# kazuto1011/dusty-gan-v2

Hardware: AMD Instinct MI355X
Metric: range-images/sec (G+D step) on dusty_v2 64x512 (higher is better)
Workload: dtype bf16; 1 GPU; configs[2]: configs/gans/dusty_v2.yaml full G+D train step (G step + D step + lazy R1 + ADA + EMA + Adam), 64x512 synthetic; global_batch=64, per_gpu_batch=64, parallelism=dp1, hip_graph=True, d_epilogue_dtype=fp32, pe_table_precomputed=True

## Files before the change

### dusty-gan-v2_amd/csrc/conv_wgrad_stream.hip

```cpp
#include "gemm_core.h"

namespace {

struct WSGeom {
  int B, H, W, C, O, Ho, Wo, k, stride, pad, ring;
  int tiles_h, tiles_w, ntiles, tiles_per_split, ctiles;
#ifdef DGV2_ABLATE
  int ablate;
#define WS_ABL (g.ablate)
#else
#define WS_ABL 0
#endif
  int x_shared;
  int x_exact;
  int* status;
};

template <typename T, int S, int MFN, int NFN, bool K3>
struct WSCfg {
  static constexpr int KS = TnFrag<T>::KS;
  static constexpr int CE = 16 / sizeof(T);
  static constexpr int TO = 16 * MFN, TC = 16 * NFN;
  static constexpr int PAD = sizeof(T) == 4 ? 16 : 0;
  static constexpr int RO = TO + PAD, RC = TC + PAD;
// ... 500 lines not shown
      rg[j][1] = src[1];
      if (!ok) rg[j][0] = rg[j][1] = make_float4(0.f, 0.f, 0.f, 0.f);
    }
#pragma unroll
    for (int j = 0; j < NX; ++j) {
      const int id = tid + j * 256;
      const int xp = xpos[j] < 0 ? 0 : xpos[j];
      int hi = h0 - 1 + (xp >> 16), wi = w0 - 1 + (xp & 0xffff);
      hi = hi < 0 ? 0 : (hi >= g.H ? g.H - 1 : hi);
      wi = wi < 0 ? wi + g.W : (wi >= g.W ? wi - g.W : wi);
      const float4* src = reinterpret_cast<const float4*>(xb + (hi * g.W + wi) * g.C + (id & 7) * 8);
      rx[j][0] = src[0];
      rx[j][1] = src[1];
    }
  };

  f32x4 acc[9][4];
#pragma unroll
  for (int t = 0; t < 9; ++t)
#pragma unroll
    for (int mw = 0; mw < 4; ++mw) acc[t][mw] = (f32x4){0.f, 0.f, 0.f, 0.f};

  const int fg = lane >> 4, fi = lane & 15;
  const int fq = fi >> 2, fp = fi & 3;
  int voffA[4][2], voffB[3][2];
#pragma unroll
  for (int h = 0; h < 2; ++h) {
    const int L = 8 * fg + fq + 4 * h;
#pragma unroll
    for (int mw = 0; mw < 4; ++mw) voffA[mw][h] = L * 128 + ((mw ^ wz_swz<128>(L)) * 32) + 8 * fp;
#pragma unroll
    for (int cs = 0; cs < 3; ++cs) voffB[cs][h] = 3 * GYB + (cs + L) * 128 + ((wave ^ wz_swz<128>(cs + L)) * 32) + 8 * fp;
  }

  const int t_begin = split * g.tiles_per_split;
  const int t_end = min(t_begin + g.tiles_per_split, g.ntiles);
  tw_n = t_begin % g.tiles_w;
  th_n = (t_begin / g.tiles_w) % g.tiles_h;
  b_n = t_begin / (g.tiles_w * g.tiles_h);
  if (t_begin < t_end) issue();
  for (int t = t_begin; t < t_end; ++t) {
    __syncthreads();
#pragma unroll
    for (int j = 0; j < NG; ++j) {
      uint4 h, m, l;
      wx_split8(rg[j][0], rg[j][1], h, m, l);
      lds_gy[gw_[j]] = h;
      lds_gy[GYB / 16 + gw_[j]] = m;
      lds_gy[2 * (GYB / 16) + gw_[j]] = l;
    }
#pragma unroll
    for (int j = 0; j < NX; ++j) {
      uint4 h, m, l;
      wx_split8(rx[j][0], rx[j][1], h, m, l);
      if (xpos[j] >= 0) {
        lds_x[xw_[j]] = h;
        if (!xe) {
          lds_x[XB / 16 + xw_[j]] = m;
          lds_x[2 * (XB / 16) + xw_[j]] = l;
        } else if ((m.x | m.y | m.z | m.w) != 0u) {
          atomicOr(g.status, DGV2_STATUS_X_INEXACT);
        }
      }
    }
    if (t + 1 < t_end) issue();
    __syncthreads();
    wx3_tile<XE>(acc, lbase, voffA, voffB);
  }
  __builtin_amdgcn_sched_barrier(0);
  asm volatile("s_nop 15\n\ts_nop 15" ::: "memory");
  __builtin_amdgcn_sched_barrier(0);

  const int lr = lane & 15, lc = lane >> 4;
  float* pb = part + (int64_t)split * g.O * 9 * g.C;
  const int c = c0 + wave * 16 + lr;
#pragma unroll
  for (int tap = 0; tap < 9; ++tap)
#pragma unroll
    for (int mw = 0; mw < 4; ++mw)
#pragma unroll
      for (int r = 0; r < 4; ++r) {
        const int o = o0 + mw * 16 + lc * 4 + r;
        pb[((int64_t)o * 9 + tap) * g.C + c] = acc[tap][mw][r];
      }
}

template <int NC>
__global__ __launch_bounds__(1024) void conv_wgrad_x3_tail_kernel(float* __restrict__ tpart, const float* __restrict__ gy,
                                                                  const float* __restrict__ x, WSGeom g, int c0, int tiles_per_ts) {
  __shared__ float red[8][128];
  const int ts = blockIdx.x, o0 = blockIdx.y * 128;
  const int ol = threadIdx.x & 127, pl = threadIdx.x >> 7;
  const int t_begin = ts * tiles_per_ts, t_end = min(t_begin + tiles_per_ts, g.ntiles);
  float acc[9][NC];
#pragma unroll
  for (int t = 0; t < 9; ++t)
#pragma unroll
    for (int k = 0; k < NC; ++k) acc[t][k] = 0.f;
  for (int tile = t_begin; tile < t_end; ++tile) {
    const int tw = tile % g.tiles_w, th = (tile / g.tiles_w) % g.tiles_h, b = tile / (g.tiles_w * g.tiles_h);
    const float* gyb = gy + (int64_t)b * g.Ho * g.Wo * g.O + o0 + ol;
    const float* xb = x + (int64_t)b * g.H * g.W * g.C + c0;
#pragma unroll 4
    for (int p = pl; p < 128; p += 8) {
      const int ho = th * 4 + (p >> 5), wo = tw * 32 + (p & 31);
      if (ho >= g.Ho) continue;
      const float gv = gyb[(ho * g.Wo + wo) * g.O];
#pragma unroll
      for (int t = 0; t < 9; ++t) {
        int hi = ho + t / 3 - 1, wi = wo + t % 3 - 1;
        hi = hi < 0 ? 0 : (hi >= g.H ? g.H - 1 : hi);
        wi = wi < 0 ? wi + g.W : (wi >= g.W ? wi - g.W : wi);
        const float* xp = xb + (hi * g.W + wi) * g.C;
#pragma unroll
        for (int k = 0; k < NC; ++k) acc[t][k] = fmaf(gv, xp[k], acc[t][k]);
      }
    }
  }
  float* out = tpart + ((int64_t)ts * g.O + o0 + ol) * 9 * NC;
#pragma unroll
  for (int t = 0; t < 9; ++t)
#pragma unroll
    for (int k = 0; k < NC; ++k) {
      red[pl][ol] = acc[t][k];
      __syncthreads();
      if (pl == 0) {
        float v = red[0][ol];
#pragma unroll
        for (int l = 1; l < 8; ++l) v += red[l][ol];
        out[t * NC + k] = v;
      }
      __syncthreads();
    }
}

__global__ __launch_bounds__(256) void conv_wgrad_x3_tail_reduce_kernel(float* __restrict__ part, const float* __restrict__ tpart,
                                                                        int O, int C, int c0, int clive, int NC, int TS, int nsplit) {
  const int nz = C - c0;
  const int64_t n = (int64_t)nsplit * O * 9 * nz;
  for (int64_t i = blockIdx.x * 256 + threadIdx.x; i < n; i += (int64_t)gridDim.x * 256) {
    const int k = (int)(i % nz);
    const int64_t r = i / nz;
    const int t = (int)(r % 9);
    const int o = (int)((r / 9) % O), split = (int)(r / 9 / O);
    float v = 0.f;
    if (split == 0 && k < NC && c0 + k < clive)
      for (int s = 0; s < TS; ++s) v += tpart[(((int64_t)s * O + o) * 9 + t) * NC + k];
    part[(((int64_t)split * O + o) * 9 + t) * C + c0 + k] = v;
  }
}

__global__ __launch_bounds__(256) void wgrad_reduce_kernel(float* __restrict__ gw, const float* __restrict__ part,
                                                           int64_t n, int nsplit, float scale = 1.f, int kkC = 0,
                                                           int Cc = 0, int64_t ldo = 0) {
  __shared__ float4 red[16][16];
  const int col = threadIdx.x & 15, sl = threadIdx.x >> 4;
  const int64_t i = ((int64_t)blockIdx.x * 16 + col) * 4;
  part += (int64_t)blockIdx.y * nsplit * n;
  gw += (int64_t)blockIdx.y * (ldo > 0 ? (n / Cc) * ldo : n);
  float4 s = make_float4(0.f, 0.f, 0.f, 0.f);
  if (i < n) {
#pragma unroll 4
    for (int k = sl; k < nsplit; k += 16) {
      const float4 v = *reinterpret_cast<const float4*>(part + (int64_t)k * n + i);
      s.x += v.x; s.y += v.y; s.z += v.z; s.w += v.w;
    }
  }
  red[sl][col] = s;
  __syncthreads();
  if (sl == 0 && i < n) {
#pragma unroll
    for (int k = 1; k < 16; ++k) {
      const float4 v = red[k][col];
      s.x += v.x; s.y += v.y; s.z += v.z; s.w += v.w;
    }
    s.x *= scale; s.y *= scale; s.z *= scale; s.w *= scale;
    if (kkC == 0 && ldo > 0) {
      const int64_t r = i / Cc;
      *reinterpret_cast<float4*>(gw + r * ldo + (i - r * Cc)) = s;
    } else if (kkC == 0) {
      *reinterpret_cast<float4*>(gw + i) = s;
    } else {
      const float v4[4] = {s.x, s.y, s.z, s.w};
      const int kk = kkC / Cc;
#pragma unroll
      for (int e = 0; e < 4; ++e) {
        const int64_t lin = i + e;
        const int64_t o = lin / kkC;
        const int r = (int)(lin - o * kkC);
        const int t = r / Cc, c = r - t * Cc;
        gw[(o * Cc + c) * kk + t] = v4[e];
      }
    }
  }
}

struct WSPlan {
  WSGeom g;
  int nsplit, otiles, mfn, nfn;
  int go;
};

bool ws_plan(WSPlan& p, int B, int H, int W, int C, int O, int k, int stride, int pad, int ring, int dtype,
             bool per_image = false) {
  if (B <= 0 || H <= 0 || W <= 0 || C <= 0 || O <= 0) return false;
  if ((k != 1 && k != 3) || pad != (k - 1) / 2 || (stride != 1 && stride != 2)) return false;
  const int ce = dtype == DGV2_BF16 ? 8 : 4;
  if (C % ce || O % ce) return false;
  WSGeom& g = p.g;
  g = WSGeom{B, H, W, C, O, (H + 2 * pad - k) / stride + 1, (W + 2 * pad - k) / stride + 1, k, stride, pad, ring};
  if (g.Ho <= 0 || g.Wo <= 0) return false;
  const bool wide32 = dtype == DGV2_F32 && k == 3 && stride == 1 && C >= 128 && O >= 128;
  const bool big = dtype == DGV2_BF16 || wide32;
  p.mfn = (big && O > 32) ? 4 : 2;
  p.nfn = (big && C > 32) ? 4 : 2;
  const int wr = stride == 1 ? 4 : 2;
  g.tiles_h = (g.Ho + wr - 1) / wr;
  g.tiles_w = (g.Wo + 31) / 32;
  g.ntiles = B * g.tiles_h * g.tiles_w;
  g.ctiles = (C + 16 * p.nfn - 1) / (16 * p.nfn);
  static const bool no_go2 = getenv("DGV2_WS_NO_GO2") != nullptr;
  static const bool go2_s1 = getenv("DGV2_WS_GO2_S1") != nullptr;
  p.go = (!no_go2 && dtype == DGV2_BF16 && p.mfn == 4 && p.nfn == 4 && k == 3 && (stride == 2 || go2_s1) && O % 128 == 0 &&
          !per_image) ? 2 : 1;
  p.otiles = (O + 16 * p.mfn * p.go - 1) / (16 * p.mfn * p.go);
  const int pairs = g.ctiles * p.otiles;
#ifdef DGV2_ABLATE
  static const int abl = getenv("DGV2_WS_ABLATE") ? atoi(getenv("DGV2_WS_ABLATE")) : 0;
  g.ablate = abl;
#endif
  g.x_shared = 0;
  static const int blocks_big = getenv("DGV2_WS_BLOCKS_BIG") ? atoi(getenv("DGV2_WS_BLOCKS_BIG")) : 512;
  static const int blocks_small = getenv("DGV2_WS_BLOCKS_SMALL") ? atoi(getenv("DGV2_WS_BLOCKS_SMALL")) : 512;
  int nsplit = (p.go == 2 ? 256 : wide32 ? 512 : (p.mfn == 4 && p.nfn == 4) ? blocks_big : blocks_small) / pairs;
  nsplit = nsplit < 1 ? 1 : (nsplit > g.ntiles ? g.ntiles : nsplit);
  g.tiles_per_split = (g.ntiles + nsplit - 1) / nsplit;
  p.nsplit = (g.ntiles + g.tiles_per_split - 1) / g.tiles_per_split;
  if (per_image) {
    const int tpi = g.tiles_h * g.tiles_w;
    int spi = nsplit / B;
    spi = spi < 1 ? 1 : (spi > tpi ? tpi : spi);
    while (tpi % spi) --spi;
    g.tiles_per_split = tpi / spi;
    p.nsplit = B * spi;
  }
  return true;
}

template <typename T, int S, int MFN, int NFN, bool K3>
int ws_launch(float* part, const void* gy, const void* x, const WSPlan& p, hipStream_t st) {
  dim3 grid(p.nsplit, p.g.ctiles * p.otiles);
  if constexpr (sizeof(T) == 2) {
    if constexpr (MFN == 4 && NFN == 4 && K3) {
      if (p.go == 2) {
        using Cf2 = WZCfg<S, MFN, NFN, K3, 2>;
        auto kern2 = conv_wgrad_stream_bf16_kernel<S, MFN, NFN, K3, 2>;
        if (Cf2::LDS > 64 * 1024) {
          hipError_t e = hipFuncSetAttribute((const void*)kern2, hipFuncAttributeMaxDynamicSharedMemorySize, (int)Cf2::LDS);
          if (e != hipSuccess) return (int)e;
        }
        kern2<<<grid, 512, Cf2::LDS, st>>>(part, (const bf16_t*)gy, (const bf16_t*)x, p.g);
        return 0;
      }
    }
    using Cf = WZCfg<S, MFN, NFN, K3>;
    auto kern = conv_wgrad_stream_bf16_kernel<S, MFN, NFN, K3, 1>;
    if (Cf::LDS > 64 * 1024) {
      hipError_t e = hipFuncSetAttribute((const void*)kern, hipFuncAttributeMaxDynamicSharedMemorySize, (int)Cf::LDS);
      if (e != hipSuccess) return (int)e;
    }
    kern<<<grid, 256, Cf::LDS, st>>>(part, (const bf16_t*)gy, (const bf16_t*)x, p.g);
  } else {
    using Cf = WSCfg<T, S, MFN, NFN, K3>;
    auto kern = conv_wgrad_stream_kernel<T, S, MFN, NFN, K3>;
    if (Cf::LDS > 64 * 1024) {
      hipError_t e = hipFuncSetAttribute((const void*)kern, hipFuncAttributeMaxDynamicSharedMemorySize, (int)Cf::LDS);
      if (e != hipSuccess) return (int)e;
    }
    kern<<<grid, 256, Cf::LDS, st>>>(part, (const T*)gy, (const T*)x, p.g);
  }
  return 0;
}

template <typename T, int S, bool K3>
int ws_dispatch(float* part, const void* gy, const void* x, const WSPlan& p, hipStream_t st) {
  if constexpr (sizeof(T) == 2) {
    if (p.mfn == 4 && p.nfn == 4) return ws_launch<T, S, 4, 4, K3>(part, gy, x, p, st);
    if (p.mfn == 4) return ws_launch<T, S, 4, 2, K3>(part, gy, x, p, st);
    if (p.nfn == 4) return ws_launch<T, S, 2, 4, K3>(part, gy, x, p, st);
  } else if constexpr (S == 1 && K3) {
    if (p.mfn == 4 && p.nfn == 4) return ws_launch<T, S, 4, 4, K3>(part, gy, x, p, st);
  }
  return ws_launch<T, S, 2, 2, K3>(part, gy, x, p, st);
}

template <typename T>
int ws_dispatch_geom(float* part, const void* gy, const void* x, const WSPlan& p, hipStream_t st) {
  if (p.g.k == 3)
    return p.g.stride == 1 ? ws_dispatch<T, 1, true>(part, gy, x, p, st) : ws_dispatch<T, 2, true>(part, gy, x, p, st);
  return p.g.stride == 1 ? ws_dispatch<T, 1, false>(part, gy, x, p, st) : ws_dispatch<T, 2, false>(part, gy, x, p, st);
}

}

extern "C" int dgv2_conv_wgrad_stream_scratch(int64_t* elems, int B, int H, int W, int C, int O, int k, int stride,
                                              int pad, int dtype) {
  if (!elems) return DGV2_EINVAL;
  *elems = 0;
  WSPlan p;
  if (!ws_plan(p, B, H, W, C, O, k, stride, pad, 1, dtype)) return DGV2_EINVAL;
  *elems = (int64_t)p.nsplit * O * k * k * C;
  return 0;
}

extern "C" int dgv2_bmm_tn_stream_scratch(int64_t* elems, int B, int H, int W, int C, int O, int dtype) {
  if (!elems) return DGV2_EINVAL;
  *elems = 0;
  WSPlan p;
  if (!ws_plan(p, B, H, W, C, O, 1, 1, 0, 0, dtype, true)) return DGV2_EINVAL;
  *elems = (int64_t)p.nsplit * O * C;
  return 0;
}

extern "C" int dgv2_bmm_tn_stream_ld(float* gw, int64_t ldo, float* scratch, int64_t scratch_elems, const void* gy,
                                     const void* x, int x_shared, int B, int H, int W, int C, int O, int dtype, void* stream) {
  if (!gw || !scratch || !gy || !x || !aligned16(gy) || !aligned16(x) || !aligned16(scratch) || !aligned16(gw))
    return DGV2_EINVAL;
  if (ldo < 0 || (ldo > 0 && (ldo < C || (ldo & 3)))) return DGV2_EINVAL;
  if (dtype != DGV2_BF16 && dtype != DGV2_F32) return DGV2_EINVAL;
  WSPlan p;
  if (!ws_plan(p, B, H, W, C, O, 1, 1, 0, 0, dtype, true)) return DGV2_EINVAL;
  p.g.x_shared = x_shared != 0;
  const int64_t n = (int64_t)O * C;
  if (scratch_elems < (int64_t)p.nsplit * n || (n & 3)) return DGV2_EINVAL;
  hipStream_t st = (hipStream_t)stream;
  const int rc = dtype == DGV2_BF16 ? ws_dispatch_geom<bf16_t>(scratch, gy, x, p, st)
                                    : ws_dispatch_geom<float>(scratch, gy, x, p, st);
  if (rc) return rc;
  dim3 grid((unsigned)((n / 4 + 15) / 16), B);
  wgrad_reduce_kernel<<<grid, 256, 0, st>>>(gw, scratch, n, p.nsplit / B, 1.f, 0, C, ldo);
  DGV2_RETURN_LAST();
}

extern "C" int dgv2_conv_wgrad_stream_pl(float* gw, float* scratch, int64_t scratch_elems, const void* gy, const void* x,
                                         int B, int H, int W, int C, int O, int k, int stride, int pad, int ring,
                                         float scale, int param_layout, int dtype, void* stream) {
  if (!gw || !scratch || !gy || !x || !aligned16(gy) || !aligned16(x) || !aligned16(scratch) || !aligned16(gw))
    return DGV2_EINVAL;
  if (dtype != DGV2_BF16 && dtype != DGV2_F32) return DGV2_EINVAL;
  WSPlan p;
  if (!ws_plan(p, B, H, W, C, O, k, stride, pad, ring, dtype)) return DGV2_EINVAL;
  const int64_t n = (int64_t)O * k * k * C;
  if (scratch_elems < (int64_t)p.nsplit * n) return DGV2_EINVAL;
  hipStream_t st = (hipStream_t)stream;
  int rc;
  if (ring && (p.g.tiles_w * 32 - 1) * stride + k - 1 - pad < 2 * W && pad <= W) p.g.ring = 2;
  rc = dtype == DGV2_BF16 ? ws_dispatch_geom<bf16_t>(scratch, gy, x, p, st) : ws_dispatch_geom<float>(scratch, gy, x, p, st);
  if (rc) return rc;
  wgrad_reduce_kernel<<<(int)((n / 4 + 15) / 16), 256, 0, st>>>(gw, scratch, n, p.nsplit, scale,
                                                                 param_layout ? k * k * C : 0, C);
  DGV2_RETURN_LAST();
}

extern "C" int dgv2_conv3x3_x3_wgrad(float* gw, float* scratch, int64_t scratch_elems, const void* gy, const void* x, int B,
                                     int H, int W, int C, int clive, int x_exact, int O, float scale, int param_layout,
                                     int* status, void* stream) {
  if (!gw || !scratch || !gy || !x || !aligned16(gy) || !aligned16(x) || !aligned16(scratch) || !aligned16(gw))
    return DGV2_EINVAL;
  if (B < 1 || H < 1 || W < 1 || C < 1 || O < 1 || clive < 1 || clive > C || x_exact < 0 || x_exact > C) return DGV2_EINVAL;
  if (x_exact > 0 && !status) return DGV2_EINVAL;
  static const bool off = getenv("DGV2_NO_CONV_X3") != nullptr || getenv("DGV2_NO_WGRAD_X3") != nullptr;
  const int ctiles = C / 64, ntail = clive - ctiles * 64;
  if (off || O % 64 || ctiles < 1 || C % 8 || ntail > 16 || W % 32) return DGV2_ENOTSUP;
  if ((int64_t)B * H * W * (C > O ? C : O) >= (1ll << 31)) return DGV2_ENOTSUP;
  WSPlan p;
  WSGeom& g = p.g;
  g = WSGeom{B, H, W, C, O, H, W, 3, 1, 1, 2};
  g.tiles_h = (H + 3) / 4;
  g.tiles_w = W / 32;
  g.ntiles = B * g.tiles_h * g.tiles_w;
  g.ctiles = ctiles;
  g.x_shared = 0;
  g.x_exact = x_exact;
  g.status = status;
#ifdef DGV2_ABLATE
  g.ablate = 0;
#endif
  const int pairs = ctiles * (O / 64);
  int nsplit = 256 / pairs;
  nsplit = nsplit < 1 ? 1 : (nsplit > g.ntiles ? g.ntiles : nsplit);
  g.tiles_per_split = (g.ntiles + nsplit - 1) / nsplit;
  nsplit = (g.ntiles + g.tiles_per_split - 1) / g.tiles_per_split;
  const int64_t n = (int64_t)O * 9 * C;
  const bool tail = C > ctiles * 64;
  const int NC = ntail <= 1 ? 1 : (ntail <= 4 ? 4 : 16);
  const int TS = g.ntiles < 64 ? g.ntiles : 64, tiles_per_ts = (g.ntiles + TS - 1) / TS;
  const int64_t tneed = tail ? (int64_t)TS * O * 9 * NC : 0;
  if (scratch_elems < (int64_t)nsplit * n + tneed || O % 128) return DGV2_ENOTSUP;
  hipStream_t st = (hipStream_t)stream;
  const bool xe = x_exact >= ctiles * 64;
  auto kern = xe ? conv_wgrad_x3_kernel<true> : conv_wgrad_x3_kernel<false>;
  static bool attr_set[2] = {false, false};
  if (!attr_set[xe]) {
    hipError_t e = hipFuncSetAttribute((const void*)kern, hipFuncAttributeMaxDynamicSharedMemorySize, (int)WXCfg::LDS);
    if (e != hipSuccess) return (int)e;
    attr_set[xe] = true;
  }
  kern<<<dim3(nsplit, pairs), 256, WXCfg::LDS, st>>>(scratch, (const float*)gy, (const float*)x, g);
  if (tail) {
    float* tpart = scratch + (int64_t)nsplit * n;
    const dim3 tg(TS, O / 128);
    const int c0 = ctiles * 64;
    if (NC == 1) conv_wgrad_x3_tail_kernel<1><<<tg, 1024, 0, st>>>(tpart, (const float*)gy, (const float*)x, g, c0, tiles_per_ts);
    else if (NC == 4) conv_wgrad_x3_tail_kernel<4><<<tg, 1024, 0, st>>>(tpart, (const float*)gy, (const float*)x, g, c0, tiles_per_ts);
    else conv_wgrad_x3_tail_kernel<16><<<tg, 1024, 0, st>>>(tpart, (const float*)gy, (const float*)x, g, c0, tiles_per_ts);
    conv_wgrad_x3_tail_reduce_kernel<<<grid_for((int64_t)nsplit * O * 9 * (C - c0), 256), 256, 0, st>>>(scratch, tpart, O, C, c0,
                                                                                                      clive, NC, TS, nsplit);
  }
  wgrad_reduce_kernel<<<(int)((n / 4 + 15) / 16), 256, 0, st>>>(gw, scratch, n, nsplit, scale, param_layout ? 9 * C : 0, C);
  DGV2_RETURN_LAST();
}

extern "C" int dgv2_conv3x3_x3_wgrad_scratch(int64_t* elems, int B, int H, int W, int C, int clive, int O) {
  if (!elems) return DGV2_EINVAL;
  *elems = 0;
  if (B < 1 || H < 1 || W < 1 || C < 64 || O < 1 || clive < 1 || clive > C) return DGV2_EINVAL;
  const int ctiles = C / 64, ntail = clive - ctiles * 64;
  if (O % 128 || C % 8 || ntail > 16 || W % 32) return DGV2_ENOTSUP;
  const int ntiles = B * ((H + 3) / 4) * (W / 32);
  int nsplit = 256 / (ctiles * (O / 64));
  nsplit = nsplit < 1 ? 1 : (nsplit > ntiles ? ntiles : nsplit);
  const int tps = (ntiles + nsplit - 1) / nsplit;
  nsplit = (ntiles + tps - 1) / tps;
  const int NC = ntail <= 1 ? 1 : (ntail <= 4 ? 4 : 16);
  const int TS = ntiles < 64 ? ntiles : 64;
  *elems = (int64_t)nsplit * O * 9 * C + (C > ctiles * 64 ? (int64_t)TS * O * 9 * NC : 0);
  return 0;
}
```

### dusty-gan-v2_amd/csrc/conv_x3.hip

```cpp
#include <stdlib.h>

#include "gemm_core.h"

namespace {

struct CX3 {
  int B, H, W, Cx;
  int nchunks;
  int O, ldy;
  int xexact;
  int tiles_h, tiles_w, ntiles, npairs, nslab, per_xcd, total;
  int* status;
  const float* bias;
  const float* resid;
  int act;
  float alpha, scale;
#ifdef DGV2_ABLATE
  int ablate;
#define X3_ABL (p.ablate)
#else
#define X3_ABL 0
#endif
};

constexpr int X_ICOLS = 34, X_NPIX = 6 * X_ICOLS, X_PIN = 208, X_PW = 9 * 64, X_NI = 4, X_NW = 5;
constexpr int X_TILE = 3 * 4 * X_PIN;
constexpr int X_WBUF = 4 * X_PW;
constexpr size_t X_LDS = sizeof(uint4) * (2 * X_TILE + 2 * X_WBUF + 512);
static_assert(X_LDS <= 160 * 1024 - 1024, "LDS image");

__device__ __forceinline__ void split3x8(const float4& lo, const float4& hi, uint4& h, uint4& m, uint4& l) {
  const float f[8] = {lo.x, lo.y, lo.z, lo.w, hi.x, hi.y, hi.z, hi.w};
  union { uint4 u; bf16_t e[8]; } ph, pm, pl;
#pragma unroll
  for (int i = 0; i < 8; ++i) {
    const bf16_t hh = (bf16_t)f[i];
    const float r1 = f[i] - (float)hh;
    const bf16_t mm = (bf16_t)r1;
    const float r2 = r1 - (float)mm;
    ph.e[i] = hh;
    pm.e[i] = mm;
    pl.e[i] = (bf16_t)r2;
  }
  h = ph.u;
  m = pm.u;
  l = pl.u;
}


__device__ __forceinline__ bool exact1x8(const float4& lo, const float4& hi, uint4& h) {
  const float f[8] = {lo.x, lo.y, lo.z, lo.w, hi.x, hi.y, hi.z, hi.w};
  union { uint4 u; bf16_t e[8]; } ph;
  bool bad = false;
#pragma unroll
  for (int i = 0; i < 8; ++i) {
    ph.e[i] = (bf16_t)f[i];
    bad |= (f[i] - (float)ph.e[i]) != 0.f;
  }
  h = ph.u;
  return bad;
}

template <bool NOP>
__device__ __forceinline__ void mfma4_bf16(f32x4& c0, f32x4& c1, f32x4& c2, f32x4& c3, const uint4& a0, const uint4& a1,
                                           const uint4& a2, const uint4& a3, const uint4& b) {
  union U { uint4 u; bf16x8 v; };
  U ua0, ua1, ua2, ua3, ub;
  ua0.u = a0; ua1.u = a1; ua2.u = a2; ua3.u = a3; ub.u = b;
  if constexpr (NOP) {
    asm volatile(
        "v_mfma_f32_16x16x32_bf16 %0, %4, %8, %0\n\t"
        "v_mfma_f32_16x16x32_bf16 %1, %5, %8, %1\n\t"
        "v_mfma_f32_16x16x32_bf16 %2, %6, %8, %2\n\t"
        "v_mfma_f32_16x16x32_bf16 %3, %7, %8, %3\n\t"
        "s_nop 7"
        : "+v"(c0), "+v"(c1), "+v"(c2), "+v"(c3)
        : "v"(ua0.v), "v"(ua1.v), "v"(ua2.v), "v"(ua3.v), "v"(ub.v));
  } else {
    asm volatile(
        "v_mfma_f32_16x16x32_bf16 %0, %4, %8, %0\n\t"
        "v_mfma_f32_16x16x32_bf16 %1, %5, %8, %1\n\t"
        "v_mfma_f32_16x16x32_bf16 %2, %6, %8, %2\n\t"
        "v_mfma_f32_16x16x32_bf16 %3, %7, %8, %3"
        : "+v"(c0), "+v"(c1), "+v"(c2), "+v"(c3)
        : "v"(ua0.v), "v"(ua1.v), "v"(ua2.v), "v"(ua3.v), "v"(ub.v));
  }
}

#define X3_SB() __builtin_amdgcn_sched_barrier(0)
#ifdef DGV2_ABLATE
__device__ int x3_abl_noreads;
#define X3_NOREADS (x3_abl_noreads != 0)
#else
#define X3_NOREADS false
#endif

template <int NX, int HZ, typename Side>
__device__ __forceinline__ void x3_stage(f32x4 (&acc)[4][2], const uint4* __restrict__ a_base, const uint4* __restrict__ xb,
                                         const int (&bpix)[2], unsigned dead, Side&& side) {
  constexpr int SLOTS = 2 * NX;
  const bool noreads = X3_NOREADS;
  uint4 a[2][4], bb[2][NX];
  unsigned dd = 0u;
  if constexpr (HZ != 0) {
    dd = dead;
    asm volatile("" : "+s"(dd));
  }
#pragma unroll
  for (int mf = 0; mf < 4; ++mf) a[0][mf] = a_base[mf * 16];
#pragma unroll
  for (int nf = 0; nf < 2; ++nf)
#pragma unroll
    for (int q = 0; q < NX; ++q) bb[nf][q] = xb[q * 4 * X_PIN + bpix[nf]];
#pragma unroll
  for (int t = 0; t < 9; ++t) {
#pragma unroll
    for (int nf = 0; nf < 2; ++nf) {
#pragma unroll
      for (int qi = 0; qi < NX; ++qi) {
        const int q = NX - 1 - qi;
        X3_SB();
        if (!(HZ && ((dd >> t) & 1u)))
        {
          mfma4_bf16<true>(acc[0][nf], acc[1][nf], acc[2][nf], acc[3][nf], a[t & 1][0], a[t & 1][1], a[t & 1][2], a[t & 1][3], bb[nf][q]);
        }
        if constexpr (HZ != 0) {
          if (t < 3 || t >= 6) {
            const int tm = t < 3 ? t + 6 : t - 6;
            if ((dd >> tm) & 1u) {
              const uint4 bx = xb[q * 4 * X_PIN + bpix[nf] + X_ICOLS + t % 3];
              mfma4_bf16<true>(acc[0][nf], acc[1][nf], acc[2][nf], acc[3][nf], a[t & 1][0], a[t & 1][1], a[t & 1][2], a[t & 1][3], bx);
            }
          }
        }
        X3_SB();
        if (t + 1 < 9 && !noreads) {
          const int ky = (t + 1) / 3, kx = (t + 1) % 3;
          bb[nf][q] = xb[q * 4 * X_PIN + bpix[nf] + ky * X_ICOLS + kx];
          const int slot = nf * NX + qi;
#pragma unroll
          for (int k = 0; k < 4; ++k)
            if (k >= slot * 4 / SLOTS && k < (slot + 1) * 4 / SLOTS) a[(t + 1) & 1][k] = a_base[(t + 1) * 64 + k * 16];
        }
      }
    }
    X3_SB();
    side(t);
  }
  X3_SB();
}

template <int HZ, bool XE>
__global__ __launch_bounds__(512, 2) void conv_x3_kernel(float* __restrict__ y, const float* __restrict__ x,
                                                         const bf16_t* __restrict__ wimg, CX3 p) {
  extern __shared__ __attribute__((aligned(16))) uint4 smem[];
  __shared__ __attribute__((aligned(16))) float s_bias[64];
  const int n = blockIdx.x, kk = n >> 3;
  const int item = (n & 7) * p.per_xcd + kk;
  if (kk >= p.per_xcd || item >= p.total) return;
  const int slab = item / p.npairs, pair = item - slab * p.npairs;

  const int tid = threadIdx.x;
  const int t256 = tid & 255, gn = tid >> 8;
  const int wave4 = (tid >> 6) & 3, lane = tid & 63;
  const int lr = lane & 15, lc = lane >> 4;
  uint4* const xs = smem + gn * X_TILE;
  uint4* const wb = smem + 2 * X_TILE;
// ... 19 lines not shown
    gh = gh < 0 ? 0 : (gh >= p.H ? p.H - 1 : gh);
    int gw = w0 - 1 + ix;
    gw = gw < 0 ? gw + p.W : (gw >= p.W ? gw - p.W : gw);
    goff[j] = (gh * p.W + gw) * p.Cx + in_plane * 8;
    lrow[j] = pix < X_NPIX ? pix : -1;
  }
  float4 rin[X_NI][2];
  bool rin_ok = true;
  auto issue_in = [&](int c0) {
    rin_ok = c0 + in_plane * 8 < p.Cx;
    const int cc = rin_ok ? c0 : -in_plane * 8;
#pragma unroll
    for (int j = 0; j < X_NI; ++j) {
      const float4* src = reinterpret_cast<const float4*>(xb_g + cc + goff[j]);
      rin[j][0] = src[0];
      rin[j][1] = src[1];
    }
  };
  typedef __attribute__((ext_vector_type(4))) unsigned u32x4;
  u32x4 rwt[X_NW];
  const size_t plane_units = (size_t)p.nslab * p.nchunks * (X_PW * 4);
  auto issue_w = [&](int st) {
    const int c = st / 3, pl = st - c * 3;
    const u32x4* img = reinterpret_cast<const u32x4*>(wimg) + pl * plane_units + ((size_t)slab * p.nchunks + c) * (X_PW * 4) + tid;
#pragma unroll
    for (int j = 0; j < X_NW; ++j)
      if (j < X_NW - 1 || tid + 512 * j < X_PW * 4) rwt[j] = img[512 * j];
  };
  const int w_plane = (tid >> 3) & 3, w_row0 = ((tid >> 5) << 3) | (tid & 7);
  auto write_w = [&](int buf) {
    uint4* dst = wb + buf * X_WBUF + w_plane * X_PW + w_row0;
#pragma unroll
    for (int j = 0; j < X_NW; ++j)
      if (j < X_NW - 1 || tid + 512 * j < X_PW * 4) *reinterpret_cast<u32x4*>(dst + 128 * j) = rwt[j];
  };

  f32x4 acc[4][2];
#pragma unroll
  for (int mf = 0; mf < 4; ++mf)
#pragma unroll
    for (int nf = 0; nf < 2; ++nf) acc[mf][nf] = (f32x4){0.f, 0.f, 0.f, 0.f};
  int bpix[2];
#pragma unroll
  for (int nf = 0; nf < 2; ++nf) bpix[nf] = wave4 * X_ICOLS + nf * 16 + lr;
  if (tid < 64) s_bias[tid] = p.bias ? p.bias[o0 + tid] : 0.f;

  unsigned dead = 0u;
  if constexpr (HZ != 0) {
    const int orow = h0 + wave4;
    unsigned m = 0;
#pragma unroll
    for (int t = 0; t < 9; ++t)
      if ((unsigned)(orow + t / 3 - 1) >= (unsigned)p.H) m |= 1u << t;
    dead = (unsigned)__builtin_amdgcn_readfirstlane((int)m);
  }

  const int nst = p.nchunks * 3;
  uint4* const w_dummy = smem + 2 * X_TILE + 2 * X_WBUF + tid;
  auto w_store = [&](int st, int j) {
    if (X3_ABL & 8) return;
    const bool in = j < X_NW - 1 || tid + 512 * j < X_PW * 4;
    uint4* dst = wb + ((st + 1) & 1) * X_WBUF + w_plane * X_PW + w_row0 + 128 * j;
    dst = in ? dst : w_dummy;
    *reinterpret_cast<u32x4*>(dst) = rwt[j];
  };
  auto w_load = [&](int st, int j) {
    if (X3_ABL & 8) return;
    const bool in = j < X_NW - 1 || tid + 512 * j < X_PW * 4;
    const int s2 = min(st + 2, nst - 1);
    const int c = s2 / 3, pl = s2 - c * 3;
    const u32x4* img = reinterpret_cast<const u32x4*>(wimg) + pl * plane_units + ((size_t)slab * p.nchunks + c) * (X_PW * 4) + tid;
    rwt[j] = img[in ? 512 * j : 0];
  };
  auto w_side = [&](int st, int t) {
    if (t < X_NW) w_store(st, t);
    if (t == 5) { w_load(st, 0); w_load(st, 1); }
    if (t > 5) w_load(st, t - 4);
  };
  uint4 xh[X_NI];
  auto split_store = [&](int j, bool all, bool ex) {
    if (ex) {
      const bool bad = exact1x8(rin[j][0], rin[j][1], xh[j]);
      if (bad && rin_ok && lrow[j] >= 0) atomicOr(p.status, DGV2_STATUS_X_INEXACT);
      if (!rin_ok) xh[j] = make_uint4(0u, 0u, 0u, 0u);
      if (all && lrow[j] >= 0) xs[in_plane * X_PIN + lrow[j]] = xh[j];
      return;
    }
    uint4 m, l;
    split3x8(rin[j][0], rin[j][1], xh[j], m, l);
    if (!rin_ok) xh[j] = m = l = make_uint4(0u, 0u, 0u, 0u);
    if (lrow[j] >= 0) {
      uint4* d = xs + in_plane * X_PIN + lrow[j];
      if (all) d[0] = xh[j];
      d[4 * X_PIN] = m;
      d[8 * X_PIN] = l;
    }
  };

  issue_w(0);
  issue_in(0);
  write_w(0);
  if (nst > 1) issue_w(1);
#pragma unroll
  for (int j = 0; j < X_NI; ++j) split_store(j, true, XE && 32 <= p.xexact);
  __syncthreads();
  const uint4* const xlane = xs + lc * X_PIN;
  for (int c = 0; c < p.nchunks; ++c) {
    const bool more = c + 1 < p.nchunks && !(X3_ABL & 4);
    const int st = c * 3;
    const bool ex = XE && (c + 1) * 32 <= p.xexact, ex_next = XE && (min(c + 1, p.nchunks - 1) + 1) * 32 <= p.xexact;
    const uint4* const a0 = wb + (st & 1) * X_WBUF + lc * X_PW + lr;
    const uint4* const a1 = wb + ((st + 1) & 1) * X_WBUF + lc * X_PW + lr;
    auto side0 = [&](int t) {
      w_side(st, t);
      if (t == 5 && !(X3_ABL & 4)) issue_in(min(c + 1, p.nchunks - 1) * 32);
    };
    if (X3_ABL & 2) { for (int t = 0; t < 9; ++t) side0(t); }
    else if (ex) x3_stage<1, HZ>(acc, a0, xlane, bpix, dead, side0);
    else x3_stage<3, HZ>(acc, a0, xlane, bpix, dead, side0);
    if (!(X3_ABL & 64)) __syncthreads();
    auto side1 = [&](int t) { w_side(st + 1, t); };
    if (X3_ABL & 2) { for (int t = 0; t < 9; ++t) side1(t); }
    else if (ex) x3_stage<1, HZ>(acc, a1, xlane, bpix, dead, side1);
    else x3_stage<2, HZ>(acc, a1, xlane, bpix, dead, side1);
    if (!(X3_ABL & 64)) __syncthreads();
    auto side2 = [&](int t) {
      if (t < X_NI && !(X3_ABL & 4)) split_store(t, false, ex_next);
      w_side(st + 2, t);
    };
    if (X3_ABL & 2) { for (int t = 0; t < 9; ++t) side2(t); }
    else x3_stage<1, HZ>(acc, a0, xlane, bpix, dead, side2);
    if (!(X3_ABL & 64)) __syncthreads();
    if (more) {
#pragma unroll
      for (int j = 0; j < X_NI; ++j)
        if (lrow[j] >= 0) xs[in_plane * X_PIN + lrow[j]] = xh[j];
      if (!(X3_ABL & 64)) __syncthreads();
    }
  }

  mfma_drain();
  const int gh = h0 + wave4;
#pragma unroll
  for (int nf = 0; nf < 2; ++nf) {
    const int gw = w0 + nf * 16 + lr;
    const bool live = tile_live && gh < p.H && gw < p.W;
    const int64_t row = (((int64_t)b * p.H + gh) * p.W + gw) * p.ldy;
#pragma unroll
    for (int mf = 0; mf < 4; ++mf) {
      const int o = o0 + mf * 16 + lc * 4;
      const float4 b4 = *reinterpret_cast<const float4*>(&s_bias[mf * 16 + lc * 4]);
      const float bq[4] = {b4.x, b4.y, b4.z, b4.w};
      float f[4];
#pragma unroll
      for (int r = 0; r < 4; ++r) {
        float t = acc[mf][nf][r] + bq[r];
        if (p.act == 3) t = fmaxf(t, t * p.alpha) * p.scale;
        f[r] = t;
      }
      if (live && o < p.O) {
        if (p.resid) {
          const float4 r4 = *reinterpret_cast<const float4*>(p.resid + row + o);
          f[0] += r4.x; f[1] += r4.y; f[2] += r4.z; f[3] += r4.w;
        }
        *reinterpret_cast<float4*>(y + row + o) = make_float4(f[0], f[1], f[2], f[3]);
      }
    }
  }
}

__global__ __launch_bounds__(256) void x3_dgrad_tail_kernel(float* __restrict__ gx, const float* __restrict__ gy,
                                                            const float* __restrict__ wt, const float* __restrict__ resid,
                                                            int B, int H, int W, int ldx, int O, int c0, int nc, int cend) {
  const int row = blockIdx.x;
  const int b = row / H, h = row - b * H;
  const int lane = threadIdx.x & 63, wave = threadIdx.x >> 6;
  const int per = (W + 3) / 4;
  const float* gimg = gy + (int64_t)b * H * W * O;
  const bool border = h == 0 || h == H - 1;
  for (int ci = 0; ci < nc; ++ci) {
    const float* wc = wt + (size_t)(c0 + ci) * 9 * O;
    for (int w0 = wave * per; w0 < min(W, (wave + 1) * per); w0 += 8) {
      float s[8];
#pragma unroll
      for (int k = 0; k < 8; ++k) s[k] = 0.f;
      for (int ob = lane * 4; ob < O; ob += 256) {
#pragma unroll
        for (int d = 0; d < 3; ++d) {
          const int gh = h + d - 1;
          if (gh < 0 || gh >= H) continue;
          const float* grow = gimg + (int64_t)gh * W * O + ob;
#pragma unroll
          for (int kx = 0; kx < 3; ++kx) {
            float4 k4 = *reinterpret_cast<const float4*>(wc + ((2 - d) * 3 + kx) * O + ob);
            if (d == 1 && border) {
              const float4 e = *reinterpret_cast<const float4*>(wc + ((h == 0 ? 0 : 2) * 3 + kx) * O + ob);
              k4.x += e.x; k4.y += e.y; k4.z += e.z; k4.w += e.w;
            }
#pragma unroll
            for (int k = 0; k < 8; ++k) {
              int j = w0 + k + 1 - kx;
              j = j < 0 ? j + W : (j >= W ? j - W : j);
              j = j >= W ? 0 : j;
              const float4 g = *reinterpret_cast<const float4*>(grow + (int64_t)j * O);
              s[k] = fmaf(g.x, k4.x, fmaf(g.y, k4.y, fmaf(g.z, k4.z, fmaf(g.w, k4.w, s[k]))));
            }
          }
        }
      }
#pragma unroll
      for (int k = 0; k < 8; ++k) {
        const float v = wave_sum(s[k]);
        const int w = w0 + k;
        if (lane == 0 && w < min(W, (wave + 1) * per)) {
          const int64_t at = ((int64_t)row * W + w) * ldx + c0 + ci;
          gx[at] = v + (resid ? resid[at] : 0.f);
        }
      }
    }
  }
  const int nz = cend - c0 - nc;
  for (int i = threadIdx.x; i < W * nz; i += 256) {
    const int64_t at = ((int64_t)row * W + i / nz) * ldx + c0 + nc + i % nz;
    gx[at] = resid ? resid[at] : 0.f;
  }
}

__global__ __launch_bounds__(256) void x3_image_fwd_kernel(bf16_t* __restrict__ w3, const float* __restrict__ w, int O, int Cp,
                                                           int nch) {
  const int n = O * 9 * nch * 4;
  const size_t plane = (size_t)(O >> 6) * nch * (X_PW * 4);
  for (int i = blockIdx.x * 256 + threadIdx.x; i < n; i += gridDim.x * 256) {
    const int c8 = i % (nch * 4), r = i / (nch * 4);
    const int t = r % 9, o = r / 9;
    float4 lo = make_float4(0.f, 0.f, 0.f, 0.f), hi = lo;
    if (c8 * 8 < Cp) {
      const float4* src = reinterpret_cast<const float4*>(w + ((size_t)o * 9 + t) * Cp + c8 * 8);
      lo = src[0];
      hi = src[1];
    }
    uint4 h, m, l;
    split3x8(lo, hi, h, m, l);
    const int row = t * 64 + (o & 63);
    const size_t unit = ((size_t)(o >> 6) * nch + (c8 >> 2)) * (X_PW * 4) + (row >> 3) * 32 + (c8 & 3) * 8 + (row & 7);
    uint4* img = reinterpret_cast<uint4*>(w3);
    img[unit] = h;
    img[plane + unit] = m;
    img[2 * plane + unit] = l;
  }
}

__global__ __launch_bounds__(256) void x3_image_bwd_kernel(bf16_t* __restrict__ w3t, const float* __restrict__ w, int O, int Cp,
                                                           int nslab) {
  const int CS = nslab * 64, nch = O / 32;
  const int n = CS * 9 * (O / 8);
  const size_t plane = (size_t)nslab * nch * (X_PW * 4);
  for (int i = blockIdx.x * 256 + threadIdx.x; i < n; i += gridDim.x * 256) {
    const int c = i % CS, r = i / CS;
    const int t = r % 9, o8 = r / 9;
    float f[8];
#pragma unroll
    for (int k = 0; k < 8; ++k) f[k] = w[((size_t)(o8 * 8 + k) * 9 + t) * Cp + c];
    uint4 h, m, l;
    split3x8(make_float4(f[0], f[1], f[2], f[3]), make_float4(f[4], f[5], f[6], f[7]), h, m, l);
    const int row = (8 - t) * 64 + (c & 63);
    const size_t unit = ((size_t)(c >> 6) * nch + (o8 >> 2)) * (X_PW * 4) + (row >> 3) * 32 + (o8 & 3) * 8 + (row & 7);
    uint4* img = reinterpret_cast<uint4*>(w3t);
    img[unit] = h;
    img[plane + unit] = m;
    img[2 * plane + unit] = l;
  }
}

template <int HZ, bool XE>
int launch_x3(float* y, const float* x, const bf16_t* wimg, CX3 p, hipStream_t st) {
  auto kern = conv_x3_kernel<HZ, XE>;
  static bool attr_set = false;
  if (!attr_set) {
    hipError_t e = hipFuncSetAttribute((const void*)kern, hipFuncAttributeMaxDynamicSharedMemorySize, (int)X_LDS);
    if (e != hipSuccess) return (int)e;
    attr_set = true;
  }
  p.tiles_h = (p.H + 3) / 4;
  p.tiles_w = p.W / 32;
  p.ntiles = p.B * p.tiles_h * p.tiles_w;
  p.npairs = (p.ntiles + 1) / 2;
  p.total = p.npairs * p.nslab;
  p.per_xcd = (p.total + 7) / 8;
#ifdef DGV2_ABLATE
  p.ablate = getenv("DGV2_X3_ABLATE") ? atoi(getenv("DGV2_X3_ABLATE")) : 0;
  {
    const int nr = (p.ablate & 128) ? 1 : 0;
    (void)hipMemcpyToSymbol(HIP_SYMBOL(x3_abl_noreads), &nr, sizeof(int));
  }
#endif
  kern<<<p.per_xcd * 8, 512, X_LDS, st>>>(y, x, wimg, p);
  return 0;
}

}

extern "C" int dgv2_conv3x3_x3_fwd(void* y, const void* x, const void* w3, int B, int H, int W, int Cx, int x_exact, int O,
                                   const float* bias, const void* resid, int act, float alpha, float scale, int* status,
                                   void* stream) {
  if (!y || !x || !w3 || B < 1 || H < 1 || W < 1 || Cx < 1 || O < 1 || x_exact < 0 || x_exact > Cx) return DGV2_EINVAL;
  if (x_exact > 0 && !status) return DGV2_EINVAL;
  if (act != 0 && act != 3) return DGV2_EINVAL;
  static const bool off = getenv("DGV2_NO_CONV_X3") != nullptr;
  if (off || W % 32 || Cx % 8 || O % 64 || Cx < 64) return DGV2_ENOTSUP;
  if (!aligned16(y) || !aligned16(x) || !aligned16(w3) || (resid && !aligned16(resid))) return DGV2_ENOTSUP;
  if ((int64_t)B * H * W * (Cx > O ? Cx : O) >= (1ll << 31)) return DGV2_ENOTSUP;
  CX3 p;
  p.B = B; p.H = H; p.W = W; p.Cx = Cx; p.nchunks = (Cx + 31) / 32; p.O = O; p.ldy = O; p.nslab = O / 64;
  p.xexact = x_exact;
  p.status = status;
  p.bias = bias; p.resid = (const float*)resid; p.act = act; p.alpha = alpha; p.scale = scale;
  const int rc = x_exact >= 32 ? launch_x3<0, true>((float*)y, (const float*)x, (const bf16_t*)w3, p, (hipStream_t)stream)
                               : launch_x3<0, false>((float*)y, (const float*)x, (const bf16_t*)w3, p, (hipStream_t)stream);
  if (rc) return rc;
  DGV2_RETURN_LAST();
}

extern "C" int dgv2_conv3x3_x3_dgrad(void* gx, const void* gy, const void* w3t, const void* wt, int B, int H, int W, int C,
                                     int ldx, int O, const void* resid, void* stream) {
  if (!gx || !gy || !w3t || !wt || B < 1 || H < 1 || W < 1 || C < 1 || ldx < C || O < 1) return DGV2_EINVAL;
  static const bool off = getenv("DGV2_NO_CONV_X3") != nullptr;
  const int nslab = C / 64, ntail = C - nslab * 64;
  if (off || H < 2 || W % 32 || O % 32 || O < 64 || nslab < 1 || ntail > 16 || ldx % 4 || nslab != ldx / 64)
    return DGV2_ENOTSUP;
  if (!aligned16(gx) || !aligned16(gy) || !aligned16(w3t) || !aligned16(wt) || (resid && !aligned16(resid))) return DGV2_ENOTSUP;
  if ((int64_t)B * H * W * (ldx > O ? ldx : O) >= (1ll << 31)) return DGV2_ENOTSUP;
  CX3 p;
  p.B = B; p.H = H; p.W = W; p.Cx = O; p.nchunks = O / 32; p.O = nslab * 64; p.ldy = ldx; p.nslab = nslab;
  p.xexact = 0;
  p.status = nullptr;
  p.bias = nullptr; p.resid = (const float*)resid; p.act = 0; p.alpha = 0.2f; p.scale = 1.f;
  hipStream_t st = (hipStream_t)stream;
  const int rc = launch_x3<1, false>((float*)gx, (const float*)gy, (const bf16_t*)w3t, p, st);
  if (rc) return rc;
  if (ldx > nslab * 64)
    x3_dgrad_tail_kernel<<<B * H, 256, 0, st>>>((float*)gx, (const float*)gy, (const float*)wt, (const float*)resid, B, H, W,
                                               ldx, O, nslab * 64, ntail, ldx);
  DGV2_RETURN_LAST();
}

extern "C" int dgv2_conv_x3_images(void* w3, void* w3t, const void* w, int O, int Cp, void* stream) {
  if ((!w3 && !w3t) || !w || O < 64 || O % 64 || Cp < 64 || Cp % 8) return DGV2_EINVAL;
  if ((w3 && !aligned16(w3)) || !aligned16(w) || (w3t && !aligned16(w3t))) return DGV2_EINVAL;
  hipStream_t st = (hipStream_t)stream;
  const int nch = (Cp + 31) / 32;
  if (w3)
    x3_image_fwd_kernel<<<grid_for((int64_t)O * 9 * nch * 4, 256), 256, 0, st>>>((bf16_t*)w3, (const float*)w, O, Cp, nch);
  if (w3t)
    x3_image_bwd_kernel<<<grid_for((int64_t)(Cp / 64) * 64 * 9 * (O / 8), 256), 256, 0, st>>>((bf16_t*)w3t, (const float*)w, O,
                                                                                                 Cp, Cp / 64);
  DGV2_RETURN_LAST();
}
```

### dusty-gan-v2_amd/csrc/mbstd.hip

```cpp
#include "common.h"

namespace {

constexpr int MB_G = 8;

struct MbGeom {
  int B, P, C, Cp, S, g, m, NS;
};

template <typename T, int N> __device__ __forceinline__ void ldN(const T* p, float (&f)[N]) {
  constexpr int V = vec16<T>::N;
#pragma unroll
  for (int h = 0; h < N / V; ++h) {
    vec16<T> v;
    v.load(p + h * V);
#pragma unroll
    for (int j = 0; j < V; ++j) f[h * V + j] = v.get(j);
  }
}
template <typename T, int N> __device__ __forceinline__ void stN(T* p, const float (&f)[N]) {
  constexpr int V = vec16<T>::N;
#pragma unroll
  for (int h = 0; h < N / V; ++h) {
    vec16<T> v;
#pragma unroll
    for (int j = 0; j < V; ++j) v.set(j, f[h * V + j]);
    v.store(p + h * V);
  }
}
template <typename TA, typename TB> struct mb_vn {
  static constexpr int value = vec16<TA>::N > vec16<TB>::N ? vec16<TA>::N : vec16<TB>::N;
};

template <typename T>
__global__ __launch_bounds__(256) void mbstd_partial_kernel(float* __restrict__ partial, const T* __restrict__ x, MbGeom q) {
  __shared__ float red[16];
  constexpr int VN = vec16<T>::N;
  const int sm = blockIdx.x, split = blockIdx.y;
  const int s = sm / q.m, mi = sm - s * q.m;
  const int64_t PC = (int64_t)q.P * q.C;
  const int64_t nvec = PC / VN;
  float acc = 0.f;
  for (int64_t v = (int64_t)split * 256 + threadIdx.x; v < nvec; v += (int64_t)q.NS * 256) {
    vec16<T> a[MB_G];
    float mu[VN];
#pragma unroll
    for (int j = 0; j < VN; ++j) mu[j] = 0.f;
#pragma unroll
    for (int gi = 0; gi < MB_G; ++gi) {
      if (gi < q.g) {
        const int b = (s * q.g + gi) * q.m + mi;
        a[gi].load(x + (int64_t)b * PC + v * VN);
#pragma unroll
        for (int j = 0; j < VN; ++j) mu[j] += a[gi].get(j);
      }
    }
    const float ig = 1.f / q.g;
#pragma unroll
    for (int j = 0; j < VN; ++j) {
      const float mean = mu[j] * ig;
      float var = 0.f;
#pragma unroll
      for (int gi = 0; gi < MB_G; ++gi)
        if (gi < q.g) {
          const float d = a[gi].get(j) - mean;
          var = fmaf(d, d, var);
        }
      acc += sqrtf(var * ig + 1e-8f);
    }
  }
  const float t = block_sum(acc, red);
  if (threadIdx.x == 0) partial[sm * q.NS + split] = t;
}

template <typename TX, typename TY>
__global__ __launch_bounds__(256) void mbstd_cat_kernel(TY* __restrict__ out, const TX* __restrict__ x,
                                                        const float* __restrict__ partial, MbGeom q) {
  constexpr int VN = mb_vn<TX, TY>::value;
  const int cvp = q.Cp / VN, cvx = q.C / VN;
  const int64_t total = (int64_t)q.B * q.P * cvp;
  const float inv = 1.f / ((float)q.P * q.C);
  for (int64_t i = (int64_t)blockIdx.x * 256 + threadIdx.x; i < total; i += (int64_t)gridDim.x * 256) {
    const int cv = (int)(i % cvp);
    const int64_t bp = i / cvp;
    float o[VN];
    if (cv < cvx) {
      ldN<TX, VN>(x + bp * q.C + cv * VN, o);
    } else {
#pragma unroll
      for (int j = 0; j < VN; ++j) o[j] = 0.f;
      if (cv == cvx) {
        const int b = (int)(bp / q.P);
        const int sg = b / q.m, mi = b - sg * q.m, s = sg / q.g;
        float st = 0.f;
        for (int k = 0; k < q.NS; ++k) st += partial[(s * q.m + mi) * q.NS + k];
        o[0] = st * inv;
      }
    }
    stN<TY, VN>(out + bp * q.Cp + cv * VN, o);
  }
}

template <typename TX, typename TG>
__global__ __launch_bounds__(256) void mbstd_bwd_kernel(TX* __restrict__ gx, const TG* __restrict__ gout,
                                                        const TX* __restrict__ x, MbGeom q) {
  __shared__ float red[16];
  __shared__ float s_gst;
  constexpr int VN = mb_vn<TX, TG>::value;
  const int sm = blockIdx.x, split = blockIdx.y;
  const int s = sm / q.m, mi = sm - s * q.m;
  const int64_t PC = (int64_t)q.P * q.C;
  float part = 0.f;
  for (int e = threadIdx.x; e < q.g * q.P; e += 256) {
    const int gi = e / q.P, p = e - gi * q.P;
    const int b = (s * q.g + gi) * q.m + mi;
    part += to_f32(gout[((int64_t)b * q.P + p) * q.Cp + q.C]);
  }
  part = block_sum(part, red);
  if (threadIdx.x == 0) s_gst = part / ((float)q.P * q.C);
  __syncthreads();
  const float k = s_gst / q.g;
  const int cvx = q.C / VN;
  const int64_t nvec = PC / VN;
  for (int64_t v = (int64_t)split * 256 + threadIdx.x; v < nvec; v += (int64_t)q.NS * 256) {
    const int64_t p = v / cvx;
    const int cv = (int)(v - p * cvx);
    float a[MB_G][VN];
    float mu[VN];
#pragma unroll
    for (int j = 0; j < VN; ++j) mu[j] = 0.f;
#pragma unroll
    for (int gi = 0; gi < MB_G; ++gi) {
      if (gi < q.g) {
        const int b = (s * q.g + gi) * q.m + mi;
        ldN<TX, VN>(x + (int64_t)b * PC + v * VN, a[gi]);
#pragma unroll
        for (int j = 0; j < VN; ++j) mu[j] += a[gi][j];
      }
    }
    const float ig = 1.f / q.g;
    float coef[VN];
#pragma unroll
    for (int j = 0; j < VN; ++j) {
      mu[j] *= ig;
      float var = 0.f;
#pragma unroll
      for (int gi = 0; gi < MB_G; ++gi)
        if (gi < q.g) {
          const float d = a[gi][j] - mu[j];
          var = fmaf(d, d, var);
        }
      coef[j] = k / sqrtf(var * ig + 1e-8f);
    }
#pragma unroll
    for (int gi = 0; gi < MB_G; ++gi) {
      if (gi < q.g) {
        const int b = (s * q.g + gi) * q.m + mi;
        float go[VN], o[VN];
        ldN<TG, VN>(gout + ((int64_t)b * q.P + p) * q.Cp + cv * VN, go);
#pragma unroll
        for (int j = 0; j < VN; ++j) o[j] = go[j] + coef[j] * (a[gi][j] - mu[j]);
        stN<TX, VN>(gx + (int64_t)b * PC + v * VN, o);
      }
    }
  }
}

bool mb_ok(const MbGeom& q, int vn) {
  return q.B > 0 && q.P > 0 && q.C > 0 && q.S > 0 && q.g > 0 && q.g <= MB_G && q.m > 0 && q.S * q.g * q.m == q.B &&
         q.C % vn == 0 && q.Cp % vn == 0 && q.Cp > q.C && (int64_t)q.B * q.P * q.Cp < (1LL << 40);
}

int mb_splits(const MbGeom& q, int vn) {
  const int64_t nvec = (int64_t)q.P * q.C / vn;
  int ns = (int)((nvec + 1023) / 1024);
  const int want = (1024 + q.S * q.m - 1) / (q.S * q.m);
  ns = ns < want ? ns : want;
  return ns < 1 ? 1 : (ns > 64 ? 64 : ns);
}

}

extern "C" int dgv2_mbstd_cat_fwd_x(void* out, float* scratch, const void* x, int B, int P, int C, int Cp, int splits,
                                    int group, int xdtype, int ydtype, void* stream) {
  if (!out || !scratch || !x || splits < 1 || group < 1 || B % (splits * group)) return DGV2_EINVAL;
  if (xdtype != ydtype && !(xdtype == DGV2_BF16 && ydtype == DGV2_F32)) return DGV2_ENOTSUP;
  MbGeom q{B, P, C, Cp, splits, group, B / (splits * group), 1};
  const int vx = xdtype == DGV2_BF16 ? 8 : 4;
  if (!mb_ok(q, vx) || !aligned16(out) || !aligned16(x)) return DGV2_EINVAL;
  q.NS = mb_splits(q, vx);
  hipStream_t st = (hipStream_t)stream;
  dim3 grid(q.S * q.m, q.NS);
  const int64_t total = (int64_t)B * P * (Cp / vx);
  const int gc = grid_for(total, 256, 4096);
  if (xdtype == DGV2_F32) {
    mbstd_partial_kernel<float><<<grid, 256, 0, st>>>(scratch, (const float*)x, q);
    mbstd_cat_kernel<float, float><<<gc, 256, 0, st>>>((float*)out, (const float*)x, scratch, q);
  } else if (xdtype == DGV2_BF16) {
    mbstd_partial_kernel<bf16_t><<<grid, 256, 0, st>>>(scratch, (const bf16_t*)x, q);
    if (ydtype == DGV2_BF16)
      mbstd_cat_kernel<bf16_t, bf16_t><<<gc, 256, 0, st>>>((bf16_t*)out, (const bf16_t*)x, scratch, q);
    else
      mbstd_cat_kernel<bf16_t, float><<<gc, 256, 0, st>>>((float*)out, (const bf16_t*)x, scratch, q);
  } else {
    return DGV2_EINVAL;
  }
  DGV2_RETURN_LAST();
}

extern "C" int dgv2_mbstd_cat_bwd_x(void* gx, const void* gout, const void* x, int B, int P, int C, int Cp, int splits,
                                    int group, int xdtype, int gdtype, void* stream) {
  if (!gx || !gout || !x || splits < 1 || group < 1 || B % (splits * group)) return DGV2_EINVAL;
  if (xdtype != gdtype && !(xdtype == DGV2_BF16 && gdtype == DGV2_F32)) return DGV2_ENOTSUP;
  MbGeom q{B, P, C, Cp, splits, group, B / (splits * group), 1};
  const int vx = xdtype == DGV2_BF16 ? 8 : 4;
  if (!mb_ok(q, vx) || !aligned16(gx) || !aligned16(gout) || !aligned16(x)) return DGV2_EINVAL;
  q.NS = mb_splits(q, vx);
  hipStream_t st = (hipStream_t)stream;
  dim3 grid(q.S * q.m, q.NS);
  if (xdtype == DGV2_F32)
    mbstd_bwd_kernel<float, float><<<grid, 256, 0, st>>>((float*)gx, (const float*)gout, (const float*)x, q);
  else if (xdtype == DGV2_BF16 && gdtype == DGV2_BF16)
    mbstd_bwd_kernel<bf16_t, bf16_t><<<grid, 256, 0, st>>>((bf16_t*)gx, (const bf16_t*)gout, (const bf16_t*)x, q);
  else if (xdtype == DGV2_BF16)
    mbstd_bwd_kernel<bf16_t, float><<<grid, 256, 0, st>>>((bf16_t*)gx, (const float*)gout, (const bf16_t*)x, q);
  else
    return DGV2_EINVAL;
  DGV2_RETURN_LAST();
}
```

### dusty-gan-v2_amd/csrc/weight_bank.hip

```cpp
#include <stdlib.h>

#include "common.h"

namespace {

constexpr int WB_MAX = 32;

struct BankArgs {
  const float* src[WB_MAX];
  void* wf[WB_MAX];
  void* wt[WB_MAX];
  void* w8[WB_MAX];
  void* w8t[WB_MAX];
  int O[WB_MAX], C[WB_MAX], Cpad[WB_MAX], kk[WB_MAX];
  float scale[WB_MAX];
};

template <typename T>
__global__ __launch_bounds__(256) void weight_bank_kernel(BankArgs a) {
  const int l = blockIdx.y;
  const int O = a.O[l], C = a.C[l], Cp = a.Cpad[l], kk = a.kk[l];
  const float s = a.scale[l];
  const float* src = a.src[l];
  T* wf = reinterpret_cast<T*>(a.wf[l]);
  T* wt = reinterpret_cast<T*>(a.wt[l]);
  const int n = O * kk * Cp;
  for (int i = blockIdx.x * 256 + threadIdx.x; i < n; i += gridDim.x * 256) {
    const int c = i % Cp, r = i / Cp;
    const int t = r % kk, o = r / kk;
    const float v = c < C ? src[(o * C + c) * kk + t] * s : 0.f;
    wf[i] = from_f32<T>(v);
    wt[(c * kk + t) * O + o] = from_f32<T>(v);
  }
}

constexpr int WB_TO = 16, WB_TC = 32, WB_KK = 9;

template <typename T, int KK>
__global__ __launch_bounds__(256) void weight_bank_tiled_kernel(BankArgs a) {
  const int l = blockIdx.y;
  const int O = a.O[l], C = a.C[l], Cp = a.Cpad[l];
  const int kk = KK > 0 ? KK : a.kk[l];
  if (KK > 0 && a.kk[l] != KK) return;
  const int tc = (Cp + WB_TC - 1) / WB_TC, to = (O + WB_TO - 1) / WB_TO;
  if ((int)blockIdx.x >= tc * to) return;
  const int o0 = (blockIdx.x / tc) * WB_TO, c0 = (blockIdx.x % tc) * WB_TC;
  const float s = a.scale[l];
  const float* src = a.src[l];
  T* wf = reinterpret_cast<T*>(a.wf[l]);
  T* wt = reinterpret_cast<T*>(a.wt[l]);
  __shared__ float tile[WB_TO][WB_TC * WB_KK + 1];
  const int run = WB_TC * kk;
  for (int e0 = threadIdx.x; e0 < WB_TO * run; e0 += 256 * 8) {
    float v[8];
#pragma unroll
    for (int u = 0; u < 8; ++u) {
      const int e = e0 + u * 256;
      const int ec = min(e, WB_TO * run - 1);
      const int o = ec / run, r = ec - o * run;
      const int c = c0 + r / kk;
      const bool ok = e < WB_TO * run && o0 + o < O && c < C;
      const size_t idx = ok ? ((size_t)(o0 + o) * C + c0) * kk + r : 0;
      v[u] = ok ? src[idx] * s : 0.f;
    }
#pragma unroll
    for (int u = 0; u < 8; ++u) {
      const int e = e0 + u * 256;
      if (e < WB_TO * run) {
        const int o = e / run, r = e - o * run;
        tile[o][r] = v[u];
      }
    }
  }
  __syncthreads();
  for (int f = threadIdx.x; f < WB_TO * run; f += 256) {
    const int c = f % WB_TC, r = f / WB_TC;
    const int t = r % kk, o = r / kk;
    if (o0 + o < O && c0 + c < Cp) wf[((size_t)(o0 + o) * kk + t) * Cp + c0 + c] = from_f32<T>(tile[o][c * kk + t]);
  }
  if (KK == 9 && sizeof(T) == 2 && a.w8[l]) {
    T* w8 = reinterpret_cast<T*>(a.w8[l]);
    const int nchunks = Cp / WB_TC;
    for (int f = threadIdx.x; f < WB_TO * run; f += 256) {
      const int c = f % WB_TC, r = f / WB_TC;
      const int t = r % kk, o = r / kk;
      if (o0 + o < O) {
        const int og = o0 + o, row = t * 64 + (og & 63), plane = c >> 3;
        const size_t unit = ((size_t)(og >> 6) * nchunks + c0 / WB_TC) * (576 * 4) + (row >> 3) * 32 + plane * 8 + (row & 7);
        w8[unit * 8 + (c & 7)] = from_f32<T>(tile[o][c * kk + t]);
      }
    }
  }
  if (KK == 9 && sizeof(T) == 2 && a.w8t[l]) {
    T* w8t = reinterpret_cast<T*>(a.w8t[l]);
    const int nchunks = O / 32;
    for (int g = threadIdx.x; g < WB_TO * run; g += 256) {
      const int o = g % WB_TO, r = g / WB_TO;
      const int t = r % kk, c = r / kk;
      if (o0 + o < O && c0 + c < Cp) {
        const int og = o0 + o, cg = c0 + c, row = (8 - t) * 64 + (cg & 63), plane = (og & 31) >> 3;
        const size_t unit = ((size_t)(cg >> 6) * nchunks + (og >> 5)) * (576 * 4) + (row >> 3) * 32 + plane * 8 + (row & 7);
        w8t[unit * 8 + (og & 7)] = from_f32<T>(tile[o][c * kk + t]);
      }
    }
  }
  if constexpr (KK == 9 && sizeof(T) == 4) {
    auto split = [](float v, bf16_t& h, bf16_t& m, bf16_t& l) {
      h = (bf16_t)v;
      const float r1 = v - (float)h;
      m = (bf16_t)r1;
      l = (bf16_t)(r1 - (float)m);
    };
    if (a.w8[l]) {
      bf16_t* w8 = reinterpret_cast<bf16_t*>(a.w8[l]);
      const int nchunks = tc;
      const size_t plane = (size_t)(O >> 6) * nchunks * (576 * 4) * 8;
      for (int f = threadIdx.x; f < WB_TO * run; f += 256) {
        const int c = f % WB_TC, r = f / WB_TC;
        const int t = r % kk, o = r / kk;
        if (o0 + o < O) {
          const int og = o0 + o, row = t * 64 + (og & 63), pl = c >> 3;
          const size_t unit = ((size_t)(og >> 6) * nchunks + c0 / WB_TC) * (576 * 4) + (row >> 3) * 32 + pl * 8 + (row & 7);
          bf16_t h, m, lo;
          split(tile[o][c * kk + t], h, m, lo);
          w8[unit * 8 + (c & 7)] = h;
          w8[plane + unit * 8 + (c & 7)] = m;
          w8[2 * plane + unit * 8 + (c & 7)] = lo;
        }
      }
    }
    if (a.w8t[l]) {
      bf16_t* w8t = reinterpret_cast<bf16_t*>(a.w8t[l]);
      const int nchunks = O / 32, nslab = Cp >> 6;
      const size_t plane = (size_t)nslab * nchunks * (576 * 4) * 8;
      for (int g = threadIdx.x; g < WB_TO * run; g += 256) {
        const int o = g % WB_TO, r = g / WB_TO;
        const int t = r % kk, c = r / kk;
        if (o0 + o < O && c0 + c < nslab * 64) {
          const int og = o0 + o, cg = c0 + c, row = (8 - t) * 64 + (cg & 63), pl = (og & 31) >> 3;
          const size_t unit = ((size_t)(cg >> 6) * nchunks + (og >> 5)) * (576 * 4) + (row >> 3) * 32 + pl * 8 + (row & 7);
          bf16_t h, m, lo;
          split(tile[o][c * kk + t], h, m, lo);
          w8t[unit * 8 + (og & 7)] = h;
          w8t[plane + unit * 8 + (og & 7)] = m;
          w8t[2 * plane + unit * 8 + (og & 7)] = lo;
        }
      }
    }
  }
  for (int g = threadIdx.x; g < WB_TO * run; g += 256) {
    const int o = g % WB_TO, r = g / WB_TO;
    const int t = r % kk, c = r / kk;
    if (o0 + o < O && c0 + c < Cp) wt[((size_t)(c0 + c) * kk + t) * O + o0 + o] = from_f32<T>(tile[o][c * kk + t]);
  }
}

}

extern "C" int dgv2_conv_weight_bank_ex(void* const* wf, void* const* wt, void* const* w8, void* const* w8t,
                                        const float* const* src, const int* O, const int* C, const int* Cpad, const int* kk,
                                        const float* scale, int L, int dtype, void* stream) {
  if (!wf || !wt || !src || !O || !C || !Cpad || !kk || !scale || L < 1 || L > WB_MAX) return DGV2_EINVAL;
  BankArgs a;
  for (int l = 0; l < L; ++l) {
    a.w8[l] = w8 ? w8[l] : nullptr;
    a.w8t[l] = w8t ? w8t[l] : nullptr;
    if (dtype == DGV2_F32) {
      if (a.w8[l] && (kk[l] != 9 || O[l] % 64 || Cpad[l] % 8)) return DGV2_EINVAL;
      if (a.w8t[l] && (kk[l] != 9 || Cpad[l] < 64 || O[l] % 32)) return DGV2_EINVAL;
      continue;
    }
    if (a.w8[l] && (kk[l] != 9 || O[l] % 64 || Cpad[l] % 32 || dtype != DGV2_BF16)) return DGV2_EINVAL;
    if (a.w8t[l] && (kk[l] != 9 || Cpad[l] % 64 || O[l] % 32 || dtype != DGV2_BF16)) return DGV2_EINVAL;
  }
  int nmax = 0, tmax = 0, kmax = 0;
  for (int l = 0; l < L; ++l) {
    if (!wf[l] || !wt[l] || !src[l] || O[l] < 1 || C[l] < 1 || Cpad[l] < C[l] || kk[l] < 1) return DGV2_EINVAL;
    a.src[l] = src[l]; a.wf[l] = wf[l]; a.wt[l] = wt[l];
    a.O[l] = O[l]; a.C[l] = C[l]; a.Cpad[l] = Cpad[l]; a.kk[l] = kk[l]; a.scale[l] = scale[l];
    const int64_t n = (int64_t)O[l] * kk[l] * Cpad[l];
    if (n >= (1 << 30)) return DGV2_EINVAL;
    nmax = n > nmax ? (int)n : nmax;
    const int tiles = ((Cpad[l] + WB_TC - 1) / WB_TC) * ((O[l] + WB_TO - 1) / WB_TO);
    tmax = tiles > tmax ? tiles : tmax;
    kmax = kk[l] > kmax ? kk[l] : kmax;
  }
  hipStream_t st = (hipStream_t)stream;
  static const bool no_tiled = getenv("DGV2_NO_WB_TILED") != nullptr;
  if (kmax <= WB_KK && !no_tiled) {
    dim3 tgrid(tmax, L);
    bool has1 = false, has9 = false, other = false;
    for (int l = 0; l < L; ++l) {
      if (kk[l] == 1) has1 = true;
      else if (kk[l] == 9) has9 = true;
      else other = true;
    }
    if (other)
      for (int l = 0; l < L; ++l)
        if (a.w8[l] || a.w8t[l]) return DGV2_ENOTSUP;
    DGV2_DISPATCH_DTYPE(dtype, {
      if (other) {
        weight_bank_tiled_kernel<T, 0><<<tgrid, 256, 0, st>>>(a);
      } else {
        if (has9) weight_bank_tiled_kernel<T, 9><<<tgrid, 256, 0, st>>>(a);
        if (has1) weight_bank_tiled_kernel<T, 1><<<tgrid, 256, 0, st>>>(a);
      }
    });
    DGV2_RETURN_LAST();
  }
  for (int l = 0; l < L; ++l)
    if (a.w8[l] || a.w8t[l]) return DGV2_ENOTSUP;
  dim3 grid(grid_for(nmax, 256, 256), L);
  DGV2_DISPATCH_DTYPE(dtype, { weight_bank_kernel<T><<<grid, 256, 0, st>>>(a); });
  DGV2_RETURN_LAST();
}
```

### dusty-gan-v2_amd/dgv2_native/__init__.py

```python
import ctypes
import os

import torch

_HERE = os.path.dirname(os.path.abspath(__file__))
LIB_PATH = os.environ.get("DGV2_LIB_PATH") or os.path.join(os.path.dirname(_HERE), "lib", "libdgv2.so")

F32, BF16 = 0, 1
F16 = 3
ABI_VERSION = 60

_c_int, _c_i64, _c_f32, _c_ptr = ctypes.c_int, ctypes.c_int64, ctypes.c_float, ctypes.c_void_p

SIGNATURES = {
    "dgv2_abi_version": [],
    "dgv2_fused_bias_act": [_c_ptr] * 4 + [_c_i64] * 3 + [_c_int, _c_int, _c_f32, _c_f32, _c_int, _c_ptr],
    "dgv2_bias_grad": [_c_ptr, _c_ptr, _c_i64, _c_i64, _c_i64, _c_int, _c_ptr],
    "dgv2_bias_act_bwd_rs": [_c_ptr] * 4 + [_c_i64, _c_int, _c_f32, _c_f32, _c_ptr, _c_ptr, _c_i64, _c_int, _c_ptr],
    "dgv2_surface_normal": [_c_ptr, _c_ptr] + [_c_int] * 5 + [_c_ptr],
    "dgv2_gemm_x3": [_c_ptr, _c_ptr, _c_i64, _c_ptr, _c_ptr, _c_int, _c_int, _c_i64, _c_int, _c_int, _c_i64, _c_i64, _c_i64,
                     _c_int, _c_f32, _c_ptr],
    "dgv2_pe_wgrad_scratch": [_c_ptr] + [_c_int] * 4,
    "dgv2_pe_wgrad": [_c_ptr, _c_ptr, _c_i64, _c_ptr, _c_ptr] + [_c_int] * 4 + [_c_i64, _c_int, _c_ptr],
    "dgv2_mbstd_cat_fwd_x": [_c_ptr] * 3 + [_c_int] * 8 + [_c_ptr],
    "dgv2_mbstd_cat_bwd_x": [_c_ptr] * 3 + [_c_int] * 8 + [_c_ptr],
    "dgv2_scale_cast": [_c_ptr] * 3 + [_c_i64, _c_int, _c_int, _c_int, _c_ptr],
    "dgv2_upfirdn2d": [_c_ptr] * 3 + [_c_int] * 15 + [_c_ptr],
    "dgv2_resample": [_c_ptr] * 4 + [_c_int] * 19 + [_c_ptr],
    "dgv2_resample_tab_add_affine": [_c_ptr] * 8 + [_c_int] + [_c_ptr] * 3 + [_c_int] * 8 + [_c_ptr],
    "dgv2_fourier_feature": [_c_ptr] * 5 + [_c_int] * 8 + [_c_ptr],
    "dgv2_downsample_angle": [_c_ptr] * 4 + [_c_int] * 5 + [_c_ptr],
    "dgv2_bmm_tn": [_c_ptr] * 3 + [_c_int] * 7 + [_c_ptr],
    "dgv2_bmm_nn_cat_sq": [_c_ptr] * 4 + [_c_int] * 5 + [_c_ptr, _c_ptr, _c_int, _c_f32, _c_f32, _c_int, _c_int, _c_ptr, _c_int, _c_ptr,
                           _c_ptr],
    "dgv2_bmm_nn_sq": [_c_ptr] * 3 + [_c_int] * 6 + [_c_i64, _c_ptr, _c_ptr, _c_int, _c_f32, _c_f32, _c_ptr, _c_int, _c_int, _c_ptr, _c_int,
                       _c_ptr, _c_ptr],
    "dgv2_modconv_pe_fwd_sq": [_c_ptr] * 4 + [_c_int] * 5 + [_c_ptr, _c_ptr, _c_int, _c_f32, _c_f32, _c_int, _c_ptr, _c_int, _c_ptr,
                               _c_ptr],
    "dgv2_modconv_pe_fwd_head": [_c_ptr] * 4 + [_c_int] * 5 + [_c_ptr, _c_ptr, _c_int, _c_f32, _c_f32, _c_int, _c_ptr, _c_int, _c_ptr,
                                 _c_ptr, _c_ptr, _c_ptr],
    "dgv2_kitti_rows": [_c_ptr, _c_ptr, _c_ptr, _c_int, _c_int, _c_ptr],
    "dgv2_kitti_project": [_c_ptr] * 4 + [_c_int] * 4 + [_c_f32, _c_f32, _c_int, _c_ptr],
    "dgv2_fps_scratch": [_c_ptr, _c_int, _c_int],
    "dgv2_fps": [_c_ptr] * 3 + [_c_int] * 3 + [_c_ptr],
    "dgv2_gather_points": [_c_ptr] * 3 + [_c_int] * 4 + [_c_ptr],
    "dgv2_gather_points_grad": [_c_ptr] * 3 + [_c_int] * 4 + [_c_ptr],
    "dgv2_chamfer_fwd": [_c_ptr] * 6 + [_c_int] * 3 + [_c_ptr],
    "dgv2_nn_search": [_c_ptr] * 4 + [_c_int] * 4 + [_c_ptr],
    "dgv2_chamfer_bwd": [_c_ptr] * 8 + [_c_int] * 3 + [_c_ptr],
    "dgv2_emd_approxmatch": [_c_ptr] * 4 + [_c_int] * 3 + [_c_ptr],
    "dgv2_emd_matchcost": [_c_ptr] * 4 + [_c_int] * 3 + [_c_ptr],
    "dgv2_emd_matchcost_grad": [_c_ptr] * 5 + [_c_int] * 3 + [_c_ptr],
    "dgv2_emd_pairwise_cost": [_c_ptr] * 3 + [_c_int] * 4 + [_c_ptr],
    "dgv2_nsgan_loss": [_c_ptr, _c_ptr, _c_ptr, _c_int, _c_int, _c_f32, _c_ptr, _c_ptr, _c_ptr],
    "dgv2_modconv_pe_dgrad_actbwd_scratch": [_c_ptr] + [_c_int] * 4,
    "dgv2_modconv_pe_dgrad_actbwd": [_c_ptr, _c_ptr, _c_ptr, _c_i64] + [_c_ptr] * 4 + [_c_f32, _c_f32] + [_c_int] * 4 + [_c_ptr],
    "dgv2_colmean_lerp": [_c_ptr, _c_ptr, _c_int, _c_int, _c_i64, _c_f32, _c_ptr],
    "dgv2_d_tail_fwd": [_c_ptr] * 6 + [_c_int, _c_int] + [_c_f32] * 4 + [_c_ptr],
    "dgv2_d_tail_bwd": [_c_ptr] * 7 + [_c_int, _c_int] + [_c_f32] * 4 + [_c_ptr],
    "dgv2_rng_fill": [_c_ptr] * 5 + [_c_int, _c_ptr, _c_ptr],
    "dgv2_modconv_up_fwd": [_c_ptr] * 4 + [_c_int] * 7 + [_c_ptr] * 6 + [_c_int, _c_f32, _c_f32, _c_int, _c_ptr, _c_int, _c_ptr,
                            _c_ptr],
    "dgv2_modconv_up_t_lag": [_c_ptr] * 4 + [_c_f32] + [_c_ptr] * 4 + [_c_int] * 9 + [_c_ptr, _c_int, _c_ptr, _c_ptr],
    "dgv2_fir_same_mfma_q8": [_c_ptr] * 3 + [_c_int] * 4 + [_c_ptr],
    "dgv2_resample_tab_q8": [_c_ptr] * 5 + [_c_int] + [_c_ptr] * 3 + [_c_int] * 7 + [_c_ptr],
    "dgv2_fp8_quant_weights": [_c_ptr] * 6 + [_c_int] + [_c_ptr] * 3,
    "dgv2_fp8_dequant": [_c_ptr, _c_ptr, _c_i64, _c_f32, _c_ptr],
    "dgv2_conv_direct_fwd_fp8": [_c_ptr] * 4 + [_c_int] * 7 + [_c_ptr, _c_ptr, _c_int, _c_f32, _c_f32, _c_ptr],
    "dgv2_modconv_up_t": [_c_ptr] * 5 + [_c_f32] + [_c_int] * 9 + [_c_ptr],
    "dgv2_up2_lag_sumsq": [_c_ptr] * 5 + [_c_int] * 5 + [_c_ptr, _c_int, _c_ptr, _c_ptr],
    "dgv2_resample_tab_actbwd_scratch": [_c_ptr] + [_c_int] * 6,
    "dgv2_resample_tab_actbwd": [_c_ptr, _c_ptr, _c_ptr, _c_i64, _c_ptr, _c_ptr] + [_c_ptr] * 3 + [_c_int] + [_c_ptr] * 3
                                + [_c_int] * 7 + [_c_f32, _c_f32, _c_int, _c_ptr],
    "dgv2_fir_same_mfma_prep_scratch": [_c_ptr, _c_int, _c_int],
    "dgv2_fir_same_mfma_prep": [_c_ptr, _c_i64] + [_c_ptr] * 3 + [_c_int] + [_c_ptr] * 3 + [_c_int] * 3 + [_c_ptr, _c_ptr],
    "dgv2_fir_same_mfma": [_c_ptr] * 3 + [_c_int] * 4 + [_c_ptr],
    "dgv2_fir_same_mfma_actbwd_scratch": [_c_ptr] + [_c_int] * 4,
    "dgv2_fir_same_mfma_actbwd": [_c_ptr, _c_ptr, _c_ptr, _c_i64, _c_ptr, _c_ptr, _c_ptr] + [_c_int] * 4 + [_c_f32, _c_f32, _c_ptr],
    "dgv2_resample_tab_sq": [_c_ptr] * 5 + [_c_int] + [_c_ptr] * 3 + [_c_int] * 10 + [_c_ptr, _c_int, _c_ptr, _c_ptr],
    "dgv2_bmm_tn_cat": [_c_ptr] * 4 + [_c_int] * 6 + [_c_ptr],
    "dgv2_lerp_list": [_c_ptr] * 3 + [_c_int, _c_f32, _c_ptr],
    "dgv2_adam_prep": [_c_ptr, _c_ptr, _c_f32, _c_f32, _c_ptr],
    "dgv2_adam_step": [_c_ptr] * 5 + [_c_int, _c_ptr] + [_c_f32] * 4 + [_c_ptr],
    "dgv2_sumsq_list": [_c_ptr, _c_ptr, _c_int, _c_ptr, _c_ptr],
    "dgv2_clip_prep": [_c_ptr, _c_int, _c_f32, _c_ptr, _c_f32, _c_f32, _c_int, _c_ptr, _c_ptr],
    "dgv2_sgd_step": [_c_ptr] * 4 + [_c_int, _c_ptr] + [_c_f32] * 3 + [_c_ptr],
    "dgv2_pack2d": [_c_ptr] * 4 + [_c_int] * 3 + [_c_ptr],
    "dgv2_unpack2d": [_c_ptr] * 4 + [_c_int] * 3 + [_c_ptr],
    "dgv2_ema_scalar": [_c_ptr] * 3 + [_c_int] + [_c_f32] * 3 + [_c_int, _c_ptr, _c_int, _c_ptr],
    "dgv2_ema_scalar_group": [_c_ptr, _c_ptr, _c_int, _c_ptr, _c_int] + [_c_f32] * 3 + [_c_int, _c_ptr, _c_ptr],
    "dgv2_bmm_nn_small": [_c_ptr] * 4 + [_c_int] * 5 + [_c_ptr],
    "dgv2_bmm_nn_small_act_scratch": [_c_ptr] + [_c_int] * 5,
    "dgv2_bmm_nn_small_act": [_c_ptr] * 4 + [_c_int] * 4 + [_c_ptr, _c_ptr, _c_f32, _c_f32, _c_ptr, _c_ptr, _c_i64, _c_int, _c_ptr],
    "dgv2_bmm_tn_small": [_c_ptr] * 3 + [_c_int] * 5 + [_c_ptr],
    "dgv2_head_bwd_scratch": [_c_ptr] + [_c_int] * 5,
    "dgv2_head_bwd": [_c_ptr] * 5 + [_c_i64] + [_c_ptr] * 6 + [_c_f32, _c_f32] + [_c_int] * 5 + [_c_ptr],
    "dgv2_transpose_list": [_c_ptr] * 5 + [_c_int] * 3 + [_c_ptr],
    "dgv2_mod_prep_all_fwd": [_c_ptr] * 13 + [_c_ptr, _c_int, _c_int, _c_ptr],
    "dgv2_mod_prep_all_bwd": [_c_ptr, _c_i64] + [_c_ptr] * 15 + [_c_ptr, _c_int, _c_int, _c_ptr, _c_i64, _c_ptr],
    "dgv2_mod_prep_all_bwd_scratch": [_c_ptr, _c_ptr, _c_ptr, _c_int, _c_int],
    "dgv2_mod_prep_fwd": [_c_ptr] * 8 + [_c_int] * 9 + [_c_ptr],
    "dgv2_mod_prep_bwd": [_c_ptr] * 11 + [_c_int] * 9 + [_c_ptr],
    "dgv2_sum_squares": [_c_ptr, _c_ptr, _c_i64, _c_int, _c_int, _c_int, _c_ptr],
    "dgv2_conv_fwd": [_c_ptr] * 3 + [_c_int] * 10 + [_c_ptr, _c_int, _c_f32, _c_f32, _c_int, _c_ptr],
    "dgv2_conv_direct_fwd": [_c_ptr] * 3 + [_c_int] * 7 + [_c_ptr, _c_ptr, _c_int, _c_f32, _c_f32, _c_int, _c_ptr],
    "dgv2_conv_direct_dgrad": [_c_ptr] * 3 + [_c_int] * 7 + [_c_ptr, _c_int, _c_ptr],
    "dgv2_conv_wgrad_direct": [_c_ptr] * 3 + [_c_int] * 10 + [_c_ptr],
    "dgv2_conv1x1_fwd": [_c_ptr] * 3 + [_c_int] * 4 + [_c_ptr, _c_int, _c_ptr],
    "dgv2_conv1x1_dgrad": [_c_ptr] * 3 + [_c_int] * 4 + [_c_ptr, _c_int, _c_ptr],
    "dgv2_gemm_stream_nn": [_c_ptr] * 3 + [_c_int] * 6 + [_c_i64, _c_ptr, _c_ptr, _c_int, _c_f32, _c_f32, _c_ptr, _c_int, _c_int, _c_ptr,
                            _c_int, _c_ptr, _c_ptr],
    "dgv2_gemm_stream_nn_cat": [_c_ptr] * 4 + [_c_int] * 5 + [_c_ptr, _c_ptr, _c_int, _c_f32, _c_f32, _c_int, _c_int, _c_ptr, _c_int,
                                _c_ptr, _c_ptr],
    "dgv2_gemm_stream_tn": [_c_ptr] * 3 + [_c_int] * 7 + [_c_ptr],
    "dgv2_gemm_stream_tn_cat": [_c_ptr] * 4 + [_c_int] * 6 + [_c_ptr],
    "dgv2_bmm_tn_stream_scratch": [_c_ptr] + [_c_int] * 6,
    "dgv2_bmm_tn_stream_ld": [_c_ptr, _c_i64, _c_ptr, _c_i64, _c_ptr, _c_ptr] + [_c_int] * 7 + [_c_ptr],
    "dgv2_conv_weight_bank_ex": [_c_ptr] * 10 + [_c_int, _c_int, _c_ptr],
    "dgv2_glin_fwd": [_c_ptr] * 6 + [_c_int] * 3 + [_c_f32, _c_f32, _c_int, _c_f32, _c_int, _c_ptr, _c_ptr],
    "dgv2_glin_dinput": [_c_ptr, _c_int, _c_ptr, _c_i64, _c_ptr, _c_ptr, _c_ptr, _c_ptr, _c_int, _c_int, _c_int, _c_f32, _c_f32,
                         _c_int, _c_ptr],
    "dgv2_glin_dweight": [_c_ptr] * 7 + [_c_int] * 3 + [_c_f32, _c_f32, _c_f32, _c_ptr, _c_ptr],
    "dgv2_conv3x3_dgrad8": [_c_ptr] * 3 + [_c_int] * 5 + [_c_ptr, _c_int, _c_ptr],
    "dgv2_conv3x3_s2_dgrad8": [_c_ptr] * 3 + [_c_int] * 6 + [_c_ptr],
    "dgv2_conv3x3_x3_wgrad_scratch": [_c_ptr] + [_c_int] * 6,
    "dgv2_conv3x3_x3_wgrad": [_c_ptr, _c_ptr, _c_i64] + [_c_ptr] * 2 + [_c_int] * 7 + [_c_f32, _c_int, _c_ptr, _c_ptr],
    "dgv2_conv_x3_images": [_c_ptr] * 3 + [_c_int] * 2 + [_c_ptr],
    "dgv2_conv3x3_x3_dgrad": [_c_ptr] * 4 + [_c_int] * 6 + [_c_ptr, _c_ptr],
    "dgv2_conv3x3_x3_fwd": [_c_ptr] * 3 + [_c_int] * 6 + [_c_ptr, _c_ptr, _c_int, _c_f32, _c_f32, _c_ptr, _c_ptr],
    "dgv2_conv3x3_fwd8": [_c_ptr] * 3 + [_c_int] * 6 + [_c_ptr, _c_ptr, _c_int, _c_f32, _c_f32, _c_int, _c_ptr],
    "dgv2_conv_wgrad_stream_scratch": [_c_ptr] + [_c_int] * 9,
    "dgv2_conv_wgrad_stream_pl": [_c_ptr, _c_ptr, _c_i64, _c_ptr, _c_ptr] + [_c_int] * 9 + [_c_f32, _c_int, _c_int, _c_ptr],
    "dgv2_conv_dgrad": [_c_ptr] * 4 + [_c_int] * 11 + [_c_ptr],
    "dgv2_conv_wgrad": [_c_ptr] * 3 + [_c_int] * 11 + [_c_ptr],
    "dgv2_stem_fwd": [_c_ptr] * 4 + [_c_int] * 5 + [_c_f32, _c_f32, _c_int, _c_ptr],
    "dgv2_stem_bwd_scratch": [_c_ptr] + [_c_int] * 4,
    "dgv2_stem_bwd_skip": [_c_ptr] * 4 + [_c_i64] + [_c_ptr] * 8 + [_c_int] + [_c_ptr] * 3 + [_c_int] * 8 + [_c_f32, _c_f32, _c_int,
                                                                                                        _c_ptr],
    "dgv2_gen_tail_fwd": [_c_ptr] * 7 + [_c_int] * 3 + [_c_f32] * 3 + [_c_ptr],
    "dgv2_gen_tail_bwd": [_c_ptr] * 11 + [_c_int] * 3 + [_c_f32] * 3 + [_c_ptr],
    "dgv2_ada_apply": [_c_ptr] * 8 + [_c_int] * 5 + [_c_ptr],
    "dgv2_ada_sample": [_c_ptr] * 7 + [_c_int] * 3 + [_c_ptr],
    "dgv2_ada_build": [_c_ptr] * 8 + [_c_int] * 4 + [_c_ptr],
    "dgv2_ada_sample_img": [_c_ptr] * 7 + [_c_int, _c_ptr],
    "dgv2_ada_fold": [_c_ptr] * 11 + [_c_int] * 6 + [_c_ptr],
    "dgv2_ada_apply_img": [_c_ptr] * 11 + [_c_int] * 5 + [_c_ptr],
    "dgv2_coords_convert": [_c_ptr] * 4 + [_c_int] * 3 + [_c_f32] * 3 + [_c_int, _c_ptr],
    "dgv2_msml_prepare": [_c_ptr] * 6 + [_c_int] * 5 + [_c_ptr],
    "dgv2_msml_fwd": [_c_ptr] * 7 + [_c_int] * 7 + [_c_ptr],
    "dgv2_msml_bwd": [_c_ptr] * 9 + [_c_int] * 7 + [_c_ptr],
    "dgv2_coords_convert_bwd": [_c_ptr] * 5 + [_c_int] * 3 + [_c_f32, _c_f32, _c_int, _c_ptr],
    "dgv2_fourier_feature_bwd": [_c_ptr] * 6 + [_c_int] * 8 + [_c_ptr],
    "dgv2_frame_points": [_c_ptr] * 4 + [_c_int] * 3 + [_c_f32, _c_f32, _c_int, _c_ptr],
    "dgv2_colorize": [_c_ptr] * 3 + [_c_int] * 4 + [_c_ptr],
    "dgv2_crf_rnn_forward": [_c_ptr] * 11 + [_c_int] * 7 + [_c_ptr],
    "dgv2_crf_rnn_backward_scratch": [_c_ptr] + [_c_int] * 5,
    "dgv2_crf_rnn_backward": [_c_ptr] * 5 + [_c_i64] + [_c_ptr] * 11 + [_c_int] * 7 + [_c_ptr],
    "dgv2_knn2d": [_c_ptr] * 4 + [_c_int] * 7 + [_c_f32, _c_ptr],
    "dgv2_seg_confusion": [_c_ptr] * 4 + [_c_i64, _c_int, _c_ptr],
    "dgv2_seg_loss_scratch": [_c_ptr] + [_c_int] * 3,
    "dgv2_seg_loss_forward": [_c_ptr] * 5 + [_c_i64] + [_c_ptr] * 4 + [_c_int] * 4 + [_c_f32, _c_int, _c_ptr],
    "dgv2_seg_loss_backward": [_c_ptr] * 7 + [_c_int] * 4 + [_c_f32, _c_int, _c_int, _c_ptr],
    "dgv2_fire_fwd": [_c_ptr] * 23 + [_c_f32] * 3 + [_c_int] * 9 + [_c_ptr],
    "dgv2_cam_fwd": [_c_ptr] * 6 + [_c_int] * 6 + [_c_ptr],
}


def _load():
    if not os.path.exists(LIB_PATH):
        raise ImportError(
            f"{LIB_PATH} not found: build it with `make` (or __graft_entry__.build()). "
            "The MI355X path has no CPU fallback."
        )
    lib = ctypes.CDLL(LIB_PATH)
    for name, argtypes in SIGNATURES.items():
        fn = getattr(lib, name)
        fn.argtypes = argtypes
        fn.restype = ctypes.c_int
    got = lib.dgv2_abi_version()
    if got != ABI_VERSION:
        raise ImportError(f"libdgv2.so ABI version {got}, binding expects {ABI_VERSION}")
    return lib


lib = _load()


def dtype_code(t):
    if t.dtype == torch.float32:
        return F32
    if t.dtype == torch.bfloat16:
        return BF16
    raise RuntimeError(f"dgv2: unsupported dtype {t.dtype} (float32 / bfloat16 only)")


def check(*tensors):
    for t in tensors:
        if t is None:
            continue
        if not t.is_cuda:
            raise RuntimeError("dgv2: tensor must be a CUDA/HIP tensor (no CPU fallback)")
        if not t.is_contiguous():
            raise RuntimeError("dgv2: tensor must be contiguous")


def ptr(t):
    return None if t is None else t.data_ptr()


def stream():
    return torch.cuda.current_stream().cuda_stream


def ptr_array(tensors):
    return (ctypes.c_void_p * len(tensors))(*[None if t is None else t.data_ptr() for t in tensors])


def addr_array(addrs):
    return (ctypes.c_void_p * len(addrs))(*[None if v is None else int(v) for v in addrs])


def int_array(vals):
    return (ctypes.c_int * len(vals))(*[int(v) for v in vals])


EINVAL = -1
ENOTSUP = -3


def call(name, *args):
    rc = getattr(lib, name)(*args)
    if rc != 0:
        raise RuntimeError(f"{name} failed with code {rc}")


def try_call(name, *args):
    rc = getattr(lib, name)(*args)
    if rc == ENOTSUP:
        return False
    if rc != 0:
        raise RuntimeError(f"{name} failed with code {rc}")
    return True


_scratch_memo = {}


def scratch_elems(entry, *args):
    key = (entry, tuple(tuple(a) if isinstance(a, (list, tuple)) else a for a in args))
    n = _scratch_memo.get(key)
    if n is None:
        out = ctypes.c_int64(0)
        rc = getattr(lib, entry)(ctypes.addressof(out), *[int_array(a) if isinstance(a, tuple) else a for a in key[1]])
        if rc not in (0, ENOTSUP):
            raise RuntimeError(f"{entry} failed with code {rc}")
        n = _scratch_memo[key] = 0 if rc else out.value
    return n


SUMSQ_PARTS = 64
SGD_N_MAX = 2147483647 - (1 << 17)
STATUS_X_INEXACT, STATUS_FIR_TABLE = 1, 2
_STATUS_TEXT = {
    STATUS_X_INEXACT: "a launch with an x_exact promise (fp32 conv on conv_x3.hip / its weight gradient: 'these input "
                      "channels hold bf16-representable values') staged a value that is not: that launch computed on the "
                      "bf16 rounding of its input",
    STATUS_FIR_TABLE: "dgv2_fir_same_mfma_prep met a table entry outside its contract: the band operands are unusable",
}
_status_words = {}


def status_word(device=None):
    idx = torch.cuda.current_device() if device is None else torch.device(device).index
    idx = torch.cuda.current_device() if idx is None else idx
    w = _status_words.get(idx)
    if w is None:
        if torch.cuda.is_current_stream_capturing():
            raise RuntimeError("dgv2: the status word must exist before a hipGraph capture (call dgv2_native.status_word() "
                               "once outside the capture; gans.trainer.Trainer does)")
# ... 19 lines not shown
```

### dusty-gan-v2_amd/gans/models/dusty_v2.py

```python
import math
import os

import numpy as np
import torch
import torch.nn as nn
import torch.nn.functional as F
from torch.nn.modules.utils import _pair

from . import base, dusty_v1, ops
from .ops import native
from .ops.fourier import _CONST_CACHE

LOW = torch.bfloat16


class MappingNetwork(nn.Sequential):

    def __init__(self, in_ch, out_ch, depth=2):
        self.in_ch, self.out_ch, self.depth = in_ch, out_ch, depth
        layers = [ops.PixelNorm()]
        ch = in_ch
        for _ in range(depth):
            layers.append(nn.Sequential(
                ops.EqualLR(nn.Linear(ch, out_ch), gain=math.sqrt(2), lr_mul=0.01),
# ... 483 lines not shown
        v = v * self.synthesis_network.output_scale
        image_orig, logit = torch.tanh(v[:, :1]), v[:, 1:2]
        soft = torch.sigmoid((logit + u.log() - (-u).log1p()) / mm.gumbel_sigmoid.temperature)
        mask = ((soft > 0.5).to(soft.dtype) - soft).detach() + soft
        image = image_orig + (1.0 - mask) * (mm.const_host - image_orig)
        return {"image": image, "raydrop_logit": logit, "w": w, "raydrop_mask": mask, "image_orig": image_orig}

    def __init__(self, mapping_kwargs, synthesis_kwargs, measurement_kwargs):
        super().__init__(
            mapping_network=MappingNetwork(**mapping_kwargs),
            synthesis_network=SynthesisNetwork(**synthesis_kwargs),
            measurement_model=dusty_v1.RayDropModel(**measurement_kwargs),
        )

    def forward_synthesis(self, w, angle=None):
        angle = self.angle if angle is None else angle
        return self.synthesis_network(w, angle)

    def forward(self, z, angle=None, style_mixing=False, truncation_psi=1.0, input_w=False, noise=None,
                second_order=False):
        mm = self.measurement_model
        if len(mm.gumbel_sigmoid._forward_hooks) > 0:
            return super().forward(z, angle, style_mixing, truncation_psi, input_w)
        low = all(getattr(m, "use_fp16", False) for m in self.synthesis_network.layers)
        with native.glin_grad(low and not second_order):
            w = z if input_w else self.forward_mapping(z, style_mixing)
            assert w.ndim == 3
            if self.training:
                self.moving_average_w(w)
            else:
                w = self.truncation_trick(w, truncation_psi)
            angle = self.angle if angle is None else angle
            noise = noise or {}
            skip, shift = self.synthesis_network.synthesize(w, angle, noise.get("shifts", "auto"), composable=second_order)
        B, H, W, _ = skip.shape
        u = noise.get("gumbel_u")
        u = native.gumbel_uniform((B, 1, H, W), skip.device) if u is None else u.float().contiguous()
        if second_order:
            return self._output_stage_composable(skip, shift, u, w)
        image, image_orig, logit, mask = native.gen_tail(
            skip, shift, u, self.synthesis_network.output_scale, mm.const_host,
            mm.gumbel_sigmoid.temperature)
        return {"image": image, "raydrop_logit": logit, "w": w, "raydrop_mask": mask, "image_orig": image_orig}


def _ring_shift(v, shift_rad):
    B, C, H, W = v.shape
    pos = torch.arange(W, dtype=torch.float32, device=v.device)[None, :] + (shift_rad / (2 * math.pi))[:, None] * W
    j0 = pos.floor()
    f = (pos - j0)[:, None, None, :]
    j0 = j0.long()
    i0 = (j0 % W)[:, None, None, :].expand(B, C, H, W)
    i1 = ((j0 + 1) % W)[:, None, None, :].expand(B, C, H, W)
    return v.gather(3, i0) * (1 - f) + v.gather(3, i1) * f


class ResidualBlock(nn.Module):

    def __init__(self, in_ch: int, out_ch: int):
        super().__init__()
        kw = dict(bias=False, ring=True, equal_lr=True)
        self.conv1 = ops.Conv2d(in_ch, in_ch, 3, 1, 1, **kw)
        self.bias_act1 = ops.FusedLeakyReLU(in_ch)
        self.resample = ops.Resample(window=[1, 3, 3, 1], ring=True)
        self.conv2 = ops.Conv2d(in_ch, out_ch, 3, 2, 1, **kw)
        self.bias_act2 = ops.FusedLeakyReLU(out_ch)
        self.skip = ops.Conv2d(in_ch, out_ch, 1, 2, 0, **kw)
        self.blur_down = native.ResampleSpec([1, 3, 3, 1], down=(2, 2), ring=True, pads=(2, 1))
        self.skip_geom = native.ConvGeom(1, 1, 1, 0, True)

    def bank_entries(self, vec):
        c = 1.0 / math.sqrt(2)
        fused = self.skip.in_ch % vec == 0 and self.skip._params_bias()[0] is None
        return [(self.conv1, self.conv1.bank_entry()), (self.conv2, self.conv2.bank_entry()),
                (self.skip, self.skip.bank_entry(wscale=c if fused else None))]

    def fp8_entries(self, vec):
        if self.conv2.in_ch % 64 or self.conv2.out_ch < 64 or self.skip.in_ch % vec or self.skip._params_bias()[0] is not None:
            return []
        c = 1.0 / math.sqrt(2)
        return [(self.conv2, self.conv2.bank_entry()[:2]), (self.skip, self.skip.bank_entry(wscale=c)[:2])]

    def _forward_fp8(self, x, bank, fp8):
        spec = self.resample.spec
        if x.requires_grad:
            hd_h, hd8, x = self.conv1.forward_cl(x, act=self.bias_act1, bank=bank, fork=True, down=spec, q8=True)
        else:
            hd_h, hd8 = self.conv1.forward_cl(x, act=self.bias_act1, bank=bank, down=spec, q8=True)
        c = 1.0 / math.sqrt(2)
        xs = native.resample_q8(x, self.blur_down)
        h = self.conv2.forward_cl((hd_h, hd8), act=self.bias_act2, act_scale=self.bias_act2.scale * c, bank=bank,
                                  fp8=fp8[self.conv2])
        return self.skip.forward_cl(xs, geom=self.skip_geom, resid=h, wscale=c, bank=bank, fp8=fp8[self.skip])

    def forward_cl(self, x, bank=None, fp8=None, xs=None):
        if (xs is None and fp8 is not None and self.conv2 in fp8 and bank is not None and bank.get(self.conv1) is not None
                and isinstance(self.resample, ops.Resample) and native.fp8_ok(x, self.conv2.out_ch)):
            return self._forward_fp8(x, bank, fp8)
        hd = None
        if bank is not None and bank.get(self.conv1) is not None and isinstance(self.resample, ops.Resample):
            if x.requires_grad and xs is None:
                hd, x = self.conv1.forward_cl(x, act=self.bias_act1, bank=bank, fork=True, down=self.resample.spec)
            else:
                hd = self.conv1.forward_cl(x, act=self.bias_act1, bank=bank, down=self.resample.spec)
        else:
            h = self.conv1.forward_cl(x, act=self.bias_act1, bank=bank)
        c = 1.0 / math.sqrt(2)
        if xs is None:
            xs = native.resample(x, self.blur_down)
        if native.conv_resid_ok(xs, self.skip_geom) and self.skip._params_bias()[0] is None:
            h = self.conv2.forward_cl(self.resample.forward_cl(h) if hd is None else hd, act=self.bias_act2,
                                      act_scale=self.bias_act2.scale * c, bank=bank)
            return self.skip.forward_cl(xs, geom=self.skip_geom, resid=h, wscale=c, bank=bank)
        h = self.conv2.forward_cl(self.resample.forward_cl(h) if hd is None else hd, act=self.bias_act2, bank=bank)
        s = self.skip.forward_cl(xs, geom=self.skip_geom, bank=bank)
        return (h + s) * c

    def forward(self, x):
        return ops.from_cl(self.forward_cl(ops.to_cl(x)))


class Discriminator(nn.Module):

    def __init__(self, in_ch: int, ch_base: int = 32, ch_max: int = 512, mbdis_group: int = 4, mbdis_feat: int = 1,
                 resolution=(64, 512), ring=True, num_fp16_layers=-1, pre_blur=True):
        super().__init__()
        res_in = _pair(256 if resolution is None else resolution)
        n_down = int(np.log2(min(res_in) / 4))
        res_out = tuple(map(lambda x: x >> n_down, res_in))

        def ch(i):
            return min(ch_base << i, ch_max)

        kw = dict(bias=False, ring=ring, equal_lr=True)
        self.num_fp16_layers = num_fp16_layers
        self.epilogue_dtype = os.environ.get("DGV2_D_EPILOGUE", "fp32")
        self.fp8_branches = os.environ.get("DGV2_FP8", "0") == "1"
        c_in = in_ch * 2 if pre_blur else in_ch
        layers = [ops.BlurVH(ring=ring)] if pre_blur else []
        layers += [ops.Conv2d(c_in, ch(0), 1, 1, 0, **kw)]
        layers += [ops.FusedLeakyReLU(ch(0))]
        layers += [ResidualBlock(ch(i), ch(i + 1)) for i in range(n_down)]
        self.layers = nn.Sequential(*layers)
        self.epilogue = nn.Sequential(
            ops.MinibatchStdDev(group=mbdis_group, features=mbdis_feat),
            ops.Conv2d(ch(4) + mbdis_feat, ch(4), 3, 1, 1, **kw),
            ops.FusedLeakyReLU(ch(4)),
            nn.Flatten(),
            ops.EqualLR(nn.Linear(ch(4) * int(np.prod(res_out)), ch(4), bias=False)),
            ops.FusedLeakyReLU(ch(4)),
            ops.EqualLR(nn.Linear(ch(4), 1)),
        )

    def _weight_bank(self):
        if self.num_fp16_layers not in (-1, 0):
            return None
        dt = LOW if self.num_fp16_layers == -1 else torch.float32
        vec = 32 if dt == LOW else 16
        items = []
        for layer in self.layers:
            if isinstance(layer, ResidualBlock):
                items += layer.bank_entries(vec)
        mb, conv = self.epilogue[0], self.epilogue[1]
        cin = conv.in_ch
        edt = self._epilogue_dtype()
        evec = 32 if edt == LOW else 16
        epi = (conv, conv.bank_entry(pad_in_to=(cin + evec - 1) // evec * evec))
        if edt == dt:
            items.append(epi)
        if len(items) > 32:
            return None
        prepared = native.conv_weight_bank([e for _, e in items], dt,
                                           image8=[dt == LOW and (True if m.geom.stride == 1 else "fwd") for m, _ in items])
        bank = {m: native.PreparedConv(e[1], e[2], *images) for (m, e), images in zip(items, prepared)}
        if edt != dt:
            images, = native.conv_weight_bank([epi[1]], edt, image8=[True])
            bank[conv] = native.PreparedConv(epi[1][1], epi[1][2], *images)
        return bank

    def _fp8_bank(self):
        items = []
        for layer in self.layers:
            if isinstance(layer, ResidualBlock):
                items += layer.fp8_entries(32)
        if not items or len(items) > 16:
            return None
        prepared = native.fp8_quant_weights([e for _, e in items])
        return {m: wd for (m, _), wd in zip(items, prepared)}

    def _epilogue_dtype(self):
        if self.epilogue_dtype not in ("fp32", "bf16"):
            raise ValueError(f"epilogue_dtype must be 'fp32' or 'bf16', got {self.epilogue_dtype!r}")
        return LOW if (self.epilogue_dtype == "bf16" and self.num_fp16_layers == -1) else torch.float32

    def _fused_stem(self, h, layers, down=None):
        blur, conv, act = layers[0], layers[1], layers[2]
        w, b, _ = conv._params()
        low = self.num_fp16_layers > 1 or self.num_fp16_layers == -1
        return native.stem(h, w, act.bias, blur.blur_h.spec.ring, act.negative_slope, act.scale,
                           LOW if low else torch.float32, down=down)

    _cut = None

    def head_parameters(self):
        return [p for m in self.epilogue[4:] for p in m.parameters()]

    def take_cut(self):
        cut, self._cut = self._cut, None
        return cut

    _bank_keep = None

    def forward(self, h, splits=1, double_backward=False, features_only=False, cut=False, reuse_bank=False):
        layers = list(self.layers)
        i = 0
        keep = self._bank_keep if (reuse_bank and not double_backward and h.is_cuda) else None
        if keep is not None and keep[0] == (self.num_fp16_layers, self._epilogue_dtype(), self.fp8_branches):
            bank, fp8 = keep[1], keep[2]
        else:
            r1_bank = double_backward and _R1_BANK and self.num_fp16_layers == -1
            bank = None if ((double_backward and not r1_bank) or not h.is_cuda) else self._weight_bank()
            fp8 = self._fp8_bank() if (bank is not None and self.fp8_branches and self.num_fp16_layers == -1) else None
            if bank is not None:
                self._bank_keep = ((self.num_fp16_layers, self._epilogue_dtype(), self.fp8_branches), bank, fp8)
        fused = (not double_backward and h.is_cuda and h.shape[1] == 1 and len(layers) > 3
                 and isinstance(layers[0], ops.BlurVH) and isinstance(layers[1], ops.Conv2d)
                 and isinstance(layers[2], ops.FusedLeakyReLU) and layers[2].bias is not None
                 and layers[1]._params_bias()[0] is None and tuple(layers[1].raw_weight().shape[1:]) == (2, 1, 1)
                 and layers[1].raw_weight().shape[0] in (8, 16, 32, 64))
        xs0 = None
        if fused:
            blk0 = layers[3] if len(layers) > 3 and isinstance(layers[3], ResidualBlock) else None
            want = (blk0 is not None and _STEM_SKIP and torch.is_grad_enabled() and fp8 is None
                    and (self.num_fp16_layers == -1 or self.num_fp16_layers == 0))
            x = self._fused_stem(h, layers, down=blk0.blur_down if want else None)
            if want:
                x, xs0 = x
            i = 3
        else:
            x = ops.to_cl(h.float())
        while i < len(layers):
            low = (self.num_fp16_layers > i) or (self.num_fp16_layers == -1)
            x = x.to(LOW if low else torch.float32)
            layer = layers[i]
            nxt = layers[i + 1] if i + 1 < len(layers) else None
            if isinstance(layer, ops.Conv2d) and isinstance(nxt, ops.FusedLeakyReLU):
                x = layer.forward_cl(x, act=nxt)
                i += 2
            elif isinstance(layer, ResidualBlock):
                x = layer.forward_cl(x, bank=bank, fp8=fp8, xs=xs0)
                xs0 = None
                i += 1
            else:
                x = layer.forward_cl(x)
                i += 1
        if features_only:
            return x
        mb, conv, act1, _, lin1, act2, lin2 = self.epilogue
        edt = self._epilogue_dtype()
        trunk_low, n_trunk = x.dtype == LOW, int(x.shape[3])
        cin = x.shape[3] + mb.features
        vec = 32 if edt == LOW else 16
        cpad = (cin + vec - 1) // vec * vec
        if (not double_backward and cpad > x.shape[3]
                and native.mbstd_cat_ok(x, mb.group, splits, mb.features, cpad, out_dtype=edt)):
            x = native.mbstd_cat(x, mb.group, splits, cpad, out_dtype=edt)
        else:
            x = mb.forward_cl(x.to(edt).float(), pad_to=cpad, splits=splits).to(edt)
        if edt == torch.float32 and trunk_low and x.dtype == torch.float32:
            x._dgv2_exact = n_trunk
        x = conv.forward_cl(x, pad_in_to=cpad, act=act1, bank=bank)
        x = native.flatten_nchw(x) if (x.is_cuda and not double_backward) else ops.from_cl(x).flatten(1)
        if cut:
            leaf = x.detach().requires_grad_(True)
            self._cut = (x, leaf)
            x = leaf
        if edt == LOW and lin1.module.bias is None and lin1.gain_ == 1.0:
            x = native.linear_low(x, lin1.module.weight, lin1.scale) if x.is_cuda else \
                F.linear(x, lin1.module.weight.to(LOW)).float() * lin1.scale
        elif x.is_cuda and lin1.module.bias is None and lin1.gain_ == 1.0 and x.shape[1] >= 8192:
            x = native.linear_f32(x.float(), lin1.module.weight, lin1.scale)
        else:
            x = lin1(x.float())
        if not double_backward and native.d_tail_ok(x, act2, lin2):
            return native.d_tail(x, act2, lin2)
        x = act2.forward_cl(x)
        return lin2(x)
```

### dusty-gan-v2_amd/gans/models/ops/native/conv.py

```python
import contextlib
import ctypes as _ct
import os
from typing import NamedTuple, Optional

import torch
from torch.autograd import Function

import dgv2_native as N
from . import act_resample
from .act_resample import ResampleSpec, _BiasActBackward, _Resample, _dt, _resample_raw, want_param_grad
from .fp8 import _conv_fwd_fp8, _handle, _resample_q8_raw, fp8_dequant
from .modgemm import _values


class ConvGeom:
    def __init__(self, kh, kw, stride, pad, ring):
        self.kh, self.kw, self.stride, self.pad, self.ring = kh, kw, stride, pad, int(bool(ring))

    def out_hw(self, H, W):
        return (H + 2 * self.pad - self.kh) // self.stride + 1, (W + 2 * self.pad - self.kw) // self.stride + 1

    @property
    def ring3x3(self):
        return bool(self.ring) and (self.kh, self.kw, self.pad) == (3, 3, 1)
# ... 91 lines not shown
    gx = torch.empty(xshape, device=gy.device, dtype=gy.dtype)
    ok = N.try_call("dgv2_conv3x3_dgrad8", N.ptr(gx), N.ptr(gy), N.ptr(w8t), B, H, W, C, gy.shape[3], N.ptr(resid), _dt(gy),
                    N.stream())
    return gx if ok else None


def _conv_dgrad_direct(gy, wt3, g, xshape, resid=None):
    B, H, W, C = xshape
    gx = torch.empty(xshape, device=gy.device, dtype=gy.dtype)
    if (g.stride == 2 and resid is None and _S2D8 and gy.dtype == torch.bfloat16 and g.ring and C % 128 == 0
            and wt3.is_contiguous()
            and N.try_call("dgv2_conv3x3_s2_dgrad8", N.ptr(gx), N.ptr(gy), N.ptr(wt3), B, H // 2, W // 2, C, gy.shape[3],
                           _dt(gy), N.stream())):
        return gx
    if N.try_call("dgv2_conv_direct_dgrad", N.ptr(gx), N.ptr(gy), N.ptr(wt3), B, H, W, C, gy.shape[3], g.kh, g.stride,
                  N.ptr(resid), _dt(gy), N.stream()):
        return gx
    if resid is None:
        raise RuntimeError("dgv2_conv_direct_dgrad refused a call without a residual")
    return _conv_dgrad_direct(gy, wt3, g, xshape) + resid


def _conv_dgrad_raw(gy, w, g, xshape, wt=None, resid=None, w8t=None):
    B, H, W, C = xshape
    O = gy.shape[3]
    if (w8t is not None and _CONV8_IMG and gy.dtype == torch.bfloat16 and g.ring3x3 and g.stride == 1
            and w8t.dtype == gy.dtype):
        N.check(gy, w8t, resid)
        gx = _conv_dgrad8(gy, w8t, xshape, resid)
        if gx is not None:
            return gx
    if (w8t is not None and _CONV_X3 and gy.dtype == torch.float32 and w8t.dtype == torch.bfloat16 and wt is not None
            and g.ring3x3 and g.stride == 1 and getattr(w8t, "_dgv2_clive", None)):
        clive = w8t._dgv2_clive
        N.check(gy, w8t, wt, resid)
        gx = torch.empty(xshape, device=gy.device, dtype=gy.dtype)
        if N.try_call("dgv2_conv3x3_x3_dgrad", N.ptr(gx), N.ptr(gy), N.ptr(w8t), N.ptr(wt), B, H, W, int(clive), C, O,
                      N.ptr(resid), N.stream()):
            return gx
    if wt is None:
        c = getattr(w, "_dgv2_vals_t", None)
        if c is not None and c[0] == w._version:
            wt = c[1]
        else:
            wt = w.permute(3, 1, 2, 0).contiguous()
            w._dgv2_vals_t = (w._version, wt)
    N.check(gy, wt, resid)
    if (w is not None and _X3_AUTO[0] and gy.dtype == torch.float32 and g.ring3x3 and g.stride == 1
            and W % 32 == 0 and H >= 2 and C % 64 <= 16):
        w3t = _x3_auto_images(w, False)
        if w3t is not None:
            gx = torch.empty(xshape, device=gy.device, dtype=gy.dtype)
            if N.try_call("dgv2_conv3x3_x3_dgrad", N.ptr(gx), N.ptr(gy), N.ptr(w3t), N.ptr(wt), B, H, W,
                          int(_X3_AUTO[1].get(C, C)), C, O, N.ptr(resid), N.stream()):
                return gx
    if _is_1x1(g) and gy.is_contiguous():
        gx = torch.empty(xshape, device=gy.device, dtype=gy.dtype)
        if _conv1x1("dgv2_conv1x1_dgrad", gx, gy, wt, B, H * W, C, O, resid):
            return gx
    even = g.stride == 1 or (H % 2 == 0 and W % 2 == 0)
    if _direct_ok(g, O % _kstep(gy) == 0) and even and not (g.kh == 1 and g.stride == 2):
        return _conv_dgrad_direct(gy, wt.reshape(C, g.kh * g.kw, O), g, xshape, resid)
    if resid is not None:
        return _conv_dgrad_raw(gy, w, g, xshape, wt) + resid
    gx = torch.empty(xshape, device=gy.device, dtype=gy.dtype)
    scratch = None
    if g.pad > 0:
        scratch = torch.empty((B, H + 2 * g.pad, W + 2 * g.pad, C), device=gy.device, dtype=gy.dtype)
    N.call("dgv2_conv_dgrad", N.ptr(gx), N.ptr(scratch), N.ptr(gy), N.ptr(wt), B, H, W, C, O, g.kh, g.kw, g.stride,
           g.pad, g.ring, _dt(gy), N.stream())
    return gx


_WGRAD_DIRECT_MAXC = int(os.environ.get("DGV2_WGRAD_DIRECT_MAXC", "64"))


_WGRAD_STREAM = os.environ.get("DGV2_NO_WGRAD_STREAM") is None


_TN_STREAM = os.environ.get("DGV2_NO_TN_STREAM") is None


_LIB_WGRAD = os.environ.get("DGV2_NO_LIB_WGRAD") is None


def _bmm_tn_small(gy, x, B, P, I, O, batch_sum=False):
    lanes = 256 // max(I * x.element_size() // 16, 1)
    ns = 1
    while B * ns < 1024 and P % (2 * ns) == 0 and P // (2 * ns) >= lanes * 16:
        ns *= 2
    parts = torch.empty((B, ns, O, I), device=x.device, dtype=torch.float32)
    if not N.try_call("dgv2_bmm_tn_small", N.ptr(parts), N.ptr(gy), N.ptr(x), B * ns, P // ns, I, O, _dt(x), N.stream()):
        return None
    if batch_sum:
        return parts.sum(dim=(0, 1))
    return parts.view(B, O, I) if ns == 1 else parts.sum(dim=1)


def _conv_wgrad_raw(gy, x, g, gscale=None, x3=None, xexact=0, out=None):
    B, H, W, C = x.shape
    O = gy.shape[3]
    N.check(gy, x)
    if x3 is None and _X3_AUTO[0]:
        x3 = int(_X3_AUTO[1].get(C, C))
    if (x3 and _CONV_X3 and x.dtype == torch.float32 and g.ring3x3 and g.stride == 1
            and O % 128 == 0 and C >= 64 and C % 8 == 0 and W % 32 == 0 and 0 <= x3 - C // 64 * 64 <= 16):
        scratch = torch.empty(N.scratch_elems("dgv2_conv3x3_x3_wgrad_scratch", B, H, W, C, int(x3), O), device=x.device,
                              dtype=torch.float32)
        gw3 = (out if (out is not None and gscale is not None and tuple(out.shape) == (O, C, 3, 3)) else
               torch.empty((O, C, 3, 3) if gscale is not None else (O, 3, 3, C), device=x.device, dtype=torch.float32))
        if N.try_call("dgv2_conv3x3_x3_wgrad", N.ptr(gw3), N.ptr(scratch), scratch.numel(), N.ptr(gy), N.ptr(x), B, H, W, C,
                      int(x3), min(int(xexact), C), O, 1.0 if gscale is None else float(gscale), int(gscale is not None),
                      N.ptr(N.status_word(x.device)), N.stream()):
            return gw3 if gscale is None else gw3.permute(0, 2, 3, 1)
    stream_ok = (_WGRAD_STREAM and g.kh == g.kw and (g.kh, g.pad) in ((3, 1), (1, 0)) and g.stride in (1, 2)
                 and C % (16 // x.element_size()) == 0 and O % (16 // x.element_size()) == 0)
    if gscale is not None:
        if not stream_ok:
            gp = _conv_wgrad_raw(gy, x, g).permute(0, 3, 1, 2)
            return torch.mul(gp, gscale, out=torch.empty(gp.shape, device=x.device)).permute(0, 2, 3, 1)
        gw = (out if (out is not None and tuple(out.shape) == (O, C, g.kh, g.kw)) else
              torch.empty((O, C, g.kh, g.kw), device=x.device, dtype=torch.float32))
    else:
        gw = torch.empty((O, g.kh, g.kw, C), device=x.device, dtype=torch.float32)
    if stream_ok:
        scratch = torch.empty(N.scratch_elems("dgv2_conv_wgrad_stream_scratch", B, H, W, C, O, g.kh, g.stride, g.pad, _dt(x)),
                              device=x.device, dtype=torch.float32)
        N.call("dgv2_conv_wgrad_stream_pl", N.ptr(gw), N.ptr(scratch), scratch.numel(), N.ptr(gy), N.ptr(x), B, H, W,
               C, O, g.kh, g.stride, g.pad, g.ring, 1.0 if gscale is None else float(gscale), int(gscale is not None),
               _dt(x), N.stream())
        return gw if gscale is None else gw.permute(0, 2, 3, 1)
    small = C % 32 == 0 and C <= _WGRAD_DIRECT_MAXC and O % 8 == 0 and g.kh == g.kw and (g.kh, g.pad) in ((3, 1), (1, 0))
    if small and g.stride in (1, 2) and (x.dtype == torch.bfloat16 or g.stride == 1):
        N.call("dgv2_conv_wgrad_direct", N.ptr(gw), N.ptr(gy), N.ptr(x), B, H, W, C, O, g.kh, g.stride, g.pad,
               g.ring, _dt(x), N.stream())
        return gw
    if g.kh == 1 and g.kw == 1 and g.stride == 1 and g.pad == 0 and C <= 4 and gy.dtype == x.dtype:
        per = _bmm_tn_small(x, gy, B, H * W, O, C, batch_sum=True)
        if per is not None:
            gw.copy_(per.t().reshape(O, 1, 1, C))
            return gw
    N.call("dgv2_conv_wgrad", N.ptr(gw), N.ptr(gy), N.ptr(x), B, H, W, C, O, g.kh, g.kw, g.stride, g.pad, g.ring,
           _dt(x), N.stream())
    return gw


class PreparedConv(NamedTuple):
    scale: float
    cpad: int
    wf: torch.Tensor
    wt: torch.Tensor
    w8: Optional[torch.Tensor] = None
    w8t: Optional[torch.Tensor] = None


class ConvEpilogue(NamedTuple):
    geom: ConvGeom
    act: Optional[tuple] = None
    down: Optional[ResampleSpec] = None
    fork: bool = False
    q8: bool = False
    x_exact: int = 0
    resid: bool = False
    fp8: Optional[tuple] = None

    @property
    def first_order(self):
        return self.fork or self.down is not None or self.fp8 is not None


def _weights(ctx, w, dtype):
    rec, gscale = getattr(w, "_dgv2_bank", (None, None))
    if rec is None or rec.wf.dtype != dtype:
        ctx.bank = (None, None, gscale)
        return _values(w, dtype).reshape(w.shape), None
    ctx.bank = (rec.wt, rec.w8t, gscale)
    return rec.wf.reshape(w.shape), rec.w8


def _dgrad(gy, w, g, xshape, wt=None, resid=None, gscale=None, w8t=None):
    return _ConvDgrad.apply(gy, w, g, xshape, wt, resid, gscale, w8t)


class _ConvDgrad(Function):

    @staticmethod
    def forward(ctx, gy, w, g, xshape, wt, resid, gscale=None, w8t=None):
        gy = gy.contiguous()
        ctx.save_for_backward(gy, w)
        ctx.g, ctx.gscale = g, gscale
        if resid is not None:
            resid = resid.contiguous().to(gy.dtype)
        if wt is not None and wt.dtype == gy.dtype:
            return _conv_dgrad_raw(gy, None, g, xshape, wt=wt, resid=resid, w8t=w8t)
        wc = _values(w, gy.dtype)
        return _conv_dgrad_raw(gy, wc, g, xshape, resid=resid)

    @staticmethod
    def backward(ctx, ggx):
        gy, w = ctx.saved_tensors
        g_gy = conv_ring(ggx, w, ctx.g) if ctx.needs_input_grad[0] else None
        g_w = _ConvWgrad.apply(gy, ggx, ctx.g, ctx.gscale) if ctx.needs_input_grad[1] else None
        return g_gy, g_w, None, None, None, (ggx if ctx.needs_input_grad[5] else None), None, None


def _wgrad_out(w, gscale):
    if gscale is None or torch.is_grad_enabled():
        return None
    base = getattr(w, "_base", None)
    out = getattr(base, "_dgv2_grad_out", None) if base is not None else None
    if out is None or out.data_ptr() % 16 or out.dtype != torch.float32 or tuple(out.shape) != tuple(base.shape):
        return None
    return out.view_as(out)


class _ConvWgrad(Function):
    @staticmethod
    def forward(ctx, gy, x, g, gscale=None, x3=None, xexact=0, out=None):
        gy = gy.contiguous()
        x = x.contiguous()
        ctx.save_for_backward(gy, x)
        ctx.g, ctx.gscale = g, gscale
        return _conv_wgrad_raw(gy.to(x.dtype), x, g, gscale, x3, xexact, out)

    @staticmethod
    def backward(ctx, ggw):
        if ctx.gscale is not None:
            ggw = ggw * ctx.gscale
        gy, x = ctx.saved_tensors
        g_gy = conv_ring(x, ggw, ctx.g) if ctx.needs_input_grad[0] else None
        g_x = _dgrad(gy, ggw, ctx.g, tuple(x.shape)) if ctx.needs_input_grad[1] else None
        return g_gy, g_x, None, None, None, None, None


class _LinearLow(Function):

    @staticmethod
    def forward(ctx, x, weight, scale):
        x16 = x.to(torch.bfloat16).contiguous()
        w16 = weight.detach().to(torch.bfloat16)
        Bn, K = x16.shape
        O = w16.shape[0]
        S = 32
        if K % (S * 8) == 0 and K >= 8192:
            kc = K // S
            part = torch.bmm(x16.view(Bn, S, kc).transpose(0, 1), w16.view(O, S, kc).permute(1, 2, 0),
                             out_dtype=torch.float32)
            y = part.sum(0)
        else:
            y = torch.mm(x16, w16.t(), out_dtype=torch.float32)
        y.mul_(scale)
        ctx.save_for_backward(x, weight, w16)
        ctx.scale = scale
        return y

    @staticmethod
    def backward(ctx, gy):
        x, weight, w16 = ctx.saved_tensors
        if torch.is_grad_enabled():
            g16 = (gy * ctx.scale).to(torch.bfloat16)
            return g16 @ weight.to(torch.bfloat16), (g16.t() @ x.to(torch.bfloat16)).float(), None
        g16 = torch.mul(gy, ctx.scale).to(torch.bfloat16)
        gx = torch.mm(g16, w16) if ctx.needs_input_grad[0] else None
        gw = None
        if ctx.needs_input_grad[1]:
            x16 = x.to(torch.bfloat16).contiguous()
            Bn, K = x16.shape
            O = w16.shape[0]
            if K % 8 == 0 and O % 8 == 0:
                gw = torch.empty((O, K), device=x.device, dtype=torch.float32)
                N.check(g16, x16)
                N.call("dgv2_bmm_tn", N.ptr(gw), N.ptr(g16), N.ptr(x16), 1, Bn, K, O, O, K, N.BF16, N.stream())
            else:
                gw = torch.mm(g16.t(), x16, out_dtype=torch.float32)
        return gx, gw, None


def linear_low(x, weight, scale):
    return _LinearLow.apply(x, weight, float(scale))


_X3 = os.environ.get("DGV2_NO_GEMM_X3") is None


def gemm_x3(a, b, a_trans, b_trans, I, J, T, scale=1.0, splits=1, out=None):
    if out is None:
        out = torch.empty((I, J), device=a.device, dtype=torch.float32)
    scratch = torch.empty(splits * I * J, device=a.device, dtype=torch.float32) if splits > 1 else None
    N.check(a, b, out)
    ok = N.try_call("dgv2_gemm_x3", N.ptr(out), N.ptr(scratch), 0 if scratch is None else scratch.numel(), N.ptr(a),
                    N.ptr(b), I, J, T, int(a_trans), int(b_trans), a.shape[1], b.shape[1], J, splits, float(scale),
                    N.stream())
    return out if ok else None


def _x3_ok(*ts):
    return _X3 and all(t.dtype == torch.float32 and t.is_cuda for t in ts)


class _LinearF32(Function):

    @staticmethod
    def forward(ctx, x, weight, scale):
        ctx.set_materialize_grads(False)
        x = x.contiguous()
        w = weight.detach()
# ... 45 lines not shown
        if gx is None:
            gx = torch.mm(g * scale, w)
        ctx.save_for_backward(g, weight)
        ctx.scale = scale
        return gx

    @staticmethod
    def backward(ctx, ggx):
        if ggx is None:
            return None, None, None
        g, weight = ctx.saved_tensors
        g_g = _LinearF32.apply(ggx, weight, ctx.scale) if ctx.needs_input_grad[0] else None
        g_w = _LinearF32Wgrad.apply(g, ggx, ctx.scale, None) if ctx.needs_input_grad[1] else None
        return g_g, g_w, None


class _LinearF32Wgrad(Function):

    @staticmethod
    def forward(ctx, g, x, scale, out):
        ctx.set_materialize_grads(False)
        g, x = g.contiguous(), x.contiguous()
        M, O = g.shape
        K = x.shape[1]
        gw = gemm_x3(g, x, True, True, O, K, M, scale=scale, out=out) if _x3_ok(g, x) else None
        if gw is None:
            gw = torch.mm((g * scale).t(), x)
        ctx.save_for_backward(g, x)
        ctx.scale = scale
        return gw

    @staticmethod
    def backward(ctx, ggw):
        if ggw is None:
            return None, None, None, None
        g, x = ctx.saved_tensors
        g_g = _LinearF32.apply(x, ggw, ctx.scale) if ctx.needs_input_grad[0] else None
        g_x = _LinearF32Dgrad.apply(g, ggw, ctx.scale) if ctx.needs_input_grad[1] else None
        return g_g, g_x, None, None


def linear_f32(x, weight, scale):
    return _LinearF32.apply(x, weight, float(scale))


class _DTail(Function):

    @staticmethod
    def forward(ctx, h, b1, w2, b2, cfg):
        ctx.set_materialize_grads(False)
        h = h.contiguous()
        B, K = h.shape
        y = torch.empty((B, 1), device=h.device, dtype=torch.float32)
        a = torch.empty_like(h)
        w2c = w2.detach().reshape(-1).contiguous()
        N.check(h, b1, w2c, b2)
        N.call("dgv2_d_tail_fwd", N.ptr(y), N.ptr(a), N.ptr(h), N.ptr(None if b1 is None else b1.detach()), N.ptr(w2c),
               N.ptr(None if b2 is None else b2.detach()), B, K, *cfg, N.stream())
        ctx.save_for_backward(a, w2, b1, b2)
        ctx.cfg = cfg
        return y

    @staticmethod
    def backward(ctx, gy):
        if gy is None:
            return None, None, None, None, None
        a, w2, b1, b2 = ctx.saved_tensors
        alpha, act_scale, scale2, gain2 = ctx.cfg
        B, K = a.shape
        if torch.is_grad_enabled():
            c = gain2 * scale2
            ga = gy.reshape(B, 1) * (c * w2.reshape(1, K))
            gh = ga * torch.where(a > 0, act_scale, alpha * act_scale)
            return (gh, gh.sum(0) if b1 is not None else None, (c * (gy.reshape(B, 1) * a).sum(0)).reshape(w2.shape),
                    (gain2 * gy.sum()).reshape(b2.shape) if b2 is not None else None, None)
        gy = gy.contiguous().float()
        gh = torch.empty_like(a)
        dev = a.device
        gb1 = torch.empty(K, device=dev, dtype=torch.float32) if (b1 is not None and want_param_grad(ctx, 1)) else None
        gw2 = torch.empty(K, device=dev, dtype=torch.float32) if want_param_grad(ctx, 2) else None
        gb2 = torch.empty(1, device=dev, dtype=torch.float32) if (b2 is not None and want_param_grad(ctx, 3)) else None
        w2c = w2.detach().reshape(-1).contiguous()
        N.check(gy, a, w2c)
        N.call("dgv2_d_tail_bwd", N.ptr(gh), N.ptr(gb1), N.ptr(gw2), N.ptr(gb2), N.ptr(gy), N.ptr(a), N.ptr(w2c), B, K,
               alpha, act_scale, scale2, gain2, N.stream())
        return (gh if ctx.needs_input_grad[0] else None, gb1, None if gw2 is None else gw2.reshape(w2.shape),
                None if gb2 is None else gb2.reshape(b2.shape), None)


_D_TAIL = os.environ.get("DGV2_NO_D_TAIL") is None


def d_tail_ok(x, act, lin):
    m = lin.module
    return bool(_D_TAIL and x.is_cuda and x.ndim == 2 and x.dtype == torch.float32 and isinstance(m, torch.nn.Linear)
                and m.out_features == 1 and m.in_features == x.shape[1] and m.weight.dtype == torch.float32
                and (act.bias is None or (act.bias.dtype == torch.float32 and act.bias.numel() == x.shape[1])))


def d_tail(x, act, lin):
    cfg = (float(act.negative_slope), float(act.scale), float(lin.scale), float(lin.gain_))
    return _DTail.apply(x, act.bias, lin.module.weight, lin.module.bias, cfg)


class _MbstdCat(Function):

    @staticmethod
    def forward(ctx, x, group, splits, cpad, out_dtype):
        x = x.contiguous()
        N.check(x)
        B, H, W, C = x.shape
        out_dtype = x.dtype if out_dtype is None else out_dtype
        out = torch.empty((B, H, W, cpad), device=x.device, dtype=out_dtype)
        scratch = torch.empty(64 * max(1, B // group), device=x.device, dtype=torch.float32)
        N.call("dgv2_mbstd_cat_fwd_x", N.ptr(out), N.ptr(scratch), N.ptr(x), B, H * W, C, cpad, splits, group, _dt(x),
               _dt(out), N.stream())
        ctx.save_for_backward(x)
        ctx.cfg = (group, splits, cpad, out_dtype)
        return out

    @staticmethod
    def backward(ctx, g):
        (x,) = ctx.saved_tensors
        group, splits, cpad, out_dtype = ctx.cfg
        B, H, W, C = x.shape
        if torch.is_grad_enabled():
            m = B // (splits * group)
            xf, gf = x.float(), g.float()
            y = xf.reshape(splits, group, m, H, W, C)
            d = y - y.mean(1, keepdim=True)
            sd = torch.sqrt((d * d).mean(1, keepdim=True) + 1e-8)
            gst = gf[..., C].reshape(splits, group, m, H * W).sum(dim=(1, 3))
            term = gst[:, None, :, None, None, None] / float(H * W * C) * d / (group * sd)
            return (gf[..., :C] + term.reshape(B, H, W, C)).to(x.dtype), None, None, None, None
        g = g.contiguous().to(out_dtype)
        gx = torch.empty_like(x)
        N.call("dgv2_mbstd_cat_bwd_x", N.ptr(gx), N.ptr(g), N.ptr(x), B, H * W, C, cpad, splits, group, _dt(x), _dt(g),
               N.stream())
        return gx, None, None, None, None


def mbstd_cat_ok(x, group, splits, features, cpad, out_dtype=None):
    vn = 8 if x.dtype == torch.bfloat16 else 4
    B, C = x.shape[0], x.shape[3]
    g = min(B // splits, group)
    mixed_ok = out_dtype in (None, x.dtype) or (x.dtype == torch.bfloat16 and out_dtype == torch.float32)
    return (x.is_cuda and features == 1 and x.dtype in (torch.bfloat16, torch.float32) and C % vn == 0 and cpad % vn == 0
            and cpad > C and 1 <= g <= 8 and B % (splits * g) == 0 and mixed_ok)


def mbstd_cat(x, group, splits, cpad, out_dtype=None):
    g = min(x.shape[0] // splits, group)
    return _MbstdCat.apply(x, g, splits, cpad, out_dtype)


class _FlattenNCHW(Function):

    @staticmethod
    def forward(ctx, x):
        x = x.contiguous()
        B, H, W, C = x.shape
        out = torch.empty((B, C * H * W), device=x.device, dtype=x.dtype)
        N.check(x)
        N.call("dgv2_transpose_list", N.ptr_array([out]), N.ptr_array([x]), N.int_array([H * W]), N.int_array([C]),
               N.int_array([C]), 1, B, x.element_size(), N.stream())
        ctx.shape = (B, H, W, C)
        return out

    @staticmethod
    def backward(ctx, g):
        B, H, W, C = ctx.shape
        if torch.is_grad_enabled():
            return g.reshape(B, C, H, W).permute(0, 2, 3, 1).contiguous()
        g = g.contiguous()
        gx = torch.empty((B, H, W, C), device=g.device, dtype=g.dtype)
        N.call("dgv2_transpose_list", N.ptr_array([gx]), N.ptr_array([g]), N.int_array([C]), N.int_array([H * W]),
               N.int_array([H * W]), 1, B, g.element_size(), N.stream())
        return gx


def flatten_nchw(x):
    return _FlattenNCHW.apply(x)


class _ScaledHandle(Function):

    @staticmethod
    def forward(ctx, param, scale, cpad):
        ctx.scale, ctx.C = scale, param.shape[1]
        O, C, kh, kw = param.shape
        return torch.empty((O, kh, kw, max(C, cpad)), device=param.device, dtype=param.dtype)

    @staticmethod
    def backward(ctx, g):
        gp = g[..., :ctx.C].permute(0, 3, 1, 2)
        out = torch.empty(gp.shape, device=g.device, dtype=g.dtype)
        return torch.mul(gp, ctx.scale, out=out), None, None


def scaled_handle(param, scale, cpad=0, bank=None):
    h = _ScaledHandle.apply(param, float(scale), int(cpad))
    h._dgv2_bank = (bank, None)
    return h


def conv8t_image_ok(p, cpad, dtype):
    return (dtype == torch.bfloat16 and tuple(p.shape[2:]) == (3, 3) and cpad % 64 == 0 and p.shape[0] % 32 == 0
            and p.shape[0] >= 64)


def conv8_image_ok(p, cpad, dtype):
    return (dtype == torch.bfloat16 and tuple(p.shape[2:]) == (3, 3) and p.shape[0] % 64 == 0 and cpad % 32 == 0
            and cpad >= 64)


def convx3_image_ok(p, cpad, dtype):
    return (dtype == torch.float32 and _CONV_X3 and tuple(p.shape[2:]) == (3, 3) and p.shape[0] % 64 == 0 and cpad % 8 == 0
            and cpad >= 64)


def convx3t_image_ok(p, cpad, dtype):
    return (dtype == torch.float32 and _CONV_X3 and tuple(p.shape[2:]) == (3, 3) and p.shape[0] % 32 == 0 and p.shape[0] >= 64
            and cpad >= 64 and p.shape[1] % 64 <= 4 and p.shape[1] // 64 == cpad // 64)


def conv_weight_bank(entries, dtype, image8=None):
    L = len(entries)
    dev = entries[0][0].device
    dims = [(p.shape[0], p.shape[1], int(cp), p.shape[2] * p.shape[3]) for p, _, cp in entries]
    sizes = [o * kk * cp for o, _, cp, kk in dims]
    flat_f = torch.empty(sum(sizes), device=dev, dtype=dtype)
    flat_t = torch.empty(sum(sizes), device=dev, dtype=dtype)
    x3 = dtype == torch.float32
    flags = image8 if image8 is not None else [False] * L
    want = [bool(f) and (convx3_image_ok if x3 else conv8_image_ok)(p, cp, dtype) for f, (p, _, cp) in zip(flags, entries)]
    want_t = [f is True and (convx3t_image_ok if x3 else conv8t_image_ok)(p, cp, dtype) for f, (p, _, cp) in zip(flags, entries)]
    if x3:
        n8 = [3 * (o // 64) * ((cp + 31) // 32) * 2304 * 8 for o, _, cp, _ in dims]
        n8t = [3 * (cp // 64) * (o // 32) * 2304 * 8 for o, _, cp, _ in dims]
    else:
        n8 = n8t = sizes
    idt = torch.bfloat16 if x3 else dtype
    flat_8 = torch.empty(sum(n for n, f in zip(n8, want) if f), device=dev, dtype=idt) if any(want) else None
    flat_8t = torch.empty(sum(n for n, f in zip(n8t, want_t) if f), device=dev, dtype=idt) if any(want_t) else None
    wfs, wts, w8s, w8ts, off, off8, off8t = [], [], [], [], 0, 0, 0
    for (o, c, cp, kk), n, m8, m8t, f, ft in zip(dims, sizes, n8, n8t, want, want_t):
        wfs.append(flat_f[off:off + n].view(o, kk, cp))
        wts.append(flat_t[off:off + n].view(cp, kk, o))
        w8s.append(flat_8[off8:off8 + m8] if f else None)
        w8ts.append(flat_8t[off8t:off8t + m8t] if ft else None)
        if ft and x3:
            w8ts[-1]._dgv2_clive = int(c)
        off += n
        off8 += m8 if f else 0
        off8t += m8t if ft else 0
    srcs = [p.detach() for p, _, _ in entries]
    N.check(*srcs)
    rest = (N.ptr_array(srcs), N.int_array([d[0] for d in dims]), N.int_array([d[1] for d in dims]),
            N.int_array([d[2] for d in dims]), N.int_array([d[3] for d in dims]),
            (_ct.c_float * L)(*[float(s) for _, s, _ in entries]), L, N.dtype_code(flat_f), N.stream())
    images = (None, None) if image8 is None else (N.ptr_array(w8s), N.ptr_array(w8ts))
    N.call("dgv2_conv_weight_bank_ex", N.ptr_array(wfs), N.ptr_array(wts), *images, *rest)
    return list(zip(wfs, wts)) if image8 is None else list(zip(wfs, wts, w8s, w8ts))


_FUSED_ACTBWD = os.environ.get("DGV2_NO_FUSED_ACTBWD") is None


def _resample_actbwd(g, out, spec, in_hw, alpha, scale):
    if not _FUSED_ACTBWD or g.dtype != out.dtype:
        return None
    B, H, W, C = out.shape
    Ho, Wo = spec.out_size(H, W)
    (ih_idx, ih_coef, ih_cnt, Eh), (iw_idx, iw_coef, iw_cnt, Ew) = spec.tables(H, W, True, g.device)
    tabs = (N.ptr(ih_idx), N.ptr(ih_coef), N.ptr(ih_cnt), Eh, N.ptr(iw_idx), N.ptr(iw_coef), N.ptr(iw_cnt), Ew)
    bands = None
    if act_resample._FIR_MFMA and g.dtype == torch.bfloat16 and (Ho, Wo) == (H, W) and C % 32 == 0:
        bands = spec.bands(H, W, True, g.device)
    mfma = bands is not None
    entry = "dgv2_fir_same_mfma_actbwd" if mfma else "dgv2_resample_tab_actbwd"
    tabs = (N.ptr(bands),) if mfma else tabs
    geo = (B, C, H, W) if mfma else (B, C, Ho, Wo, H, W)
    tail = (alpha, scale) if mfma else (alpha, scale, _dt(g))
    if mfma:
        need = N.scratch_elems(entry + "_scratch", B, C, H, W)
    else:
        need = N.scratch_elems(entry + "_scratch", B, C, H, W, Eh, _dt(g)) if Ew <= 4 else 0
    if need == 0:
        return None
    g = g.contiguous()
    N.check(g, out)
    gpre = torch.empty_like(out)
    gb = torch.empty(C, device=g.device, dtype=torch.float32)
    scratch = torch.empty(need, device=g.device, dtype=torch.float32)
    N.call(entry, N.ptr(gpre), N.ptr(gb), N.ptr(scratch), scratch.numel(), N.ptr(g), N.ptr(out), *tabs, *geo, *tail, N.stream())
    return gpre, gb


class _Conv(Function):

    @staticmethod
    def forward(ctx, x, w, bias, resid, x8, ep):
        ctx.set_materialize_grads(False)
        assert (ep.act is not None) == (bias is not None) and ep.resid == (resid is not None) and not (ep.act and ep.resid)
        assert ep.act is not None or (ep.down is None and not ep.fork), "blur/down and fork belong to the activation's forms"
        assert ep.fp8 is None or (ep.down is None and not ep.fork), "an e4m3 input has no blur/down or fork form"
        alpha, scale = ep.act or (0.2, 1.0)
        act = 0 if ep.act is None else 3
        if bias is not None:
            ctx.size_b = bias.numel()
            bias = bias.detach().float().contiguous()
        if resid is not None:
            resid = resid.contiguous()
        if ep.fp8 is not None:
            _weights(ctx, w, torch.bfloat16)
            x = x8
            out = _conv_fwd_fp8(x8, ep.fp8[0], ep.fp8[1], ep.geom, bias, act, alpha, scale, resid)
        else:
            x = x.contiguous()
            wc, w8 = _weights(ctx, w, x.dtype)
            out = _conv_fwd_raw(x, wc, ep.geom, bias, act, alpha, scale, resid, w8, ep.x_exact)
        ctx.save_for_backward(x, w, *(() if ep.act is None else (out,)))
        ctx.ep = ep
        if ep.down is None:
            y = (out,)
        elif ep.q8:
            y8 = _resample_q8_raw(out, ep.down, tuple(out.shape[1:3]))
            if y8 is None:
                raise RuntimeError("dgv2: no e4m3 resampling kernel covers this shape (check native.fp8_ok first)")
            ctx.mark_non_differentiable(y8)
            y = (_handle(y8.shape, x.device), y8)
        else:
            y = (_resample_raw(out, ep.down, False, tuple(out.shape[1:3])),)
        if ep.fork:
            y += (x.view_as(x),)
        return y if len(y) > 1 else y[0]

    @staticmethod
    def backward(ctx, gy, *rest):
        ep = ctx.ep
        gx_sibling = rest[-1] if ep.fork else None
        if gy is None:
            return gx_sibling, None, None, None, None, None
        x, w, *out = ctx.saved_tensors
        want_gw = ctx.needs_input_grad[1] if ep.first_order else want_param_grad(ctx, 1)
        gb = None
        if ep.act is not None:
            out, (alpha, scale) = out[0], ep.act
            fused = None
            if ep.down is not None:
                in_hw = tuple(out.shape[1:3])
                if not torch.is_grad_enabled():
                    fused = _resample_actbwd(gy.to(out.dtype), out, ep.down, in_hw, alpha, scale)
                if fused is None:
                    gy = _Resample.apply(gy, ep.down, True, in_hw)
            want_gb = ep.first_order or want_param_grad(ctx, 2)
            gy, gb = fused or _BiasActBackward.apply(gy, out, want_gb, alpha, scale, 1, ctx.size_b)
        wt, w8t, gscale = ctx.bank
        gx, gw = gx_sibling, None
        if ep.fp8 is not None:
            if ep.resid:
                gy = gy.contiguous()
            if ctx.needs_input_grad[0]:
                gx = _dgrad(gy, w, ep.geom, tuple(x.shape), wt, None, gscale)
            if want_gw:
                gw = _ConvWgrad.apply(gy, fp8_dequant(x), ep.geom, gscale)
        else:
            if ctx.needs_input_grad[0]:
                gx = _dgrad(gy, w, ep.geom, tuple(x.shape), wt, gx_sibling, gscale, w8t)
            if want_gw:
                x3 = None
                if gy.dtype == torch.float32 and w8t is not None and w8t.dtype == torch.bfloat16:
                    x3 = getattr(w8t, "_dgv2_clive", None)
                gw = _ConvWgrad.apply(gy, x, ep.geom, gscale, x3, ep.x_exact, _wgrad_out(w, gscale))
        return gx, gw, gb, (gy if ep.resid and ctx.needs_input_grad[3] else None), None, None


def conv_ring_ep(x, w, ep, bias=None, resid=None):
    x, x8 = x if ep.fp8 is not None else (x, None)
    return _Conv.apply(x, w, bias, resid, x8, ep)


def conv_ring(x, w, geom):
    return conv_ring_ep(x, w, ConvEpilogue(geom))


def conv_resid_ok(x, geom):
    return _direct_ok(geom, x.shape[3] % _kstep(x) == 0)


__all__ = ["ConvGeom", "x3_auto", "PreparedConv", "ConvEpilogue", "linear_low", "gemm_x3", "linear_f32", "d_tail_ok",
           "d_tail", "mbstd_cat_ok", "mbstd_cat", "flatten_nchw", "scaled_handle", "conv8t_image_ok", "conv8_image_ok",
           "convx3_image_ok", "convx3t_image_ok", "conv_weight_bank", "conv_ring_ep", "conv_ring", "conv_resid_ok",
           "_conv_fwd_raw", "_conv_dgrad_direct", "_conv_dgrad_raw", "_bmm_tn_small", "_conv_wgrad_raw",
           "_resample_actbwd", "_Conv"]
```

### include/dgv2.h

```cpp
#ifndef DGV2_H
#define DGV2_H

#include <stdint.h>

#ifdef __cplusplus
extern "C" {
#endif

#define DGV2_F32 0
#define DGV2_BF16 1
#define DGV2_FP8 2
#define DGV2_F16 3
#define DGV2_EINVAL (-1)
#define DGV2_ENOTSUP (-3)

#define DGV2_STATUS_X_INEXACT 1
#define DGV2_STATUS_FIR_TABLE 2

int dgv2_abi_version(void);


int dgv2_fused_bias_act(void* y, const void* x, const void* bias, const void* ref,
                        int64_t size_x, int64_t step_b, int64_t size_b,
                        int act, int grad, float alpha, float scale, int dtype, void* stream);

int dgv2_bias_grad(float* gb, const void* x, int64_t size_x, int64_t step_b, int64_t size_b,
                   int dtype, void* stream);

int dgv2_bias_act_bwd_rs(void* gx, float* gb, const void* gy, const void* ref, int64_t rows, int C,
                         float alpha, float scale, const float* row_scale, float* scratch,
                         int64_t scratch_elems, int dtype, void* stream);
int dgv2_scale_cast(void* y, const void* x, const float* row_scale, int64_t n, int C, int xdtype, int ydtype,
                    void* stream);

int dgv2_upfirdn2d(void* out, const void* in, const float* kernel,
                   int major, int in_h, int in_w, int minor, int kh, int kw,
                   int up_x, int up_y, int down_x, int down_y,
                   int pad_x0, int pad_x1, int pad_y0, int pad_y1, int dtype, void* stream);

int dgv2_resample(void* y, const void* x, const float* taps_h, const float* taps_w,
                  int B, int H, int W, int C, int Ho, int Wo, int ldx, int ldy,
                  int kh, int up_h, int down_h, int p0_h,
                  int kw, int up_w, int down_w, int p0_w,
                  int ring, int adjoint, int dtype, void* stream);

int dgv2_resample_tab_sq(void* y, const void* x, const int* idx_h, const float* coef_h, const int* cnt_h,
                         int Eh, const int* idx_w, const float* coef_w, const int* cnt_w, int Ew,
                         int B, int C, int ldx, int ldy, int in_h, int in_w, int out_h, int out_w,
                         int dtype, float* sumsq, int sumsq_cap, int* sumsq_used, void* stream);

int dgv2_resample_tab_add_affine(void* y, const void* x, const void* resid, const float* rscale, const float* rbias,
                                 const int* idx_h, const float* coef_h, const int* cnt_h, int Eh, const int* idx_w,
                                 const float* coef_w, const int* cnt_w, int Ew, int B, int C, int in_h, int in_w, int out_h,
                                 int out_w, int dtype, void* stream);

int dgv2_resample_tab_actbwd_scratch(int64_t* elems, int B, int C, int out_h, int out_w, int Eh, int dtype);
int dgv2_resample_tab_actbwd(void* y, float* gb, float* scratch, int64_t scratch_elems, const void* x, const void* ref,
                             const int* idx_h, const float* coef_h, const int* cnt_h, int Eh, const int* idx_w,
                             const float* coef_w, const int* cnt_w, int Ew, int B, int C, int in_h, int in_w, int out_h,
                             int out_w, float alpha, float scale, int dtype, void* stream);

int dgv2_fir_same_mfma_prep_scratch(int64_t* bytes, int H, int W);
int dgv2_fir_same_mfma_prep(void* bands, int64_t bands_bytes, const int* idx_h, const float* coef_h, const int* cnt_h,
                            int Eh, const int* idx_w, const float* coef_w, const int* cnt_w, int Ew, int H, int W,
                            int* status, void* stream);
int dgv2_fir_same_mfma(void* y, const void* x, const void* bands, int B, int C, int H, int W, void* stream);
int dgv2_fir_same_mfma_actbwd_scratch(int64_t* elems, int B, int C, int H, int W);
int dgv2_fir_same_mfma_actbwd(void* y, float* gb, float* scratch, int64_t scratch_elems, const void* x, const void* ref,
                              const void* bands, int B, int C, int H, int W, float alpha, float scale, void* stream);

int dgv2_fourier_feature(void* out, const float* angle, const float* shift,
                         const float* freqs, const float* phase,
                         int B, int Ba, int H, int W, int F, int ld, int c0, int dtype, void* stream);

int dgv2_downsample_angle(float* out, const float* in, const float* shift, const float* taps,
                          int B, int Ba, int H, int W, int ring, void* stream);

int dgv2_bmm_tn(float* gw, const void* gy, const void* x, int B, int P, int I, int O,
                int ldgy, int ldx, int dtype, void* stream);

int dgv2_modconv_up_fwd(void* y, const void* t, const void* xs, const void* wimg, int B, int Hout, int Wout, int Hin,
                        int Win, int Ks, int O, const int* idx_h, const float* coef_h, const int* idx_w,
                        const float* coef_w, const float* bias, const float* in_scale, int act, float alpha, float scale,
                        int dtype, float* sumsq, int sumsq_cap, int* sumsq_used, void* stream);
int dgv2_modconv_up_t(void* tcm, void* wimg, const void* h, const void* w, const float* row_scale, float gain, int B,
                      int Hlow, int Wlow, int Ka, int Ks, int O, int I, int koff, int dtype, void* stream);
int dgv2_modconv_up_t_lag(void* tcm, void* wimg, const void* h, const void* w, float gain, const float* ghd,
                          const float* gho, const float* gwd, const float* gwo, int B, int Hlow, int Wlow, int Ka, int Ks,
                          int O, int I, int koff, int dtype, float* sumsq, int sumsq_cap, int* sumsq_used, void* stream);
int dgv2_up2_lag_sumsq(const void* h, const float* ghd, const float* gho, const float* gwd, const float* gwo, int B,
                       int Hin, int Win, int C, int dtype, float* sumsq, int sumsq_cap, int* sumsq_used, void* stream);
int dgv2_bmm_nn_sq(void* y, const void* x, const void* w, int B, int P, int I, int O, int ldx, int ldy,
                   int64_t wstride, const float* row_scale, const float* bias, int act, float alpha, float scale,
                   const void* resid , int dtype, int ydtype,
                   float* sumsq, int sumsq_cap, int* sumsq_used, void* stream);
int dgv2_bmm_nn_cat_sq(void* y, const void* xa, const void* xs, const void* w, int B, int P, int Ka, int Ks,
                       int O, const float* row_scale, const float* bias, int act, float alpha, float scale, int dtype, int ydtype,
                       float* sumsq, int sumsq_cap, int* sumsq_used, void* stream);
int dgv2_bmm_tn_cat(float* gw, const void* gy, const void* xa, const void* xs, int B, int P, int Ka, int Ks,
                    int O, int dtype, void* stream);
int dgv2_bmm_tn_small(float* gw, const void* gy, const void* x, int B, int P, int I, int O, int dtype,
                      void* stream);
int dgv2_bmm_nn_small(void* y, const void* x, const void* w, const void* resid, int B, int P, int O, int K,
                      int dtype, void* stream);
int dgv2_bmm_nn_small_act_scratch(int64_t* elems, int B, int P, int O, int K, int dtype);
int dgv2_bmm_nn_small_act(void* y, const void* x, const void* w, const void* resid, int B, int P, int O, int K,
                          const void* ref, const float* row_scale, float alpha, float ascale, float* gb,
                          float* scratch, int64_t scratch_elems, int dtype, void* stream);
int dgv2_head_bwd_scratch(int64_t* elems, int B, int P, int O, int K, int dtype);
int dgv2_head_bwd(void* y, float* gw, float* gbh, float* gb_up, float* scratch, int64_t scratch_elems, const float* gyf,
                  const float* cvec, const void* w, const void* resid, const void* ref, const float* row_scale, float alpha,
                  float ascale, int B, int P, int O, int K, int dtype, void* stream);

int dgv2_modconv_pe_fwd_sq(void* y, const void* xa, const void* xs, const void* w, int B, int P, int Ka, int Ks,
                           int O, const float* row_scale, const float* bias, int act, float alpha, float scale, int dtype, float* sumsq,
                           int sumsq_cap, int* sumsq_used, void* stream);
int dgv2_modconv_pe_fwd_head(void* y, const void* xa, const void* xs, const void* w, int B, int P, int Ka, int Ks,
                             int O, const float* row_scale, const float* bias, int act, float alpha, float scale, int dtype,
                             float* sumsq, int sumsq_cap, int* sumsq_used, const void* head_w, float* head_out, void* stream);

int dgv2_modconv_pe_dgrad_actbwd_scratch(int64_t* elems, int B, int P, int K, int dtype);
int dgv2_modconv_pe_dgrad_actbwd(void* gpre, float* gb, float* scratch, int64_t scratch_elems, const void* gy,
                                 const void* wt, const void* yref, const float* up_scale, float alpha, float scale, int B,
                                 int P, int K, int dtype, void* stream);

int dgv2_lerp_list(float* const* dst, const float* const* src, const int* n, int L, float weight, void* stream);
int dgv2_adam_prep(float* sc, float* step, float b1, float b2, void* stream);
int dgv2_adam_step(float* const* p, const float* const* g, float* const* m, float* const* v, const int* n,
                   int L, const float* sc, float lr, float b1, float b2, float eps, void* stream);

#define DGV2_SUMSQ_PARTS 64
#define DGV2_SGD_N_MAX (2147483647 - (1 << 17))
int dgv2_sumsq_list(const float* const* g, const int* n, int L, float* partials, void* stream);
int dgv2_clip_prep(const float* partials, int count, float max_norm, float* scale_state, float growth, float backoff,
                   int growth_interval, float* sc, void* stream);
int dgv2_sgd_step(float* const* p, const float* const* g, float* const* m, const int* n, int L, const float* sc, float lr,
                  float momentum, float weight_decay, void* stream);

int dgv2_pack2d(float* packed, const float* const* src, const int* rows, const int* cols, int L, int Rmax,
                int Cmax, void* stream);
int dgv2_unpack2d(float* const* dst, const float* packed, const int* rows, const int* cols, int L, int Rmax,
                  int Cmax, void* stream);

int dgv2_ema_scalar(float* ema, float* snapshot, const float* sumsq, int nsum, float add, float inv_count,
                    float weight, int update, float* cvec, int ncvec, void* stream);
int dgv2_ema_scalar_group(float* const* emas, const int* rows, int n, const float* sumsq, int nsum, float add,
                          float inv_count, float weight, int update, float* cvec, void* stream);
int dgv2_mod_prep_fwd(void* wb, float* dsave, float* stats, const float* W, const float* s,
                      const float* ema_var, const float* shift, const float* fw, int B, int O, int I,
                      int Otot, int row_off, int demod, int cin, int F, int wb_dtype, void* stream);
int dgv2_mod_prep_bwd(float* gW, float* gs, float* corr, const float* G, const float* W, const float* s,
                      const float* stats, const float* dsave, const float* ema_var, const float* shift,
                      const float* fw, int B, int O, int I, int Otot, int row_off, int demod, int cin,
                      int F, int corr_elems, void* stream);

int dgv2_mod_prep_all_fwd(void* const* wb, float* const* dsave, float* stats, float* rot, const float* const* W,
                          const float* const* s, const float* const* fw, const int* O, const int* I,
                          const int* Otot, const int* row_off, const int* cin, const int* flags,
                          const float* shift, int B, int L, void* stream);
int dgv2_mod_prep_all_bwd(float* flat, int64_t flat_elems, float* const* out, const int* ncorr,
                          const float* const* G, const float* const* W, const float* const* s,
                          const float* stats, const float* rot, float* const* dsave,
                          const float* const* fw, const int* O, const int* I, const int* Otot,
                          const int* row_off, const int* cin, const int* flags, const float* shift, int B,
                          int L, float* scratch, int64_t scratch_elems, void* stream);
int dgv2_mod_prep_all_bwd_scratch(int64_t* elems, const int* O, const int* I, int B, int L);

int dgv2_transpose_list(void* const* dst, const void* const* src, const int* rows, const int* cols,
                        const int* ld, int L, int B, int elem_size, void* stream);

int dgv2_sum_squares(float* acc, const void* x, int64_t N, int C, int ld, int dtype, void* stream);

int dgv2_mbstd_cat_fwd_x(void* out, float* scratch, const void* x, int B, int P, int C, int Cp, int splits, int group,
                         int xdtype, int ydtype, void* stream);
int dgv2_mbstd_cat_bwd_x(void* gx, const void* gout, const void* x, int B, int P, int C, int Cp, int splits, int group,
                         int xdtype, int gdtype, void* stream);
int dgv2_gemm_x3(float* c, float* scratch, int64_t scratch_elems, const float* a, const float* b, int I, int J,
                 int64_t T, int a_trans, int b_trans, int64_t lda, int64_t ldb, int64_t ldo, int splits, float scale,
                 void* stream);
int dgv2_pe_wgrad_scratch(int64_t* elems, int B, int P, int O, int Ks);
int dgv2_pe_wgrad(float* gw, float* scratch, int64_t scratch_elems, const void* g, const void* pe, int B, int P, int O,
                  int Ks, int64_t ldo, int col0, void* stream);

int dgv2_conv_fwd(void* y, const void* x, const void* w, int B, int H, int W, int C, int O,
                  int kh, int kw, int stride, int pad, int ring,
                  const float* bias, int act, float alpha, float scale, int dtype, void* stream);
int dgv2_conv_dgrad(void* gx, void* gxp_scratch, const void* gy, const void* wt,
                    int B, int H, int W, int C, int O,
                    int kh, int kw, int stride, int pad, int ring, int dtype, void* stream);
int dgv2_conv_wgrad(float* gw, const void* gy, const void* x, int B, int H, int W, int C, int O,
                    int kh, int kw, int stride, int pad, int ring, int dtype, void* stream);

int dgv2_conv_wgrad_direct(float* gw, const void* gy, const void* x, int B, int H, int W, int C, int O,
                           int k, int stride, int pad, int ring, int dtype, void* stream);

int dgv2_bmm_tn_stream_scratch(int64_t* elems, int B, int H, int W, int C, int O, int dtype);
int dgv2_bmm_tn_stream_ld(float* gw, int64_t ldo, float* scratch, int64_t scratch_elems, const void* gy, const void* x,
                          int x_shared, int B, int H, int W, int C, int O, int dtype, void* stream);

int dgv2_conv_weight_bank_ex(void* const* wf, void* const* wt, void* const* w8, void* const* w8t,
                             const float* const* src, const int* O, const int* C, const int* Cpad, const int* kk,
                             const float* scale, int L, int dtype, void* stream);
int dgv2_conv3x3_fwd8(void* y, const void* x, const void* w8, int B, int Hin, int Win, int Cin, int O, int stride,
                      const float* bias, const void* resid, int act, float alpha, float scale, int dtype, void* stream);
int dgv2_conv3x3_dgrad8(void* gx, const void* gy, const void* w8t, int B, int H, int W, int C, int O, const void* resid,
                        int dtype, void* stream);
int dgv2_conv3x3_s2_dgrad8(void* gx, const void* gy, const void* wt, int B, int Hg, int Wg, int C, int O, int dtype,
                           void* stream);

int dgv2_conv3x3_x3_fwd(void* y, const void* x, const void* w3, int B, int H, int W, int Cx, int x_exact, int O,
                        const float* bias, const void* resid, int act, float alpha, float scale, int* status,
                        void* stream);
int dgv2_conv3x3_x3_dgrad(void* gx, const void* gy, const void* w3t, const void* wt, int B, int H, int W, int C, int ldx,
                          int O, const void* resid, void* stream);
int dgv2_conv3x3_x3_wgrad(float* gw, float* scratch, int64_t scratch_elems, const void* gy, const void* x, int B, int H,
                          int W, int C, int clive, int x_exact, int O, float scale, int param_layout, int* status,
                          void* stream);
int dgv2_conv3x3_x3_wgrad_scratch(int64_t* elems, int B, int H, int W, int C, int clive, int O);
int dgv2_conv_x3_images(void* w3, void* w3t, const void* w, int O, int Cp, void* stream);

int dgv2_conv_wgrad_stream_scratch(int64_t* elems, int B, int H, int W, int C, int O, int k, int stride,
                                   int pad, int dtype);
int dgv2_conv_wgrad_stream_pl(float* gw, float* scratch, int64_t scratch_elems, const void* gy, const void* x,
                              int B, int H, int W, int C, int O, int k, int stride, int pad, int ring,
                              float scale, int param_layout, int dtype, void* stream);

int dgv2_conv_direct_fwd(void* y, const void* x, const void* w, int B, int H, int W, int Cin, int O, int k, int stride,
                         const float* bias, const void* resid, int act, float alpha, float scale, int dtype, void* stream);
int dgv2_conv_direct_dgrad(void* gx, const void* gy, const void* wt, int B, int H, int W, int C, int O, int k, int stride,
                           const void* resid, int dtype, void* stream);

int dgv2_conv1x1_fwd(void* y, const void* x, const void* wf, int B, int P, int C, int O, const void* resid, int dtype,
                     void* stream);
int dgv2_conv1x1_dgrad(void* gx, const void* gy, const void* wt, int B, int P, int C, int O, const void* resid,
                       int dtype, void* stream);

int dgv2_gemm_stream_nn(void* y, const void* x, const void* w, int B, int P, int I, int O, int ldx, int ldy,
                        int64_t wstride, const float* row_scale, const float* bias, int act, float alpha, float scale,
                        const void* resid, int dtype, int ydtype, float* sumsq, int sumsq_cap, int* sumsq_used,
                        void* stream);
int dgv2_gemm_stream_nn_cat(void* y, const void* xa, const void* xs, const void* w, int B, int P, int Ka, int Ks, int O,
                            const float* row_scale, const float* bias, int act, float alpha, float scale, int dtype,
                            int ydtype, float* sumsq, int sumsq_cap, int* sumsq_used, void* stream);
int dgv2_gemm_stream_tn(float* gw, const void* gy, const void* x, int B, int P, int I, int O, int ldgy, int ldx, int dtype,
                        void* stream);
int dgv2_gemm_stream_tn_cat(float* gw, const void* gy, const void* xa, const void* xs, int B, int P, int Ka, int Ks, int O,
                            int dtype, void* stream);

int dgv2_stem_fwd(void* y, const float* x, const float* w, const float* bias, int B, int H, int W, int O,
                  int ring, float alpha, float scale, int ydtype, void* stream);
int dgv2_stem_bwd_scratch(int64_t* elems, int B, int H, int W, int O);
int dgv2_stem_bwd_skip(float* gx, float* gw, float* gb, float* scratch, int64_t scratch_elems, const void* gy, const void* y,
                       const float* x, const float* w, const void* gsk, const int* idx_h, const float* coef_h,
                       const int* cnt_h, int Eh, const int* idx_w, const float* coef_w, const int* cnt_w, int Ew, int Hs,
                       int Ws, int B, int H, int W, int O, int ring, float alpha, float scale, int dtype, void* stream);

int dgv2_gen_tail_fwd(float* image, float* image_orig, float* logit, float* mask,
                      const float* skip, const float* shift, const float* u,
                      int B, int H, int W, float out_scale, float raydrop_const, float temperature,
                      void* stream);
int dgv2_gen_tail_bwd(float* g_skip, float* scratch, const float* g_image, const float* g_image_orig,
                      const float* g_logit, const float* g_mask,
                      const float* image_orig, const float* logit, const float* mask, const float* u,
                      const float* shift, int B, int H, int W, float out_scale, float raydrop_const,
                      float temperature, void* stream);

int dgv2_ada_apply(float* y, const float* x, const float* Ay, const float* kx, const int* off,
                   const int* sgn, const float* a, const float* c, int B, int H, int W, int K,
                   int transpose, void* stream);

int dgv2_ada_sample(float* gaff, float* a, float* c, const float* u, const float* n, const float* p,
                    const float* policy_host, int B, int H, int W, void* stream);
int dgv2_ada_build(float* Ay, float* kx, int* off, int* sgn, const float* gaff, const float* M1y,
                   const float* M1x, const float* taps, int B, int H, int W, int K, void* stream);

int dgv2_ada_sample_img(float* g, float* sigma, float* cut, const float* u2, const float* n2, const float* p,
                        const float* policy_host, int B, void* stream);
int dgv2_ada_fold(float* Ay2, float* kx2, int* off2, float* c2, const float* Ay, const float* kx, const int* off,
                  const int* sgn, const float* c, const float* g, const float* fbank, int B, int H, int W, int K,
                  int NB, int T, void* stream);
int dgv2_ada_apply_img(float* y, const float* x, const float* Ay, const float* kx, const int* off, const int* sgn,
                       const float* a, const float* c, const float* cut, const float* sigma, const float* eps, int B,
                       int H, int W, int K, int transpose, void* stream);

int dgv2_coords_convert(float* out, const float* in, const float* mask, const float* angle,
                        int B, int H, int W, float min_depth, float max_depth, float raydrop_const,
                        int mode, void* stream);

int dgv2_surface_normal(float* out, const float* points, int B, int H, int W, int d, int mode, void* stream);

int dgv2_nsgan_loss(float* stats, float* gy, const float* y, int n_real, int n_fake, float gy_scale, float* sign_cum,
                    float* n_cum, void* stream);

int dgv2_d_tail_fwd(float* y, float* a, const float* h, const float* b1, const float* w2, const float* b2, int B, int K,
                    float alpha, float act_scale, float scale2, float gain2, void* stream);
int dgv2_d_tail_bwd(float* gh, float* gb1, float* gw2, float* gb2, const float* gy, const float* a, const float* w2,
                    int B, int K, float alpha, float act_scale, float scale2, float gain2, void* stream);

int dgv2_colmean_lerp(float* dst, const float* src, int B, int K, int64_t ld, float w, void* stream);

int dgv2_rng_fill(float* const* out, const int64_t* count, const int* kind, const float* a, const float* b, int nseg,
                  uint64_t* state, void* stream);

int dgv2_kitti_rows(int* row, int* counts, const float* pts, int n, int H, void* stream);
int dgv2_kitti_project(float* out, unsigned long long* key, const float* pts, const int* row, int n, int H, int W,
                       int Wout, float min_depth, float max_depth, int apply_mask, void* stream);

int dgv2_fps_scratch(int64_t* floats, int B, int n);
int dgv2_fps(int* idxs, float* temp, const float* xyz, int B, int n, int m, void* stream);
int dgv2_gather_points(float* out, const float* points, const int* idx, int B, int C, int n, int m, void* stream);
int dgv2_gather_points_grad(float* grad_points, const float* grad_out, const int* idx, int B, int C, int n, int m,
                            void* stream);

int dgv2_chamfer_fwd(float* dist1, int* idx1, float* dist2, int* idx2, const float* xyz1, const float* xyz2, int B,
                     int n, int m, void* stream);
int dgv2_nn_search(float* dist, int* idx, const float* xyz, const float* ref, int B, int n, int m, int ref_shared,
                   void* stream);
int dgv2_chamfer_bwd(float* gxyz1, float* gxyz2, const float* xyz1, const float* xyz2, const float* gdist1,
                     const float* gdist2, const int* idx1, const int* idx2, int B, int n, int m, void* stream);

int dgv2_emd_approxmatch(float* match, float* temp, const float* xyz1, const float* xyz2, int B, int n, int m,
                         void* stream);
int dgv2_emd_matchcost(float* cost, const float* match, const float* xyz1, const float* xyz2, int B, int n, int m,
                       void* stream);
int dgv2_emd_matchcost_grad(float* grad1, float* grad2, const float* match, const float* xyz1, const float* xyz2, int B,
                            int n, int m, void* stream);

#define DGV2_EMD_PAIR_MAX_POINTS 4096
int dgv2_emd_pairwise_cost(float* cost, const float* xyz1, const float* xyz2, int B1, int B2, int n, int m,
                           void* stream);

int dgv2_fir_same_mfma_q8(void* y8, const void* x, const void* bands, int B, int C, int H, int W, void* stream);
int dgv2_resample_tab_q8(void* y8, const void* x, const int* idx_h, const float* coef_h, const int* cnt_h, int Eh,
                         const int* idx_w, const float* coef_w, const int* cnt_w, int Ew, int B, int C, int in_h,
                         int in_w, int out_h, int out_w, void* stream);
int dgv2_fp8_quant_weights(void* const* w8, const void* const* src, const int* O, const int* C, const int* kk,
                           const float* eq, int n, float* descale, void* amax, void* stream);
int dgv2_fp8_dequant(void* y, const void* x, int64_t n, float scale, void* stream);
int dgv2_conv_direct_fwd_fp8(void* y, const void* x8, const void* w8, const float* acc_scale, int B, int H, int W, int Cin,
                             int O, int k, int stride, const float* bias, const void* resid, int act, float alpha,
                             float scale, void* stream);

int dgv2_glin_fwd(float* const* y, const float* const* x, const float* const* w, const float* const* bias, const int* N,
                  const int* lda, int L, int B, int K, float alpha, float beta, int act, float slope, int prenorm,
                  float* rnorm, void* stream);
int dgv2_glin_dinput(float* dx, int ldx, float* scratch, int64_t scratch_elems, const float* const* g,
                     const float* const* yact, const float* const* w, const int* N, int L, int B, int K, float alpha,
                     float slope, int accumulate, void* stream);
int dgv2_glin_dweight(float* const* dw, float* const* dbias, const float* const* g, const float* const* yact,
                      const float* const* x, const int* N, const int* ldx, int L, int B, int K, float alpha, float beta,
                      float slope, const float* rnorm, void* stream);

int dgv2_msml_prepare(float* refp, float* maskp, float* normp, float* invm, const float* ref, const float* mask, int B,
                      int C, int H, int W, int L, void* stream);
int dgv2_msml_fwd(float* loss, float* genp, const float* gen, const float* refp, const float* maskp, const float* normp,
                  const float* invm, int B, int C, int H, int W, int L, int metric, int relative, void* stream);
int dgv2_msml_bwd(float* ggen, float* gscratch, const float* gloss, const float* gen, const float* genp,
                  const float* refp, const float* maskp, const float* normp, const float* invm, int B, int C, int H, int W,
                  int L, int metric, int relative, void* stream);
int dgv2_coords_convert_bwd(float* gx, const float* gout, const float* in, const float* mask, const float* angle, int B,
                            int H, int W, float min_depth, float max_depth, int mode, void* stream);
int dgv2_fourier_feature_bwd(float* g_angle, const void* g, const float* angle, const float* shift, const float* freqs,
                             const float* phase, int B, int Ba, int H, int W, int F, int ld, int c0, int dtype,
                             void* stream);

int dgv2_frame_points(float* points, float* colors, const float* image, const float* angle, int B, int H, int W,
                      float min_depth, float max_depth, int border, void* stream);
int dgv2_colorize(float* out, const float* x, const float* lut, int B, int H, int W, int n_colors, void* stream);

int dgv2_crf_rnn_forward(float* out, float* qsave, const float* unary, const float* xyz, const float* mask,
                         const float* kernel_gamma, const float* kernel_alpha, const float* theta_beta,
// ... 38 lines not shown
```

Measured before the change: 5493 range-images/s.

## Fold constant minibatch-stddev channel into D epilogue conv algebraically

```diff
diff --git a/dusty-gan-v2_amd/csrc/conv_wgrad_stream.hip b/dusty-gan-v2_amd/csrc/conv_wgrad_stream.hip
--- a/dusty-gan-v2_amd/csrc/conv_wgrad_stream.hip
+++ b/dusty-gan-v2_amd/csrc/conv_wgrad_stream.hip
@@ -676,7 +676,7 @@
 
 __global__ __launch_bounds__(256) void wgrad_reduce_kernel(float* __restrict__ gw, const float* __restrict__ part,
                                                            int64_t n, int nsplit, float scale = 1.f, int kkC = 0,
-                                                           int Cc = 0, int64_t ldo = 0) {
+                                                           int Cc = 0, int64_t ldo = 0, int Cparam = 0) {
   __shared__ float4 red[16][16];
   const int col = threadIdx.x & 15, sl = threadIdx.x >> 4;
   const int64_t i = ((int64_t)blockIdx.x * 16 + col) * 4;
@@ -713,7 +713,7 @@
         const int64_t o = lin / kkC;
         const int r = (int)(lin - o * kkC);
         const int t = r / Cc, c = r - t * Cc;
-        gw[(o * Cc + c) * kk + t] = v4[e];
+        gw[(o * (Cparam > 0 ? Cparam : Cc) + c) * kk + t] = v4[e];
       }
     }
   }
@@ -945,6 +945,74 @@
   DGV2_RETURN_LAST();
 }
 
+namespace {
+__global__ __launch_bounds__(256) void conv_wgrad_x3_const_kernel(float* __restrict__ gw, float* __restrict__ gb,
+                                                                  const float* __restrict__ st,
+                                                                  const float* __restrict__ gy_sum, int B, int O, int C,
+                                                                  float scale) {
+  const int o = blockIdx.x * 256 + threadIdx.x;
+  if (o >= O) return;
+  float sw = 0.f, sb = 0.f;
+  for (int b = 0; b < B; ++b) {
+    const float g = gy_sum[(int64_t)b * O + o];
+    sw = fmaf(st[b], g, sw);
+    sb += g;
+  }
+  if (gw) {
+    float* w9 = gw + ((int64_t)o * (C + 1) + C) * 9;
+#pragma unroll
+    for (int t = 0; t < 9; ++t) w9[t] = sw * scale;
+  }
+  if (gb) gb[o] = sb;
+}
+}
+
+extern "C" int dgv2_conv3x3_x3_wgrad_cs(float* gw, float* gb, float* scratch, int64_t scratch_elems, const void* gy, const void* x,
+                                        const float* st, const float* gy_sum, int B, int H, int W, int C, int x_exact, int O,
+                                        float scale, int* status, void* stream) {
+  if (!gw || !scratch || !gy || !x || !st || !gy_sum || !aligned16(gy) || !aligned16(x) || !aligned16(scratch))
+    return DGV2_EINVAL;
+  if (B < 1 || H < 1 || W < 1 || C < 1 || O < 1 || x_exact < 0 || x_exact > C) return DGV2_EINVAL;
+  if (x_exact > 0 && !status) return DGV2_EINVAL;
+  static const bool off = getenv("DGV2_NO_CONV_X3") != nullptr || getenv("DGV2_NO_WGRAD_X3") != nullptr;
+  const int ctiles = C / 64;
+  if (off || O % 128 || ctiles < 1 || C % 64 || W % 32) return DGV2_ENOTSUP;
+  if ((int64_t)B * H * W * (C > O ? C : O) >= (1ll << 31)) return DGV2_ENOTSUP;
+  WSPlan p;
+  WSGeom& g = p.g;
+  g = WSGeom{B, H, W, C, O, H, W, 3, 1, 1, 2};
+  g.tiles_h = (H + 3) / 4;
+  g.tiles_w = W / 32;
+  g.ntiles = B * g.tiles_h * g.tiles_w;
+  g.ctiles = ctiles;
+  g.x_shared = 0;
+  g.x_exact = x_exact;
+  g.status = status;
+#ifdef DGV2_ABLATE
+  g.ablate = 0;
+#endif
+  const int pairs = ctiles * (O / 64);
+  int nsplit = 256 / pairs;
+  nsplit = nsplit < 1 ? 1 : (nsplit > g.ntiles ? g.ntiles : nsplit);
+  g.tiles_per_split = (g.ntiles + nsplit - 1) / nsplit;
+  nsplit = (g.ntiles + g.tiles_per_split - 1) / g.tiles_per_split;
+  const int64_t n = (int64_t)O * 9 * C;
+  if (scratch_elems < (int64_t)nsplit * n) return DGV2_ENOTSUP;
+  hipStream_t stm = (hipStream_t)stream;
+  const bool xe = x_exact >= C;
+  auto kern = xe ? conv_wgrad_x3_kernel<true> : conv_wgrad_x3_kernel<false>;
+  static bool attr_set[2] = {false, false};
+  if (!attr_set[xe]) {
+    hipError_t e = hipFuncSetAttribute((const void*)kern, hipFuncAttributeMaxDynamicSharedMemorySize, (int)WXCfg::LDS);
+    if (e != hipSuccess) return (int)e;
+    attr_set[xe] = true;
+  }
+  kern<<<dim3(nsplit, pairs), 256, WXCfg::LDS, stm>>>(scratch, (const float*)gy, (const float*)x, g);
+  wgrad_reduce_kernel<<<(int)((n / 4 + 15) / 16), 256, 0, stm>>>(gw, scratch, n, nsplit, scale, 9 * C, C, 0, C + 1);
+  conv_wgrad_x3_const_kernel<<<(O + 255) / 256, 256, 0, stm>>>(gw, gb, st, gy_sum, B, O, C, scale);
+  DGV2_RETURN_LAST();
+}
+
 extern "C" int dgv2_conv3x3_x3_wgrad_scratch(int64_t* elems, int B, int H, int W, int C, int clive, int O) {
   if (!elems) return DGV2_EINVAL;
   *elems = 0;
diff --git a/dusty-gan-v2_amd/csrc/conv_x3.hip b/dusty-gan-v2_amd/csrc/conv_x3.hip
--- a/dusty-gan-v2_amd/csrc/conv_x3.hip
+++ b/dusty-gan-v2_amd/csrc/conv_x3.hip
@@ -13,6 +13,9 @@
   int* status;
   const float* bias;
   const float* resid;
+  const float* cst;
+  const float* cwsum;
+  int nchw;
   int act;
   float alpha, scale;
 #ifdef DGV2_ABLATE
@@ -338,13 +341,23 @@
       const float4 b4 = *reinterpret_cast<const float4*>(&s_bias[mf * 16 + lc * 4]);
       const float bq[4] = {b4.x, b4.y, b4.z, b4.w};
       float f[4];
+      float cw[4] = {0.f, 0.f, 0.f, 0.f};
+      const float cs = p.cst ? p.cst[b] : 0.f;
+      if (p.cst) {
+        const float4 c4 = *reinterpret_cast<const float4*>(p.cwsum + (o < p.O ? o : 0));
+        cw[0] = c4.x; cw[1] = c4.y; cw[2] = c4.z; cw[3] = c4.w;
+      }
 #pragma unroll
       for (int r = 0; r < 4; ++r) {
-        float t = acc[mf][nf][r] + bq[r];
+        float t = (p.cst ? fmaf(cs, cw[r], acc[mf][nf][r]) : acc[mf][nf][r]) + bq[r];
         if (p.act == 3) t = fmaxf(t, t * p.alpha) * p.scale;
         f[r] = t;
       }
-      if (live && o < p.O) {
+      if (live && o < p.O && p.nchw) {
+        float* yo = y + (((int64_t)b * p.O + o) * p.H + gh) * p.W + gw;
+#pragma unroll
+        for (int r = 0; r < 4; ++r) yo[(int64_t)r * p.H * p.W] = f[r];
+      } else if (live && o < p.O) {
         if (p.resid) {
           const float4 r4 = *reinterpret_cast<const float4*>(p.resid + row + o);
           f[0] += r4.x; f[1] += r4.y; f[2] += r4.z; f[3] += r4.w;
@@ -501,6 +514,28 @@
   p.xexact = x_exact;
   p.status = status;
   p.bias = bias; p.resid = (const float*)resid; p.act = act; p.alpha = alpha; p.scale = scale;
+  p.cst = p.cwsum = nullptr; p.nchw = 0;
+  const int rc = x_exact >= 32 ? launch_x3<0, true>((float*)y, (const float*)x, (const bf16_t*)w3, p, (hipStream_t)stream)
+                               : launch_x3<0, false>((float*)y, (const float*)x, (const bf16_t*)w3, p, (hipStream_t)stream);
+  if (rc) return rc;
+  DGV2_RETURN_LAST();
+}
+
+extern "C" int dgv2_conv3x3_x3_fwd_cs(void* y, const void* x, const void* w3, int B, int H, int W, int Cx, int x_exact, int O,
+                                      const float* bias, const float* st, const float* wsum, int nchw, int act, float alpha,
+                                      float scale, int* status, void* stream) {
+  if (!y || !x || !w3 || B < 1 || H < 1 || W < 1 || Cx < 1 || O < 1 || x_exact < 0 || x_exact > Cx) return DGV2_EINVAL;
+  if ((x_exact > 0 && !status) || (act != 0 && act != 3) || ((st == nullptr) != (wsum == nullptr))) return DGV2_EINVAL;
+  static const bool off = getenv("DGV2_NO_CONV_X3") != nullptr;
+  if (off || W % 32 || Cx % 8 || O % 64 || Cx < 64) return DGV2_ENOTSUP;
+  if (!aligned16(y) || !aligned16(x) || !aligned16(w3) || (wsum && !aligned16(wsum))) return DGV2_ENOTSUP;
+  if ((int64_t)B * H * W * (Cx > O ? Cx : O) >= (1ll << 31)) return DGV2_ENOTSUP;
+  CX3 p;
+  p.B = B; p.H = H; p.W = W; p.Cx = Cx; p.nchunks = (Cx + 31) / 32; p.O = O; p.ldy = O; p.nslab = O / 64;
+  p.xexact = x_exact;
+  p.status = status;
+  p.bias = bias; p.resid = nullptr; p.act = act; p.alpha = alpha; p.scale = scale;
+  p.cst = st; p.cwsum = wsum; p.nchw = nchw != 0;
   const int rc = x_exact >= 32 ? launch_x3<0, true>((float*)y, (const float*)x, (const bf16_t*)w3, p, (hipStream_t)stream)
                                : launch_x3<0, false>((float*)y, (const float*)x, (const bf16_t*)w3, p, (hipStream_t)stream);
   if (rc) return rc;
@@ -521,6 +556,7 @@
   p.xexact = 0;
   p.status = nullptr;
   p.bias = nullptr; p.resid = (const float*)resid; p.act = 0; p.alpha = 0.2f; p.scale = 1.f;
+  p.cst = p.cwsum = nullptr; p.nchw = 0;
   hipStream_t st = (hipStream_t)stream;
   const int rc = launch_x3<1, false>((float*)gx, (const float*)gy, (const bf16_t*)w3t, p, st);
   if (rc) return rc;
diff --git a/dusty-gan-v2_amd/csrc/epilogue_cs.hip b/dusty-gan-v2_amd/csrc/epilogue_cs.hip
--- /dev/null
+++ b/dusty-gan-v2_amd/csrc/epilogue_cs.hip
@@ -0,0 +1,65 @@
+#include "common.h"
+
+namespace {
+
+constexpr int EC_T = 64;
+
+__global__ __launch_bounds__(256) void epilogue_actbwd_t_kernel(float* __restrict__ gy, float* __restrict__ gy_sum,
+                                                                const float* __restrict__ g, const float* __restrict__ out, int O,
+                                                                int P, float alpha, float scale) {
+  __shared__ float tile[EC_T][EC_T + 1];
+  const int b = blockIdx.y, o0 = blockIdx.x * EC_T;
+  const int tid = threadIdx.x;
+  const int lp = tid & 15, lo = tid >> 4;
+  float sum[4] = {0.f, 0.f, 0.f, 0.f};
+  for (int p0 = 0; p0 < P; p0 += EC_T) {
+    const bool in = p0 + lp * 4 < P;
+#pragma unroll
+    for (int j = 0; j < 4; ++j) {
+      const int o = lo + 16 * j;
+      const int64_t at = ((int64_t)b * O + o0 + o) * P + (in ? p0 + lp * 4 : 0);
+      const float4 g4 = *reinterpret_cast<const float4*>(g + at);
+      const float4 f4 = *reinterpret_cast<const float4*>(out + at);
+      float v[4];
+      v[0] = (f4.x > 0.f ? g4.x : g4.x * alpha) * scale;
+      v[1] = (f4.y > 0.f ? g4.y : g4.y * alpha) * scale;
+      v[2] = (f4.z > 0.f ? g4.z : g4.z * alpha) * scale;
+      v[3] = (f4.w > 0.f ? g4.w : g4.w * alpha) * scale;
+      if (in) {
+#pragma unroll
+        for (int e = 0; e < 4; ++e) tile[o][lp * 4 + e] = v[e];
+        sum[j] += (v[0] + v[1]) + (v[2] + v[3]);
+      }
+    }
+    __syncthreads();
+#pragma unroll
+    for (int k = 0; k < 4; ++k) {
+      const int p = lo + 16 * k;
+      if (p0 + p < P) {
+        const float4 w = make_float4(tile[lp * 4][p], tile[lp * 4 + 1][p], tile[lp * 4 + 2][p], tile[lp * 4 + 3][p]);
+        *reinterpret_cast<float4*>(gy + ((int64_t)b * P + p0 + p) * O + o0 + lp * 4) = w;
+      }
+    }
+    __syncthreads();
+  }
+#pragma unroll
+  for (int j = 0; j < 4; ++j) {
+    float s = sum[j];
+    s += __shfl_xor(s, 1);
+    s += __shfl_xor(s, 2);
+    s += __shfl_xor(s, 4);
+    s += __shfl_xor(s, 8);
+    if (lp == 0) gy_sum[(int64_t)b * O + o0 + lo + 16 * j] = s;
+  }
+}
+
+}
+
+extern "C" int dgv2_epilogue_actbwd_t(void* gy, float* gy_sum, const void* g, const void* out, int B, int P, int O, float alpha,
+                                      float scale, void* stream) {
+  if (!gy || !gy_sum || !g || !out || B < 1 || P < 1 || O < 1) return DGV2_EINVAL;
+  if (O % EC_T || P % 4 || B > 65535 || !aligned16(gy) || !aligned16(g) || !aligned16(out)) return DGV2_ENOTSUP;
+  epilogue_actbwd_t_kernel<<<dim3(O / EC_T, B), 256, 0, (hipStream_t)stream>>>((float*)gy, gy_sum, (const float*)g,
+                                                                              (const float*)out, O, P, alpha, scale);
+  DGV2_RETURN_LAST();
+}
diff --git a/dusty-gan-v2_amd/csrc/mbstd.hip b/dusty-gan-v2_amd/csrc/mbstd.hip
--- a/dusty-gan-v2_amd/csrc/mbstd.hip
+++ b/dusty-gan-v2_amd/csrc/mbstd.hip
@@ -101,9 +101,32 @@
   }
 }
 
+template <typename TX, typename TY>
+__global__ __launch_bounds__(256) void mbstd_widen_kernel(TY* __restrict__ out, float* __restrict__ st,
+                                                          const TX* __restrict__ x, const float* __restrict__ partial, MbGeom q) {
+  constexpr int VN = mb_vn<TX, TY>::value;
+  const int64_t total = (int64_t)q.B * q.P * q.C / VN;
+  const int64_t i0 = (int64_t)blockIdx.x * 256 + threadIdx.x;
+  if (i0 < q.B) {
+    const int b = (int)i0;
+    const int sg = b / q.m, mi = b - sg * q.m, s = sg / q.g;
+    float v = 0.f;
+    for (int k = 0; k < q.NS; ++k) v += partial[(s * q.m + mi) * q.NS + k];
+    st[b] = v * (1.f / ((float)q.P * q.C));
+  }
+  for (int64_t i = i0; i < total; i += (int64_t)gridDim.x * 256) {
+    float o[VN];
+    ldN<TX, VN>(x + i * VN, o);
+    stN<TY, VN>(out + i * VN, o);
+  }
+}
+
 template <typename TX, typename TG>
 __global__ __launch_bounds__(256) void mbstd_bwd_kernel(TX* __restrict__ gx, const TG* __restrict__ gout,
-                                                        const TX* __restrict__ x, MbGeom q) {
+                                                        const TX* __restrict__ x, MbGeom q,
+                                                        const float* __restrict__ gy_sum = nullptr,
+                                                        const float* __restrict__ wsum = nullptr, int O = 0,
+                                                        float* __restrict__ gst_out = nullptr) {
   __shared__ float red[16];
   __shared__ float s_gst;
   constexpr int VN = mb_vn<TX, TG>::value;
@@ -111,13 +134,23 @@
   const int s = sm / q.m, mi = sm - s * q.m;
   const int64_t PC = (int64_t)q.P * q.C;
   float part = 0.f;
-  for (int e = threadIdx.x; e < q.g * q.P; e += 256) {
-    const int gi = e / q.P, p = e - gi * q.P;
-    const int b = (s * q.g + gi) * q.m + mi;
-    part += to_f32(gout[((int64_t)b * q.P + p) * q.Cp + q.C]);
+  if (gy_sum) {
+    for (int gi = 0; gi < q.g; ++gi) {
+      const int b = (s * q.g + gi) * q.m + mi;
+      for (int o = threadIdx.x; o < O; o += 256) part = fmaf(wsum[o], gy_sum[(int64_t)b * O + o], part);
+    }
+  } else {
+    for (int e = threadIdx.x; e < q.g * q.P; e += 256) {
+      const int gi = e / q.P, p = e - gi * q.P;
+      const int b = (s * q.g + gi) * q.m + mi;
+      part += to_f32(gout[((int64_t)b * q.P + p) * q.Cp + q.C]);
+    }
   }
   part = block_sum(part, red);
-  if (threadIdx.x == 0) s_gst = part / ((float)q.P * q.C);
+  if (threadIdx.x == 0) {
+    s_gst = part / ((float)q.P * q.C);
+    if (gst_out && split == 0) gst_out[sm] = part;
+  }
   __syncthreads();
   const float k = s_gst / q.g;
   const int cvx = q.C / VN;
@@ -228,3 +261,34 @@
     return DGV2_EINVAL;
   DGV2_RETURN_LAST();
 }
+
+extern "C" int dgv2_mbstd_widen_fwd(void* out, float* st, float* scratch, const void* x, int B, int P, int C, int splits,
+                                    int group, void* stream) {
+  if (!out || !st || !scratch || !x || splits < 1 || group < 1 || B < 1 || B % (splits * group)) return DGV2_EINVAL;
+  MbGeom q{B, P, C, C + 8, splits, group, B / (splits * group), 1};
+  if (!mb_ok(q, 8) || !aligned16(out) || !aligned16(x)) return DGV2_EINVAL;
+  q.Cp = C;
+  q.NS = mb_splits(q, 8);
+  hipStream_t st_ = (hipStream_t)stream;
+  dim3 grid(q.S * q.m, q.NS);
+  mbstd_partial_kernel<bf16_t><<<grid, 256, 0, st_>>>(scratch, (const bf16_t*)x, q);
+  int gc = grid_for((int64_t)B * P * (C / 8), 256, 4096);
+  const int gmin = (B + 255) / 256;
+  gc = gc < gmin ? gmin : gc;
+  mbstd_widen_kernel<bf16_t, float><<<gc, 256, 0, st_>>>((float*)out, st, (const bf16_t*)x, scratch, q);
+  DGV2_RETURN_LAST();
+}
+
+extern "C" int dgv2_mbstd_bwd_cs(void* gx, float* gst, const void* gout, const void* x, const float* gy_sum, const float* wsum,
+                                 int O, int B, int P, int C, int splits, int group, void* stream) {
+  if (!gx || !gout || !x || !gy_sum || !wsum || O < 1 || splits < 1 || group < 1 || B < 1 || B % (splits * group))
+    return DGV2_EINVAL;
+  MbGeom q{B, P, C, C + 8, splits, group, B / (splits * group), 1};
+  if (!mb_ok(q, 8) || !aligned16(gx) || !aligned16(gout) || !aligned16(x)) return DGV2_EINVAL;
+  q.Cp = C;
+  q.NS = mb_splits(q, 8);
+  dim3 grid(q.S * q.m, q.NS);
+  mbstd_bwd_kernel<bf16_t, float><<<grid, 256, 0, (hipStream_t)stream>>>((bf16_t*)gx, (const float*)gout, (const bf16_t*)x, q,
+                                                                        gy_sum, wsum, O, gst);
+  DGV2_RETURN_LAST();
+}
diff --git a/dusty-gan-v2_amd/csrc/weight_bank.hip b/dusty-gan-v2_amd/csrc/weight_bank.hip
--- a/dusty-gan-v2_amd/csrc/weight_bank.hip
+++ b/dusty-gan-v2_amd/csrc/weight_bank.hip
@@ -14,6 +14,8 @@
   void* w8t[WB_MAX];
   int O[WB_MAX], C[WB_MAX], Cpad[WB_MAX], kk[WB_MAX];
   float scale[WB_MAX];
+  int Csrc;
+  float* wsum;
 };
 
 template <typename T>
@@ -47,9 +49,17 @@
   const int o0 = (blockIdx.x / tc) * WB_TO, c0 = (blockIdx.x % tc) * WB_TC;
   const float s = a.scale[l];
   const float* src = a.src[l];
+  const int Cs = a.Csrc > 0 ? a.Csrc : C;
   T* wf = reinterpret_cast<T*>(a.wf[l]);
   T* wt = reinterpret_cast<T*>(a.wt[l]);
   __shared__ float tile[WB_TO][WB_TC * WB_KK + 1];
+  if (KK == 9 && a.wsum && c0 == 0 && threadIdx.x < WB_TO && o0 + (int)threadIdx.x < O) {
+    const float* w9 = src + ((size_t)(o0 + threadIdx.x) * Cs + C) * 9;
+    float v = 0.f;
+#pragma unroll
+    for (int t = 0; t < 9; ++t) v += w9[t] * s;
+    a.wsum[o0 + threadIdx.x] = v;
+  }
   const int run = WB_TC * kk;
   for (int e0 = threadIdx.x; e0 < WB_TO * run; e0 += 256 * 8) {
     float v[8];
@@ -60,7 +70,7 @@
       const int o = ec / run, r = ec - o * run;
       const int c = c0 + r / kk;
       const bool ok = e < WB_TO * run && o0 + o < O && c < C;
-      const size_t idx = ok ? ((size_t)(o0 + o) * C + c0) * kk + r : 0;
+      const size_t idx = ok ? ((size_t)(o0 + o) * Cs + c0) * kk + r : 0;
       v[u] = ok ? src[idx] * s : 0.f;
     }
 #pragma unroll
@@ -162,6 +172,8 @@
                                         const float* scale, int L, int dtype, void* stream) {
   if (!wf || !wt || !src || !O || !C || !Cpad || !kk || !scale || L < 1 || L > WB_MAX) return DGV2_EINVAL;
   BankArgs a;
+  a.Csrc = 0;
+  a.wsum = nullptr;
   for (int l = 0; l < L; ++l) {
     a.w8[l] = w8 ? w8[l] : nullptr;
     a.w8t[l] = w8t ? w8t[l] : nullptr;
@@ -214,3 +226,17 @@
   DGV2_DISPATCH_DTYPE(dtype, { weight_bank_kernel<T><<<grid, 256, 0, st>>>(a); });
   DGV2_RETURN_LAST();
 }
+
+extern "C" int dgv2_conv_weight_bank_cs(void* wf, void* wt, void* w8, void* w8t, float* wsum, const float* src, int O, int C,
+                                        float scale, void* stream) {
+  if (!wf || !wt || !w8 || !w8t || !wsum || !src || O < 64 || O % 64 || C < 64 || C % 64) return DGV2_EINVAL;
+  if ((int64_t)O * 9 * (C + 1) >= (1 << 30)) return DGV2_EINVAL;
+  BankArgs a;
+  a.src[0] = src; a.wf[0] = wf; a.wt[0] = wt; a.w8[0] = w8; a.w8t[0] = w8t;
+  a.O[0] = O; a.C[0] = C; a.Cpad[0] = C; a.kk[0] = 9; a.scale[0] = scale;
+  a.Csrc = C + 1;
+  a.wsum = wsum;
+  dim3 tgrid((C / WB_TC) * (O / WB_TO), 1);
+  weight_bank_tiled_kernel<float, 9><<<tgrid, 256, 0, (hipStream_t)stream>>>(a);
+  DGV2_RETURN_LAST();
+}
diff --git a/dusty-gan-v2_amd/dgv2_native/__init__.py b/dusty-gan-v2_amd/dgv2_native/__init__.py
--- a/dusty-gan-v2_amd/dgv2_native/__init__.py
+++ b/dusty-gan-v2_amd/dgv2_native/__init__.py
@@ -125,6 +125,12 @@
     "dgv2_conv3x3_s2_dgrad8": [_c_ptr] * 3 + [_c_int] * 6 + [_c_ptr],
     "dgv2_conv3x3_x3_wgrad_scratch": [_c_ptr] + [_c_int] * 6,
     "dgv2_conv3x3_x3_wgrad": [_c_ptr, _c_ptr, _c_i64] + [_c_ptr] * 2 + [_c_int] * 7 + [_c_f32, _c_int, _c_ptr, _c_ptr],
+    "dgv2_mbstd_widen_fwd": [_c_ptr] * 4 + [_c_int] * 5 + [_c_ptr],
+    "dgv2_mbstd_bwd_cs": [_c_ptr] * 6 + [_c_int] * 6 + [_c_ptr],
+    "dgv2_conv_weight_bank_cs": [_c_ptr] * 6 + [_c_int, _c_int, _c_f32, _c_ptr],
+    "dgv2_conv3x3_x3_fwd_cs": [_c_ptr] * 3 + [_c_int] * 6 + [_c_ptr] * 3 + [_c_int, _c_int, _c_f32, _c_f32, _c_ptr, _c_ptr],
+    "dgv2_epilogue_actbwd_t": [_c_ptr] * 4 + [_c_int] * 3 + [_c_f32, _c_f32, _c_ptr],
+    "dgv2_conv3x3_x3_wgrad_cs": [_c_ptr] * 3 + [_c_i64] + [_c_ptr] * 4 + [_c_int] * 6 + [_c_f32, _c_ptr, _c_ptr],
     "dgv2_conv_x3_images": [_c_ptr] * 3 + [_c_int] * 2 + [_c_ptr],
     "dgv2_conv3x3_x3_dgrad": [_c_ptr] * 4 + [_c_int] * 6 + [_c_ptr, _c_ptr],
     "dgv2_conv3x3_x3_fwd": [_c_ptr] * 3 + [_c_int] * 6 + [_c_ptr, _c_ptr, _c_int, _c_f32, _c_f32, _c_ptr, _c_ptr],
diff --git a/dusty-gan-v2_amd/gans/models/dusty_v2.py b/dusty-gan-v2_amd/gans/models/dusty_v2.py
--- a/dusty-gan-v2_amd/gans/models/dusty_v2.py
+++ b/dusty-gan-v2_amd/gans/models/dusty_v2.py
@@ -659,7 +659,21 @@
             ops.EqualLR(nn.Linear(ch(4), 1)),
         )
 
-    def _weight_bank(self):
+    def _const_stat(self, double_backward):
+        mb, conv, act1 = self.epilogue[0], self.epilogue[1], self.epilogue[2]
+        p = conv.raw_weight()
+        return bool(native.conv._CONST_STAT and native.conv._CONV_X3 and not double_backward and self.num_fp16_layers == -1
+                    and self._epilogue_dtype() == torch.float32 and mb.features == 1 and conv.geom.ring3x3
+                    and conv.geom.stride == 1 and p.is_cuda and p.shape[1] % 64 == 1 and p.shape[0] % 128 == 0
+                    and conv._params_bias()[0] is None and act1.bias is not None)
+
+    def _epilogue_bank_cat(self):
+        conv = self.epilogue[1]
+        ent = conv.bank_entry(pad_in_to=(conv.in_ch + 15) // 16 * 16)
+        images, = native.conv_weight_bank([ent], torch.float32, image8=[True])
+        return native.PreparedConv(ent[1], ent[2], *images)
+
+    def _weight_bank(self, const_stat=False):
         if self.num_fp16_layers not in (-1, 0):
             return None
         dt = LOW if self.num_fp16_layers == -1 else torch.float32
@@ -680,7 +694,9 @@
         prepared = native.conv_weight_bank([e for _, e in items], dt,
                                            image8=[dt == LOW and (True if m.geom.stride == 1 else "fwd") for m, _ in items])
         bank = {m: native.PreparedConv(e[1], e[2], *images) for (m, e), images in zip(items, prepared)}
-        if edt != dt:
+        if edt != dt and const_stat:
+            bank[conv] = native.conv_weight_bank_cs(epi[1][0], epi[1][1])
+        elif edt != dt:
             images, = native.conv_weight_bank([epi[1]], edt, image8=[True])
             bank[conv] = native.PreparedConv(epi[1][1], epi[1][2], *images)
         return bank
@@ -717,19 +733,21 @@
         return cut
 
     _bank_keep = None
+    epilogue_form = None
 
     def forward(self, h, splits=1, double_backward=False, features_only=False, cut=False, reuse_bank=False):
         layers = list(self.layers)
         i = 0
         keep = self._bank_keep if (reuse_bank and not double_backward and h.is_cuda) else None
-        if keep is not None and keep[0] == (self.num_fp16_layers, self._epilogue_dtype(), self.fp8_branches):
+        cs = h.is_cuda and self._const_stat(double_backward)
+        if keep is not None and keep[0] == (self.num_fp16_layers, self._epilogue_dtype(), self.fp8_branches, cs):
             bank, fp8 = keep[1], keep[2]
         else:
             r1_bank = double_backward and _R1_BANK and self.num_fp16_layers == -1
-            bank = None if ((double_backward and not r1_bank) or not h.is_cuda) else self._weight_bank()
+            bank = None if ((double_backward and not r1_bank) or not h.is_cuda) else self._weight_bank(const_stat=cs)
             fp8 = self._fp8_bank() if (bank is not None and self.fp8_branches and self.num_fp16_layers == -1) else None
             if bank is not None:
-                self._bank_keep = ((self.num_fp16_layers, self._epilogue_dtype(), self.fp8_branches), bank, fp8)
+                self._bank_keep = ((self.num_fp16_layers, self._epilogue_dtype(), self.fp8_branches, cs), bank, fp8)
         fused = (not double_backward and h.is_cuda and h.shape[1] == 1 and len(layers) > 3
                  and isinstance(layers[0], ops.BlurVH) and isinstance(layers[1], ops.Conv2d)
                  and isinstance(layers[2], ops.FusedLeakyReLU) and layers[2].bias is not None
@@ -765,6 +783,17 @@
             return x
         mb, conv, act1, _, lin1, act2, lin2 = self.epilogue
         edt = self._epilogue_dtype()
+        rec = None if bank is None else bank.get(conv)
+        self.epilogue_form = "cat"
+        if rec is not None and rec.wsum is not None:
+            if native.epilogue_const_ok(x.shape, x.dtype, conv.geom, conv.out_ch, mb.features, mb.group, splits, edt,
+                                        double_backward) and rec.cpad == x.shape[3]:
+                p_raw, s_used, _ = conv.bank_entry()
+                x = native.epilogue_const(x, p_raw.permute(0, 2, 3, 1), act1.bias, rec, mb.group, splits,
+                                          (act1.negative_slope, act1.scale))
+                self.epilogue_form = "const_stat"
+                return self._head(x, lin1, act2, lin2, edt, cut, double_backward)
+            bank[conv] = self._epilogue_bank_cat()
         trunk_low, n_trunk = x.dtype == LOW, int(x.shape[3])
         cin = x.shape[3] + mb.features
         vec = 32 if edt == LOW else 16
@@ -778,6 +807,9 @@
             x._dgv2_exact = n_trunk
         x = conv.forward_cl(x, pad_in_to=cpad, act=act1, bank=bank)
         x = native.flatten_nchw(x) if (x.is_cuda and not double_backward) else ops.from_cl(x).flatten(1)
+        return self._head(x, lin1, act2, lin2, edt, cut, double_backward)
+
+    def _head(self, x, lin1, act2, lin2, edt, cut, double_backward):
         if cut:
             leaf = x.detach().requires_grad_(True)
             self._cut = (x, leaf)
diff --git a/dusty-gan-v2_amd/gans/models/ops/native/conv.py b/dusty-gan-v2_amd/gans/models/ops/native/conv.py
--- a/dusty-gan-v2_amd/gans/models/ops/native/conv.py
+++ b/dusty-gan-v2_amd/gans/models/ops/native/conv.py
@@ -267,6 +267,7 @@
     wt: torch.Tensor
     w8: Optional[torch.Tensor] = None
     w8t: Optional[torch.Tensor] = None
+    wsum: Optional[torch.Tensor] = None
 
 
 class ConvEpilogue(NamedTuple):
@@ -618,6 +619,108 @@
 def mbstd_cat(x, group, splits, cpad, out_dtype=None):
     g = min(x.shape[0] // splits, group)
     return _MbstdCat.apply(x, g, splits, cpad, out_dtype)
+
+
+_CONST_STAT = os.environ.get("DGV2_NO_CONST_STAT") is None
+
+
+def epilogue_const_ok(xshape, xdtype, geom, out_ch, features, group, splits, epilogue_dtype=torch.float32,
+                      double_backward=False):
+    if not (_CONST_STAT and _CONV_X3) or double_backward or features != 1:
+        return False
+    if xdtype != torch.bfloat16 or epilogue_dtype != torch.float32:
+        return False
+    if not (geom.ring3x3 and geom.stride == 1):
+        return False
+    B, H, W, C = (int(v) for v in xshape)
+    g = min(B // max(splits, 1), group)
+    return (splits >= 1 and 1 <= g <= 8 and B % (splits * g) == 0 and B <= 65535 and H >= 2 and W % 32 == 0
+            and C >= 64 and C % 64 == 0 and out_ch % 128 == 0 and B * H * W * max(C, out_ch) < 2 ** 31)
+
+
+def conv_weight_bank_cs(param, scale):
+    O, C = int(param.shape[0]), int(param.shape[1]) - 1
+    dev = param.device
+    wf = torch.empty((O, 9, C), device=dev, dtype=torch.float32)
+    wt = torch.empty((C, 9, O), device=dev, dtype=torch.float32)
+    w8 = torch.empty(3 * (O // 64) * (C // 32) * 2304 * 8, device=dev, dtype=torch.bfloat16)
+    w8t = torch.empty(3 * (C // 64) * (O // 32) * 2304 * 8, device=dev, dtype=torch.bfloat16)
+    wsum = torch.empty(O, device=dev, dtype=torch.float32)
+    src = param.detach()
+    N.check(src)
+    N.call("dgv2_conv_weight_bank_cs", N.ptr(wf), N.ptr(wt), N.ptr(w8), N.ptr(w8t), N.ptr(wsum), N.ptr(src), O, C,
+           float(scale), N.stream())
+    return PreparedConv(float(scale), C, wf, wt, w8, w8t, wsum)
+
+
+class _EpilogueConst(Function):
+
+    @staticmethod
+    def forward(ctx, x, w, bias, rec, group, splits, act):
+        ctx.set_materialize_grads(False)
+        x = x.contiguous()
+        B, H, W, C = x.shape
+        O = rec.wf.shape[0]
+        alpha, scale = act
+        g = min(B // splits, group)
+        dev = x.device
+        xw = torch.empty((B, H, W, C), device=dev, dtype=torch.float32)
+        st = torch.empty(B, device=dev, dtype=torch.float32)
+        scratch = torch.empty(64 * max(1, B // g), device=dev, dtype=torch.float32)
+        b = bias.detach().float().contiguous()
+        N.check(x, b)
+        N.call("dgv2_mbstd_widen_fwd", N.ptr(xw), N.ptr(st), N.ptr(scratch), N.ptr(x), B, H * W, C, splits, g, N.stream())
+        y = torch.empty((B, O * H * W), device=dev, dtype=torch.float32)
+        N.call("dgv2_conv3x3_x3_fwd_cs", N.ptr(y), N.ptr(xw), N.ptr(rec.w8), B, H, W, C, C, O, N.ptr(b), N.ptr(st),
+               N.ptr(rec.wsum), 1, 3, alpha, scale, N.ptr(N.status_word(dev)), N.stream())
+        ctx.save_for_backward(x, xw, st, y, w)
+        ctx.rec, ctx.cfg = rec, (g, splits, alpha, scale, tuple(bias.shape))
+        return y
+
+    @staticmethod
+    def backward(ctx, gflat):
+        if gflat is None:
+            return None, None, None, None, None, None, None
+        if torch.is_grad_enabled():
+            raise RuntimeError("dgv2: the constant-statistic epilogue is first order only (double_backward passes keep the "
+                               "concatenated form)")
+        x, xw, st, y, w = ctx.saved_tensors
+        rec = ctx.rec
+        g, splits, alpha, scale, bshape = ctx.cfg
+        B, H, W, C = x.shape
+        O, P = rec.wf.shape[0], H * W
+        dev = x.device
+        gflat = gflat.contiguous().float()
+        gy = torch.empty((B, H, W, O), device=dev, dtype=torch.float32)
+        gys = torch.empty((B, O), device=dev, dtype=torch.float32)
+        N.check(gflat)
+        N.call("dgv2_epilogue_actbwd_t", N.ptr(gy), N.ptr(gys), N.ptr(gflat), N.ptr(y), B, P, O, alpha, scale, N.stream())
+        gx = gw = gb = None
+        if ctx.needs_input_grad[0]:
+            gxw = torch.empty((B, H, W, C), device=dev, dtype=torch.float32)
+            N.call("dgv2_conv3x3_x3_dgrad", N.ptr(gxw), N.ptr(gy), N.ptr(rec.w8t), N.ptr(rec.wt), B, H, W, C, C, O, None,
+                   N.stream())
+            gx = torch.empty_like(x)
+            N.call("dgv2_mbstd_bwd_cs", N.ptr(gx), None, N.ptr(gxw), N.ptr(x), N.ptr(gys), N.ptr(rec.wsum), O, B, P, C,
+                   splits, g, N.stream())
+        want_gw, want_gb = want_param_grad(ctx, 1), want_param_grad(ctx, 2)
+        if want_gw:
+            out = _wgrad_out(w, rec.scale)
+            if out is None or tuple(out.shape) != (O, C + 1, 3, 3):
+                out = torch.empty((O, C + 1, 3, 3), device=dev, dtype=torch.float32)
+            gb = torch.empty(O, device=dev, dtype=torch.float32) if want_gb else None
+            scratch = torch.empty(N.scratch_elems("dgv2_conv3x3_x3_wgrad_scratch", B, H, W, C, C, O), device=dev,
+                                  dtype=torch.float32)
+            N.call("dgv2_conv3x3_x3_wgrad_cs", N.ptr(out), N.ptr(gb), N.ptr(scratch), scratch.numel(), N.ptr(gy), N.ptr(xw),
+                   N.ptr(st), N.ptr(gys), B, H, W, C, C, O, rec.scale, N.ptr(N.status_word(dev)), N.stream())
+            gw = out.permute(0, 2, 3, 1)
+        elif want_gb:
+            gb = gys.sum(0)
+        return gx, gw, (None if gb is None else gb.reshape(bshape)), None, None, None, None
+
+
+def epilogue_const(x, w, bias, rec, group, splits, act):
+    return _EpilogueConst.apply(x, w, bias, rec, int(group), int(splits), (float(act[0]), float(act[1])))
 
 
 class _FlattenNCHW(Function):
@@ -856,7 +959,7 @@
 
 
 __all__ = ["ConvGeom", "x3_auto", "PreparedConv", "ConvEpilogue", "linear_low", "gemm_x3", "linear_f32", "d_tail_ok",
-           "d_tail", "mbstd_cat_ok", "mbstd_cat", "flatten_nchw", "scaled_handle", "conv8t_image_ok", "conv8_image_ok",
+           "d_tail", "mbstd_cat_ok", "mbstd_cat", "epilogue_const_ok", "conv_weight_bank_cs", "epilogue_const", "flatten_nchw", "scaled_handle", "conv8t_image_ok", "conv8_image_ok",
            "convx3_image_ok", "convx3t_image_ok", "conv_weight_bank", "conv_ring_ep", "conv_ring", "conv_resid_ok",
            "_conv_fwd_raw", "_conv_dgrad_direct", "_conv_dgrad_raw", "_bmm_tn_small", "_conv_wgrad_raw",
            "_resample_actbwd", "_Conv"]
diff --git a/include/dgv2.h b/include/dgv2.h
--- a/include/dgv2.h
+++ b/include/dgv2.h
@@ -175,6 +175,10 @@
                          int xdtype, int ydtype, void* stream);
 int dgv2_mbstd_cat_bwd_x(void* gx, const void* gout, const void* x, int B, int P, int C, int Cp, int splits, int group,
                          int xdtype, int gdtype, void* stream);
+int dgv2_mbstd_widen_fwd(void* out, float* st, float* scratch, const void* x, int B, int P, int C, int splits, int group,
+                         void* stream);
+int dgv2_mbstd_bwd_cs(void* gx, float* gst, const void* gout, const void* x, const float* gy_sum, const float* wsum, int O,
+                      int B, int P, int C, int splits, int group, void* stream);
 int dgv2_gemm_x3(float* c, float* scratch, int64_t scratch_elems, const float* a, const float* b, int I, int J,
                  int64_t T, int a_trans, int b_trans, int64_t lda, int64_t ldb, int64_t ldo, int splits, float scale,
                  void* stream);
@@ -217,6 +221,16 @@
                           int W, int C, int clive, int x_exact, int O, float scale, int param_layout, int* status,
                           void* stream);
 int dgv2_conv3x3_x3_wgrad_scratch(int64_t* elems, int B, int H, int W, int C, int clive, int O);
+int dgv2_conv_weight_bank_cs(void* wf, void* wt, void* w8, void* w8t, float* wsum, const float* src, int O, int C,
+                             float scale, void* stream);
+int dgv2_conv3x3_x3_fwd_cs(void* y, const void* x, const void* w3, int B, int H, int W, int Cx, int x_exact, int O,
+                           const float* bias, const float* st, const float* wsum, int nchw, int act, float alpha,
+                           float scale, int* status, void* stream);
+int dgv2_epilogue_actbwd_t(void* gy, float* gy_sum, const void* g, const void* out, int B, int P, int O, float alpha,
+                           float scale, void* stream);
+int dgv2_conv3x3_x3_wgrad_cs(float* gw, float* gb, float* scratch, int64_t scratch_elems, const void* gy, const void* x,
+                             const float* st, const float* gy_sum, int B, int H, int W, int C, int x_exact, int O,
+                             float scale, int* status, void* stream);
 int dgv2_conv_x3_images(void* w3, void* w3t, const void* w, int O, int Cp, void* stream);
 
 int dgv2_conv_wgrad_stream_scratch(int64_t* elems, int B, int H, int W, int C, int O, int k, int stride,
```

New measurement: 5537 range-images/s (median of 6 runs). No clear change (+0.8%).
